# LasseWolter/laughter-detection-icsi

Measured on AMD Instinct MI355X. Metric: 1 s@16 kHz segments/sec (featurize+ResNet fwd/bwd), higher is better.
Workload: dtype f32 (64->64 and 32->32 convolutions: f16x2 split operands with per-tile power-of-two scales, f32 accumulate; error vs float64 within 1.5x of the exact-f32 kernels'); 1 GPU; BASELINE configs[2]: end-to-end featurize (HIP fbank 44 mel) + ResNetBigger resnet_base fwd/bwd + clip + Adam, random labels, dropout 0.5; global_batch=512, parallelism=dp1, overlap_wgrad=False, overlap_wgrad_small=True, bf16x3_convs=True, f16x2_convs=True, relu_bits=True, virtual_a1=True

## Files before the change

### include/lad_hip.h

```cpp
#ifndef LAD_HIP_H
#define LAD_HIP_H

#include <stdint.h>

#ifdef __cplusplus
extern "C" {
#endif

#define LAD_VERSION 100

enum lad_status {
    LAD_OK = 0,
    LAD_ERR_INVALID = -1,
    LAD_ERR_HIP = -2,
    LAD_ERR_NOMEM = -3,
    LAD_NOT_COVERED = 1
};

int lad_version(void);
const char *lad_last_error(void);

enum lad_pad_mode {
    LAD_PAD_KALDI_MIRROR = 0,
    LAD_PAD_CENTER_REFLECT = 1,
// ... 20 lines not shown

int lad_fbank_plan_create(const lad_fbank_cfg *cfg, const float *window, const float *melbank,
                          const float *dct, void **plan_out);
int lad_fbank_plan_destroy(void *plan);
int lad_fbank_plan_set_kernel(void *plan, int32_t which);
int lad_fbank_plan_has_fast_kernel(const void *plan);
int64_t lad_fbank_num_frames(const void *plan, int64_t samples_per_clip);
int lad_fbank_forward(void *plan, const float *pcm, int64_t n_clips, int64_t samples_per_clip,
                      float *out, void *stream);
int lad_fbank_forward_long(void *plan, const float *pcm, int64_t n_samples, float *out, void *stream);

int lad_gather_segments(const float *const *chan_ptr, const int64_t *chan_frames, const int32_t *chan,
                        const int64_t *first, const int32_t *count, int64_t n_seg, int32_t n_frames, int32_t F, float pad,
                        float *out, void *stream);

typedef struct lad_augment_params {
    uint64_t seed;
    uint32_t epoch;
    float p, mix_p;
    float snr_lo, snr_hi;
    float gain_lo, gain_hi;
    int32_t W;
    int32_t n_time, Wt;
    int32_t n_freq, Wf;
} lad_augment_params;
int lad_gather_segments_aug(const float *const *chan_ptr, const int64_t *chan_frames, const int32_t *chan,
                            const int64_t *first, const int32_t *count, int64_t n_seg, int32_t n_frames, int32_t F, float pad,
                            const lad_augment_params *params, const int32_t *noise_list, int32_t n_noise,
                            int64_t min_noise_frames, float *out, void *stream);

int lad_assemble_windows(const void *stream_act, const void *strips, void *out, int64_t n_windows, int32_t H, int32_t W,
                         int32_t band, int32_t row_bytes, void *stream);


int64_t lad_act_rows(int64_t batch, int32_t H, int32_t W);

int64_t lad_conv_packed_weight_floats(int32_t cout, int32_t cin, int32_t taps, int32_t mode);
int lad_conv_pack_weights(const float *w, int32_t cout, int32_t cin, int32_t taps, int32_t mode, float *wt,
                          void *stream);
int lad_conv_pack_weights_multi(const void *descs, int32_t n_desc, void *stream);
int64_t lad_conv_num_tiles(int64_t batch, int32_t H, int32_t W);
int lad_conv_fwd(const float *in, const float *wt, const float *bias, const float *addend, float *out,
                 float *stat_partials, int64_t batch, int32_t H, int32_t W, int32_t cin, int32_t cout, int32_t taps,
                 void *stream);
int lad_conv_s2_fwd(const float *in, const float *wt, const float *bias, float *out, float *stat_partials,
                    int64_t batch, int32_t H, int32_t W, int32_t cin, int32_t cout, int32_t taps, void *stream);
int lad_bn_fold(const float *gamma, const float *beta, const float *running_mean, const float *running_var,
                const float *conv_bias, int32_t channels, float *scale, float *shift, void *stream);
int lad_conv_fwd_eval(const float *in, const float *wt, const float *scale, const float *shift, const float *addend,
                      float *out, int64_t batch, int32_t H, int32_t W, int32_t cin, int32_t cout, int32_t taps,
                      int32_t relu, void *stream);
int lad_conv_s2_fwd_eval(const float *in, const float *wt, const float *scale, const float *shift, float *out,
                         int64_t batch, int32_t H, int32_t W, int32_t cin, int32_t cout, int32_t taps, int32_t relu,
                         void *stream);
int lad_upsample2(const float *src, float *up, int64_t batch, int32_t H, int32_t W, int32_t channels, void *stream);
int lad_conv_s2_dgrad(const float *dout, const float *wt, float *dx, int64_t batch, int32_t H, int32_t W, int32_t cin,
                      int32_t cout, int32_t taps, int32_t accumulate, void *stream);
int64_t lad_conv_s2_wgrad_workspace_floats(int32_t cin, int32_t cout, int32_t taps);
int lad_conv_s2_wgrad(const float *in, const float *dout, float *workspace, float *dw, float *dbias, int64_t batch, int32_t H,
                      int32_t W, int32_t cin, int32_t cout, int32_t taps, void *stream);
int64_t lad_conv_s2_wgrad_fused_workspace_floats(int32_t cin, int32_t cout);
int lad_conv_s2_wgrad_fused(const float *in, const float *dout, const float *dout_sc, float *workspace, float *dw,
                            float *dbias, float *dw_sc, int64_t batch, int32_t H, int32_t W, int32_t cin, int32_t cout,
                            void *stream);
int lad_conv_s2_fwd_fused(const float *in, const float *wt, const float *bias, const float *wt_sc, float *out,
                          float *stat_partials, float *out_sc, float *stat_partials_sc, int64_t batch, int32_t H, int32_t W,
                          int32_t cin, int32_t cout, void *stream);
int lad_conv_s2_dgrad_fused(const float *dout, const float *wt, const float *dout_sc, const float *wt_sc, float *dx,
                            int64_t batch, int32_t H, int32_t W, int32_t cin, int32_t cout, void *stream);
int64_t lad_conv_s2b3_packed_weight_bytes(void);
int lad_conv_s2b3_pack_weights(const float *w, const float *w_sc, void *wt, void *stream);
int lad_conv_s2b3_fwd(const float *in, const void *wt, const float *bias, float *out, float *stat_partials, float *out_sc,
                      float *stat_partials_sc, int64_t batch, int32_t H, int32_t W, void *stream);
int64_t lad_conv_s2b3_dgrad_packed_weight_bytes(void);
int lad_conv_s2b3_dgrad_pack_weights(const float *w, const float *w_sc, void *wt, void *stream);
int lad_conv_s2b3_pack_weights_pair(const float *w, const float *w_sc, void *wt_fwd, void *wt_dgrad, void *stream);
int64_t lad_conv_s2b3_dgrad_partials(int64_t batch, int32_t H, int32_t W);
int lad_conv_s2b3_dgrad(const float *dout, const float *dout_sc, const void *wt, float *dx, float *stat_partials, const float *bn_x,
                        const uint64_t *bn_bits, const float *bn_coef, int64_t batch, int32_t H, int32_t W, void *stream);
int64_t lad_conv_s2_dgrad_partials(int64_t batch, int32_t H, int32_t W);
int lad_conv_s2_dgrad_fused_bnstat(const float *dout, const float *wt, const float *dout_sc, const float *wt_sc, float *dx,
                                   float *stat_partials, const float *bn_x, const uint64_t *bn_bits, const float *bn_coef,
                                   int64_t batch, int32_t H, int32_t W, int32_t cin, int32_t cout, void *stream);
int64_t lad_conv_wgrad_workspace_floats(int32_t cin, int32_t cout, int32_t taps);
int lad_conv_wgrad(const float *in, const float *dout, float *workspace, float *dw, float *dbias, int64_t batch,
                   int32_t H, int32_t W, int32_t cin, int32_t cout, int32_t taps, void *stream);

int64_t lad_conv_b3_packed_weight_bytes(void);
int lad_conv_b3_pack_weights(const float *w, int32_t mode, void *wt, void *stream);
int lad_conv_b3_fwd_f32(const float *in, const void *wt, const float *bias, const float *addend, float *out,
                        float *partials, int64_t batch, int32_t H, int32_t W, void *stream);
int lad_conv_b3_fwd_f32_gated(const float *in, const void *wt, const float *bias, const float *addend,
                              const uint64_t *addend_bits, float *out, float *partials, int64_t batch, int32_t H,
                              int32_t W, void *stream);
int lad_conv_b3_dgrad_bnstat(const float *in, const void *wt, const float *addend, const uint64_t *addend_bits,
                             float *out, float *stat_partials, const float *bn_x, const uint64_t *bn_bits,
                             const float *bn_coef, int64_t batch, int32_t H, int32_t W, void *stream);
int64_t lad_conv_b3c_packed_weight_bytes(int32_t channels);
int lad_conv_b3c_pack_weights(const float *w, int32_t mode, void *wt, int32_t channels, void *stream);
int lad_conv_b3c_fwd_f32(const float *in, const void *wt, const float *bias, const float *addend, float *out,
                         float *partials, int64_t batch, int32_t H, int32_t W, int32_t channels, void *stream);
int lad_conv_b3c_dgrad_bnstat(const float *in, const void *wt, const float *addend, float *out, float *stat_partials,
                              const float *bn_x, const float *bn_coef, int64_t batch, int32_t H, int32_t W,
                              int32_t channels, void *stream);
int lad_conv_b3c_fwd_f32_bnrelu(const float *in, const float *in_coef, const void *wt, const float *bias, float *out,
                                float *partials, int64_t batch, int32_t H, int32_t W, int32_t channels, void *stream);
int64_t lad_conv_h2_packed_weight_bytes(int32_t channels);
int lad_conv_h2_pack_weights_multi(const void *table, int32_t n, int32_t channels, void *stream);
int lad_conv_wgrad_h2(const float *in, const float *in_coef, const float *dout, float *workspace, float *dw, float *dbias,
                      int64_t batch, int32_t H, int32_t W, int32_t channels, void *stream);
int lad_conv_wgrad_h2_bnbwd(const float *in, const float *in_coef, const float *dy, const float *bn_x, const uint64_t *bn_bits,
                            const float *bn_coef, const float *bcoef, float *dc, float *workspace, float *dw, float *dbias,
                            int64_t batch, int32_t H, int32_t W, int32_t channels, void *stream);
int lad_conv_h2(const float *in, const float *in_coef, const void *wt, const float *bias, const float *addend,
                const uint64_t *addend_bits, float *out, float *partials, const float *bn_x, const uint64_t *bn_bits,
                const float *bn_coef, int64_t batch, int32_t H, int32_t W, int32_t channels, void *stream);
int64_t lad_conv_wgrad_b3c_workspace_floats(int32_t channels);
int lad_conv_wgrad_b3c(const float *in, const float *in_coef, const float *dout, float *workspace, float *dw, float *dbias,
                       int64_t batch, int32_t H, int32_t W, int32_t channels, void *stream);
int lad_conv_b3_fwd_f32_bnrelu(const float *in, const float *in_coef, const void *wt, const float *bias, float *out,
                               float *partials, int64_t batch, int32_t H, int32_t W, void *stream);
int lad_conv_wgrad_b3_bnrelu(const float *in, const float *in_coef, const float *dout, float *workspace, float *dw,
                             float *dbias, int64_t batch, int32_t H, int32_t W, void *stream);
int lad_wgrad_defer_begin(void);
int lad_wgrad_defer_flush(void *stream);
int lad_conv_wgrad_b3(const float *in, const float *dout, float *workspace, float *dw, float *dbias, int64_t batch,
                      int32_t H, int32_t W, void *stream);

int lad_stem_fwd(const float *feat, const float *weight, float *out, float *stat_partials, int64_t batch, int32_t H,
                 int32_t W, int32_t cout, void *stream);
int lad_stem_fwd_eval(const float *feat, const float *weight, const float *scale, const float *shift, float *out,
                      int64_t batch, int32_t H, int32_t W, int32_t cout, int64_t frame_stride, int64_t frames_avail,
                      void *stream);
int64_t lad_stem_moments_workspace_doubles(void);
int64_t lad_stem_moments_doubles(void);
int lad_stem_bn_stats(const float *feat, const float *weight, const float *gamma, const float *beta, float *running_mean,
                      float *running_var, float momentum, float *coef, double *moments, double *workspace, int64_t batch, int32_t H,
                      int32_t W, int32_t cout, void *stream);
int64_t lad_stem_bwd_onepass_workspace_floats(void);
int lad_stem_bwd_onepass(const float *feat, const float *weight, const float *dy, const float *coef, const float *gamma,
                         const double *moments, float *workspace, float *dw, float *dgamma, float *dbeta, int64_t batch, int32_t H,
                         int32_t W, int32_t cout, void *stream);
int64_t lad_stem_wgrad_workspace_floats(void);
int lad_stem_wgrad(const float *feat, const float *dout, float *workspace, float *dw, int64_t batch, int32_t H,
                   int32_t W, int32_t cout, void *stream);
int lad_stem_wgrad_bn(const float *feat, const float *dy, const float *x, const float *weight, const float *coef,
                      const float *bcoef, float *workspace, float *dw, int64_t batch, int32_t H, int32_t W, int32_t cout,
                      void *stream);
int64_t lad_stem_bn_bwd_groups(int64_t batch, int32_t H, int32_t W);
int lad_stem_bn_bwd_sums(const float *feat, const float *weight, const float *dy, const float *coef, float *partials,
                         int64_t batch, int32_t H, int32_t W, int32_t cout, void *stream);

int lad_bn_finalize(float *stat_partials, int64_t n_tiles, int32_t channels, int64_t count, const float *gamma,
                    const float *beta, float *running_mean, float *running_var, float momentum, float *coef,
                    void *stream);
int lad_bn_finalize_pair(float *stat_partials_a, float *stat_partials_b, int64_t n_tiles, int32_t channels, int64_t count,
                         const float *gamma_a, const float *beta_a, float *running_mean_a, float *running_var_a, float *coef_a,
                         const float *gamma_b, const float *beta_b, float *running_mean_b, float *running_var_b, float *coef_b,
                         float momentum, void *stream);
int lad_bn_act(const float *x, const float *coef, const float *res, const float *res_coef, float *y, int64_t batch,
               int32_t H, int32_t W, int32_t channels, int32_t relu, void *stream);
int64_t lad_bn_bwd_workspace_floats(int32_t channels);
int lad_bn_bwd(const float *dy, const float *y, const float *x, const float *coef, const float *gamma,
               const float *xs, const float *scoef, const float *sgamma, float *dx, float *aux, float *dgamma,
               float *dbeta, float *dsgamma, float *dsbeta, float *workspace, float *bcoef, float *pre_partials,
               int64_t pre_tiles, int64_t batch, int32_t H, int32_t W, int32_t channels, int32_t relu, int32_t mode,
               void *stream);
int lad_bn_act_bits(const float *x, const float *coef, const float *res, const float *res_coef, float *y,
                    uint64_t *y_bits, int64_t batch, int32_t H, int32_t W, int32_t channels, void *stream);
int lad_bn_bwd_bits(const float *dy, const uint64_t *y_bits, const float *x, const float *coef, const float *gamma,
                    float *dx, float *dgamma, float *dbeta, float *workspace, float *bcoef, float *pre_partials,
                    int64_t pre_tiles, int64_t batch, int32_t H, int32_t W, int32_t channels, void *stream);
int lad_conv_fwd_bnstat(const float *in, const float *wt, const float *addend, float *out, float *stat_partials,
                        const float *bn_x, const float *bn_y, const float *bn_coef, int64_t batch, int32_t H, int32_t W,
                        int32_t cin, int32_t cout, int32_t taps, void *stream);

int lad_pool_fwd(const float *x, float *pooled, int64_t batch, int32_t H, int32_t W, int32_t channels, void *stream);
int lad_pool_bwd(const float *dpooled, float *dx, int64_t batch, int32_t H, int32_t W, int32_t channels, void *stream);
int64_t lad_head_workspace_floats(int64_t batch, int32_t F);
int lad_head_fwd_train(const float *const *params, const float *pooled, int64_t batch, int32_t F, const float *drop1,
                       const float *drop2, const int32_t *labels, float momentum, float *h, float *stats,
                       float *probs, float *metrics, void *stream);
int lad_head_fwd_train_rng(const float *const *params, const float *pooled, int64_t batch, int32_t F, float *drop1, float *drop2, float keep,
                           uint64_t seed, int64_t *rng_counter, int64_t *nbt, int32_t n_nbt, const int32_t *labels, float momentum,
                           float *h, float *stats, float *probs, float *metrics, void *stream);
int lad_head_fwd_eval(const float *const *params, const float *pooled, int64_t batch, int32_t F, float *probs,
                      void *stream);
int lad_bce_metrics(const float *probs, const int32_t *labels, int64_t n, float *metrics, void *stream);
int lad_head_bwd(const float *const *params, float *const *grads, const float *pooled, const float *h,
                 const float *stats, const float *probs, const float *dprobs, int64_t batch, int32_t F,
                 const float *drop1, const float *drop2, const int32_t *labels, float *workspace, float *dpooled,
                 void *stream);

int64_t lad_f16_packed_weight_halfs(int32_t cout, int32_t cin, int32_t taps);
int lad_f16_pack_weights(const float *w, int32_t cout, int32_t cin, int32_t taps, void *wt, void *stream);
int lad_f16_stem_fwd(const float *feat, const float *weight, const float *scale, const float *shift, void *out,
                     int64_t batch, int32_t H, int32_t W, int32_t cout, int64_t frame_stride, int64_t frames_avail,
                     void *stream);
int lad_f16_conv_fwd(const void *in, const void *wt, const float *scale, const float *shift, const void *addend, void *out,
                     int64_t batch, int32_t H, int32_t W, int32_t cin, int32_t cout, int32_t taps, int32_t relu,
                     void *stream);
int lad_f16_conv_s2_fwd(const void *in, const void *wt, const float *scale, const float *shift, void *out, int64_t batch,
                        int32_t H, int32_t W, int32_t cin, int32_t cout, int32_t taps, int32_t relu, void *stream);
int lad_f16_block_fwd(const void *x, const void *wt1, const float *scale1, const float *shift1, const void *wt2,
                      const float *scale2, const float *shift2, void *y, int64_t batch, int32_t H, int32_t W, int32_t channels,
                      void *stream);
int lad_f16_block_fwd_stem_rows(const void *stream_act, int64_t stream_rows, int64_t stream_row0, const float *feat, int64_t frames_avail,
                                const float *stem_weight, const float *stem_scale, const float *stem_shift, const void *wt1,
                                const float *scale1, const float *shift1, const void *wt2, const float *scale2, const float *shift2, void *y,
                                int64_t batch, int32_t H, int32_t W, void *stream);
int lad_f16_conv_s2_strips_fwd(const void *act, const void *wt, const float *scale, const float *shift, void *out, const void *wt_sc,
                               const float *scale_sc, const float *shift_sc, void *out_sc, int64_t n_windows, int32_t H, int32_t W,
                               int32_t band, int32_t strip_rows, int64_t bottom_image0, int64_t stream_row0, int64_t act_rows,
                               int32_t out_rows, void *stream);
int lad_f16_tail_fwd(const void *act, int64_t n_windows, int32_t H, int32_t W, int32_t band, int32_t strip_rows, int64_t bot_img0,
                     int64_t stream_row0, int32_t phases, int64_t phase_img, int64_t act_rows, const void *const *conv_params,
                     const float *const *head_params, int32_t F, float *probs, void *stream);
int lad_f16_conv_s2_fwd_windows(const void *act, const void *wt, const float *scale, const float *shift, void *out,
                                int64_t n_windows, int32_t H, int32_t W, int32_t band, int32_t cin, int32_t cout, int32_t taps,
                                int32_t relu, void *stream);
int lad_f16_conv_s2_fwd_mapped(const void *act, const void *wt, const float *scale, const float *shift, void *out,
                               int64_t n_windows, int32_t H, int32_t W, int32_t band, int32_t strip_rows, int64_t bottom_image0,
                               int64_t stream_row0, int32_t phases, int64_t phase_rows, int64_t act_rows, int32_t out_rows,
                               int32_t cin, int32_t cout, int32_t taps, int32_t relu, void *stream);
int lad_f16_conv_s2_fwd_sc(const void *in, const void *wt, const float *scale, const float *shift, void *out, const void *wt_sc,
                           const float *scale_sc, const float *shift_sc, void *out_sc, int64_t batch, int32_t H, int32_t W,
                           int32_t cin, int32_t cout, int32_t relu, void *stream);
int lad_f16_conv_s2_fwd_mapped_sc(const void *act, const void *wt, const float *scale, const float *shift, void *out,
                                  const void *wt_sc, const float *scale_sc, const float *shift_sc, void *out_sc, int64_t n_windows,
                                  int32_t H, int32_t W, int32_t band, int32_t strip_rows, int64_t bottom_image0, int64_t stream_row0,
                                  int32_t phases, int64_t phase_rows, int64_t act_rows, int32_t out_rows, int32_t cin, int32_t cout,
                                  int32_t relu, void *stream);
int lad_f16_pool_fwd(const void *x, float *pooled, int64_t batch, int32_t H, int32_t W, int32_t channels, void *stream);

int32_t lad_grad_sumsq_partials(void);
int lad_grad_sumsq(const float *grad, int64_t n, float *partials, int64_t *step_counter, void *stream);
int lad_grad_accumulate(float *acc, const float *grad, int64_t n, double scale, void *stream);
int lad_adam_step(float *param, float *grad, float *exp_avg, float *exp_avg_sq, int64_t n,
                  const float *sumsq_partials, double grad_scale, double max_norm, double lr, double beta1,
                  double beta2, double eps, int64_t step, const int64_t *step_counter, int32_t zero_grad,
                  float *norm_out, void *stream);

enum lad_runs_dtype { LAD_RUNS_F32 = 0, LAD_RUNS_F64 = 1 };
int32_t lad_runs_tile_frames(void);
int32_t lad_runs_max_thresholds(void);
int64_t lad_runs_workspace_bytes(int64_t channels, int64_t frames, int32_t n_thresholds);
int lad_runs_count(const void *probs, int32_t dtype, int64_t channels, int64_t frames, const double *thresholds,
                   int32_t n_thresholds, void *workspace, void *stream);
int lad_runs_fill(const void *probs, int32_t dtype, int64_t channels, int64_t frames, const double *thresholds,
                  int32_t n_thresholds, const void *workspace, const int32_t *counts_host, int32_t *table,
// ... 89 lines not shown
```

### laughter-detection-icsi_amd/_hip.py

```python
import ctypes
import os

import torch

_HERE = os.path.dirname(os.path.abspath(__file__))
LIB_PATH = os.environ.get("LAD_HIP_LIB") or os.path.join(_HERE, "liblad_hip.so")

c_void_p = ctypes.c_void_p
c_int = ctypes.c_int
c_i64 = ctypes.c_int64
c_float = ctypes.c_float
c_double = ctypes.c_double
c_i32 = ctypes.c_int32
c_float_p = ctypes.POINTER(ctypes.c_float)


class LadHipError(RuntimeError):
    pass


class FbankCfg(ctypes.Structure):
    _fields_ = [("n_fft", ctypes.c_int32), ("frame_len", ctypes.c_int32), ("hop", ctypes.c_int32),
                ("n_mels", ctypes.c_int32), ("n_mfcc", ctypes.c_int32), ("pad_mode", ctypes.c_int32),
                ("log_mode", ctypes.c_int32), ("remove_dc", ctypes.c_int32), ("preemph", ctypes.c_float),
                ("log_floor", ctypes.c_float)]


class AugmentParams(ctypes.Structure):
    _fields_ = [("seed", ctypes.c_uint64), ("epoch", ctypes.c_uint32), ("p", ctypes.c_float), ("mix_p", ctypes.c_float),
                ("snr_lo", ctypes.c_float), ("snr_hi", ctypes.c_float), ("gain_lo", ctypes.c_float), ("gain_hi", ctypes.c_float),
                ("W", ctypes.c_int32), ("n_time", ctypes.c_int32), ("Wt", ctypes.c_int32), ("n_freq", ctypes.c_int32),
                ("Wf", ctypes.c_int32)]


SIGNATURES = {
    "lad_version": (c_int, []),
    "lad_last_error": (ctypes.c_char_p, []),
    "lad_fbank_plan_create": (c_int, [ctypes.POINTER(FbankCfg), c_void_p, c_void_p, c_void_p,
                                      ctypes.POINTER(c_void_p)]),
    "lad_fbank_plan_destroy": (c_int, [c_void_p]),
    "lad_fbank_plan_set_kernel": (c_int, [c_void_p, c_int]),
    "lad_fbank_plan_has_fast_kernel": (c_int, [c_void_p]),
    "lad_fbank_num_frames": (c_i64, [c_void_p, c_i64]),
    "lad_fbank_forward": (c_int, [c_void_p, c_void_p, c_i64, c_i64, c_void_p, c_void_p]),
    "lad_fbank_forward_long": (c_int, [c_void_p, c_void_p, c_i64, c_void_p, c_void_p]),
    "lad_gather_segments": (c_int, [c_void_p] * 5 + [c_i64, c_i32, c_i32, c_float, c_void_p, c_void_p]),
    "lad_gather_segments_aug": (c_int, [c_void_p] * 5 + [c_i64, c_i32, c_i32, c_float, ctypes.POINTER(AugmentParams), c_void_p, c_i32, c_i64,
                                        c_void_p, c_void_p]),
    "lad_assemble_windows": (c_int, [c_void_p, c_void_p, c_void_p, c_i64, c_i32, c_i32, c_i32, c_i32, c_void_p]),
    "lad_act_rows": (c_i64, [c_i64, c_i32, c_i32]),
    "lad_conv_packed_weight_floats": (c_i64, [c_i32, c_i32, c_i32, c_i32]),
    "lad_conv_pack_weights": (c_int, [c_void_p, c_i32, c_i32, c_i32, c_i32, c_void_p, c_void_p]),
    "lad_conv_pack_weights_multi": (c_int, [c_void_p, c_i32, c_void_p]),
    "lad_conv_num_tiles": (c_i64, [c_i64, c_i32, c_i32]),
    "lad_conv_fwd": (c_int, [c_void_p] * 6 + [c_i64, c_i32, c_i32, c_i32, c_i32, c_i32, c_void_p]),
    "lad_conv_b3_packed_weight_bytes": (c_i64, []),
    "lad_conv_b3_pack_weights": (c_int, [c_void_p, c_i32, c_void_p, c_void_p]),
    "lad_conv_b3_fwd_f32": (c_int, [c_void_p] * 6 + [c_i64, c_i32, c_i32, c_void_p]),
    "lad_conv_b3c_packed_weight_bytes": (c_i64, [c_i32]),
    "lad_conv_b3c_pack_weights": (c_int, [c_void_p, c_i32, c_void_p, c_i32, c_void_p]),
    "lad_conv_b3c_fwd_f32": (c_int, [c_void_p] * 6 + [c_i64, c_i32, c_i32, c_i32, c_void_p]),
    "lad_conv_b3c_fwd_f32_bnrelu": (c_int, [c_void_p] * 6 + [c_i64, c_i32, c_i32, c_i32, c_void_p]),
    "lad_conv_b3c_dgrad_bnstat": (c_int, [c_void_p] * 7 + [c_i64, c_i32, c_i32, c_i32, c_void_p]),
    "lad_conv_h2_packed_weight_bytes": (c_i64, [c_i32]),
    "lad_conv_h2_pack_weights_multi": (c_int, [c_void_p, c_i32, c_i32, c_void_p]),
    "lad_conv_wgrad_h2": (c_int, [c_void_p] * 6 + [c_i64, c_i32, c_i32, c_i32, c_void_p]),
    "lad_conv_h2": (c_int, [c_void_p] * 11 + [c_i64, c_i32, c_i32, c_i32, c_void_p]),
    "lad_conv_wgrad_h2_bnbwd": (c_int, [c_void_p] * 11 + [c_i64, c_i32, c_i32, c_i32, c_void_p]),
    "lad_conv_wgrad_b3c_workspace_floats": (c_i64, [c_i32]),
    "lad_conv_wgrad_b3c": (c_int, [c_void_p] * 6 + [c_i64, c_i32, c_i32, c_i32, c_void_p]),
    "lad_conv_b3_fwd_f32_gated": (c_int, [c_void_p] * 7 + [c_i64, c_i32, c_i32, c_void_p]),
    "lad_conv_b3_fwd_f32_bnrelu": (c_int, [c_void_p] * 6 + [c_i64, c_i32, c_i32, c_void_p]),
    "lad_conv_wgrad_b3_bnrelu": (c_int, [c_void_p] * 6 + [c_i64, c_i32, c_i32, c_void_p]),
    "lad_wgrad_defer_begin": (c_int, []),
    "lad_wgrad_defer_flush": (c_int, [c_void_p]),
    "lad_conv_b3_dgrad_bnstat": (c_int, [c_void_p] * 9 + [c_i64, c_i32, c_i32, c_void_p]),
    "lad_conv_wgrad_b3": (c_int, [c_void_p] * 5 + [c_i64, c_i32, c_i32, c_void_p]),
    "lad_conv_s2_fwd": (c_int, [c_void_p] * 5 + [c_i64, c_i32, c_i32, c_i32, c_i32, c_i32, c_void_p]),
    "lad_bn_fold": (c_int, [c_void_p] * 5 + [c_i32, c_void_p, c_void_p, c_void_p]),
    "lad_conv_fwd_eval": (c_int, [c_void_p] * 6 + [c_i64, c_i32, c_i32, c_i32, c_i32, c_i32, c_i32, c_void_p]),
    "lad_conv_s2_fwd_eval": (c_int, [c_void_p] * 5 + [c_i64, c_i32, c_i32, c_i32, c_i32, c_i32, c_i32, c_void_p]),
    "lad_upsample2": (c_int, [c_void_p, c_void_p, c_i64, c_i32, c_i32, c_i32, c_void_p]),
    "lad_conv_s2_dgrad": (c_int, [c_void_p] * 3 + [c_i64, c_i32, c_i32, c_i32, c_i32, c_i32, c_i32, c_void_p]),
    "lad_conv_s2_wgrad_workspace_floats": (c_i64, [c_i32, c_i32, c_i32]),
    "lad_conv_s2_fwd_fused": (c_int, [c_void_p] * 8 + [c_i64, c_i32, c_i32, c_i32, c_i32, c_void_p]),
    "lad_conv_s2_dgrad_partials": (c_i64, [c_i64, c_i32, c_i32]),
    "lad_conv_s2b3_packed_weight_bytes": (c_i64, []),
    "lad_conv_s2b3_pack_weights": (c_int, [c_void_p, c_void_p, c_void_p, c_void_p]),
    "lad_conv_s2b3_fwd": (c_int, [c_void_p] * 7 + [c_i64, c_i32, c_i32, c_void_p]),
    "lad_conv_s2b3_dgrad_packed_weight_bytes": (c_i64, []),
    "lad_conv_s2b3_dgrad_pack_weights": (c_int, [c_void_p, c_void_p, c_void_p, c_void_p]),
    "lad_conv_s2b3_pack_weights_pair": (c_int, [c_void_p] * 5),
    "lad_conv_s2b3_dgrad_partials": (c_i64, [c_i64, c_i32, c_i32]),
    "lad_conv_s2b3_dgrad": (c_int, [c_void_p] * 8 + [c_i64, c_i32, c_i32, c_void_p]),
    "lad_conv_s2_dgrad_fused_bnstat": (c_int, [c_void_p] * 9 + [c_i64, c_i32, c_i32, c_i32, c_i32, c_void_p]),
    "lad_conv_s2_dgrad_fused": (c_int, [c_void_p] * 5 + [c_i64, c_i32, c_i32, c_i32, c_i32, c_void_p]),
    "lad_conv_s2_wgrad_fused_workspace_floats": (c_i64, [c_i32, c_i32]),
    "lad_conv_s2_wgrad_fused": (c_int, [c_void_p] * 7 + [c_i64, c_i32, c_i32, c_i32, c_i32, c_void_p]),
    "lad_conv_s2_wgrad": (c_int, [c_void_p] * 5 + [c_i64, c_i32, c_i32, c_i32, c_i32, c_i32, c_void_p]),
    "lad_conv_wgrad_workspace_floats": (c_i64, [c_i32, c_i32, c_i32]),
    "lad_conv_wgrad": (c_int, [c_void_p] * 5 + [c_i64, c_i32, c_i32, c_i32, c_i32, c_i32, c_void_p]),
    "lad_stem_fwd": (c_int, [c_void_p] * 4 + [c_i64, c_i32, c_i32, c_i32, c_void_p]),
    "lad_stem_fwd_eval": (c_int, [c_void_p] * 5 + [c_i64, c_i32, c_i32, c_i32, c_i64, c_i64, c_void_p]),
    "lad_stem_wgrad_workspace_floats": (c_i64, []),
    "lad_stem_wgrad": (c_int, [c_void_p] * 4 + [c_i64, c_i32, c_i32, c_i32, c_void_p]),
    "lad_stem_wgrad_bn": (c_int, [c_void_p] * 8 + [c_i64, c_i32, c_i32, c_i32, c_void_p]),
    "lad_stem_bn_bwd_groups": (c_i64, [c_i64, c_i32, c_i32]),
    "lad_stem_bn_bwd_sums": (c_int, [c_void_p] * 5 + [c_i64, c_i32, c_i32, c_i32, c_void_p]),
    "lad_bn_finalize": (c_int, [c_void_p, c_i64, c_i32, c_i64, c_void_p, c_void_p, c_void_p, c_void_p, c_float,
                                c_void_p, c_void_p]),
    "lad_stem_moments_workspace_doubles": (c_i64, []),
    "lad_stem_moments_doubles": (c_i64, []),
    "lad_stem_bn_stats": (c_int, [c_void_p] * 6 + [c_float] + [c_void_p] * 3 + [c_i64, c_i32, c_i32, c_i32, c_void_p]),
    "lad_stem_bwd_onepass_workspace_floats": (c_i64, []),
    "lad_stem_bwd_onepass": (c_int, [c_void_p] * 10 + [c_i64, c_i32, c_i32, c_i32, c_void_p]),
    "lad_bn_finalize_pair": (c_int, [c_void_p, c_void_p, c_i64, c_i32, c_i64] + [c_void_p] * 10 + [c_float, c_void_p]),
    "lad_bn_act": (c_int, [c_void_p] * 5 + [c_i64, c_i32, c_i32, c_i32, c_i32, c_void_p]),
    "lad_bn_bwd_workspace_floats": (c_i64, [c_i32]),
    "lad_bn_act_bits": (c_int, [c_void_p] * 6 + [c_i64, c_i32, c_i32, c_i32, c_void_p]),
    "lad_bn_bwd_bits": (c_int, [c_void_p] * 11 + [c_i64, c_i64, c_i32, c_i32, c_i32, c_void_p]),
    "lad_bn_bwd": (c_int, [c_void_p] * 17 + [c_i64, c_i64, c_i32, c_i32, c_i32, c_i32, c_i32, c_void_p]),
    "lad_conv_fwd_bnstat": (c_int, [c_void_p] * 8 + [c_i64, c_i32, c_i32, c_i32, c_i32, c_i32, c_void_p]),
    "lad_pool_fwd": (c_int, [c_void_p, c_void_p, c_i64, c_i32, c_i32, c_i32, c_void_p]),
    "lad_pool_bwd": (c_int, [c_void_p, c_void_p, c_i64, c_i32, c_i32, c_i32, c_void_p]),
    "lad_head_workspace_floats": (c_i64, [c_i64, c_i32]),
    "lad_head_fwd_train": (c_int, [c_void_p, c_void_p, c_i64, c_i32, c_void_p, c_void_p, c_void_p, c_float,
                                   c_void_p, c_void_p, c_void_p, c_void_p, c_void_p]),
    "lad_head_fwd_train_rng": (c_int, [c_void_p, c_void_p, c_i64, c_i32, c_void_p, c_void_p, c_float, ctypes.c_uint64, c_void_p, c_void_p, c_i32,
                                       c_void_p, c_float, c_void_p, c_void_p, c_void_p, c_void_p, c_void_p]),
    "lad_head_fwd_eval": (c_int, [c_void_p, c_void_p, c_i64, c_i32, c_void_p, c_void_p]),
    "lad_bce_metrics": (c_int, [c_void_p, c_void_p, c_i64, c_void_p, c_void_p]),
    "lad_head_bwd": (c_int, [c_void_p] * 7 + [c_i64, c_i32] + [c_void_p] * 6),
    "lad_f16_packed_weight_halfs": (c_i64, [c_i32, c_i32, c_i32]),
    "lad_f16_pack_weights": (c_int, [c_void_p, c_i32, c_i32, c_i32, c_void_p, c_void_p]),
    "lad_f16_stem_fwd": (c_int, [c_void_p] * 5 + [c_i64, c_i32, c_i32, c_i32, c_i64, c_i64, c_void_p]),
    "lad_f16_conv_fwd": (c_int, [c_void_p] * 6 + [c_i64, c_i32, c_i32, c_i32, c_i32, c_i32, c_i32, c_void_p]),
    "lad_f16_block_fwd": (c_int, [c_void_p] * 8 + [c_i64, c_i32, c_i32, c_i32, c_void_p]),
    "lad_f16_conv_s2_fwd_sc": (c_int, [c_void_p] * 9 + [c_i64, c_i32, c_i32, c_i32, c_i32, c_i32, c_void_p]),
    "lad_f16_conv_s2_fwd_mapped_sc": (c_int, [c_void_p] * 9 + [c_i64, c_i32, c_i32, c_i32, c_i32, c_i64, c_i64, c_i32, c_i64, c_i64, c_i32,
                                              c_i32, c_i32, c_i32, c_void_p]),
    "lad_f16_conv_s2_fwd": (c_int, [c_void_p] * 5 + [c_i64, c_i32, c_i32, c_i32, c_i32, c_i32, c_i32, c_void_p]),
    "lad_f16_conv_s2_fwd_windows": (c_int, [c_void_p] * 5 + [c_i64, c_i32, c_i32, c_i32, c_i32, c_i32, c_i32, c_i32, c_void_p]),
    "lad_f16_conv_s2_fwd_mapped": (c_int, [c_void_p] * 5 + [c_i64, c_i32, c_i32, c_i32, c_i32, c_i64, c_i64, c_i32, c_i64, c_i64, c_i32,
                                                          c_i32, c_i32, c_i32, c_i32, c_void_p]),
    "lad_f16_block_fwd_stem_rows": (c_int, [c_void_p, c_i64, c_i64, c_void_p, c_i64] + [c_void_p] * 10 + [c_i64, c_i32, c_i32, c_void_p]),
    "lad_f16_conv_s2_strips_fwd": (c_int, [c_void_p] * 9 + [c_i64, c_i32, c_i32, c_i32, c_i32, c_i64, c_i64, c_i64, c_i32, c_void_p]),
    "lad_f16_tail_fwd": (c_int, [c_void_p, c_i64, c_i32, c_i32, c_i32, c_i32, c_i64, c_i64, c_i32, c_i64, c_i64, c_void_p, c_void_p, c_i32,
                                 c_void_p, c_void_p]),
    "lad_f16_pool_fwd": (c_int, [c_void_p, c_void_p, c_i64, c_i32, c_i32, c_i32, c_void_p]),
    "lad_grad_sumsq_partials": (c_i32, []),
    "lad_grad_sumsq": (c_int, [c_void_p, c_i64, c_void_p, c_void_p, c_void_p]),
    "lad_grad_accumulate": (c_int, [c_void_p, c_void_p, c_i64, c_double, c_void_p]),
    "lad_adam_step": (c_int, [c_void_p] * 4 + [c_i64, c_void_p] + [c_double] * 6 + [c_i64, c_void_p, c_i32, c_void_p, c_void_p]),
    "lad_runs_tile_frames": (c_i32, []),
    "lad_runs_max_thresholds": (c_i32, []),
    "lad_runs_workspace_bytes": (c_i64, [c_i64, c_i64, c_i32]),
    "lad_runs_count": (c_int, [c_void_p, c_i32, c_i64, c_i64, ctypes.POINTER(c_double), c_i32, c_void_p, c_void_p]),
    "lad_runs_fill": (c_int, [c_void_p, c_i32, c_i64, c_i64, ctypes.POINTER(c_double), c_i32, c_void_p,
                              ctypes.POINTER(c_i32), c_void_p, c_i64, c_void_p]),
    "lad_score_max_min_lengths": (c_i32, []),
    "lad_score_workspace_bytes": (c_i64, [c_i64, c_i64, c_i32, c_i32]),
    "lad_score_runs": (c_int, [c_void_p, c_void_p, ctypes.POINTER(c_i32), c_i64, c_i64, c_i32, c_void_p, c_void_p,
                               ctypes.POINTER(c_i32), ctypes.POINTER(c_i32), c_i64, c_void_p, ctypes.POINTER(c_double),
                               ctypes.POINTER(c_double), c_i32, c_void_p, c_void_p, c_void_p]),
    "lad_score_events_workspace_bytes": (c_i64, [c_i64, c_i64, c_i32, c_i32, c_i64]),
    "lad_score_events": (c_int, [c_void_p, c_void_p, ctypes.POINTER(c_i32), c_i64, c_i64, c_i32, c_void_p, c_void_p,
                                 ctypes.POINTER(c_i32), ctypes.POINTER(c_i32), c_i64, c_void_p, ctypes.POINTER(c_double),
                                 ctypes.POINTER(c_double), c_i32, c_i32, c_i32, c_void_p, c_void_p, c_void_p]),
    "lad_binarize_max_settings": (c_i32, []),
    "lad_binarize_workspace_bytes": (c_i64, [c_i64, c_i64, c_i32]),
    "lad_binarize_count": (c_int, [c_void_p, c_i32, c_i64, c_i64, ctypes.POINTER(c_double), ctypes.POINTER(c_double), c_i32,
                                   c_void_p, c_void_p]),
    "lad_binarize_fill": (c_int, [c_void_p, c_i32, c_i64, c_i64] + [ctypes.POINTER(c_double)] * 3
                          + [c_i32, c_void_p, ctypes.POINTER(c_double), c_void_p, ctypes.POINTER(c_i32), c_void_p, c_void_p, c_i64,
                             c_void_p]),
    "lad_viterbi_max_settings": (c_i32, []),
    "lad_viterbi_table_entries": (c_i32, []),
    "lad_viterbi_workspace_bytes": (c_i64, [c_i64, c_i64, c_i32]),
    "lad_viterbi_count": (c_int, [c_void_p, c_i32, c_i64, c_i64, c_void_p] + [ctypes.POINTER(c_i32)] * 3
                          + [c_i32, c_void_p, c_void_p, c_void_p]),
    "lad_viterbi_fill": (c_int, [c_void_p, ctypes.POINTER(c_i32), c_i64, c_i64, c_i32, c_void_p, c_i64, c_void_p]),
    "lad_surface_max_levels": (c_i32, []),
    "lad_surface_tile_frames": (c_i32, []),
    "lad_surface_workspace_bytes": (c_i64, [c_i64, c_i64, c_i64, c_i32, c_i32]),
    "lad_score_surface": (c_int, [c_void_p, c_i32, c_i64, c_i64, ctypes.POINTER(c_double), c_i32, c_void_p, c_void_p,
                                  ctypes.POINTER(c_i32), ctypes.POINTER(c_i32), c_i64, c_void_p, ctypes.POINTER(c_double),
                                  ctypes.POINTER(c_double), c_i32, c_void_p, c_void_p, c_void_p]),
    "lad_surface_events_workspace_bytes": (c_i64, [c_i64, c_i64, c_i64, c_i32, c_i32]),
    "lad_score_surface_events": (c_int, [c_void_p, c_i32, c_i64, c_i64, ctypes.POINTER(c_double), c_i32, c_void_p, c_void_p,
                                         ctypes.POINTER(c_i32), ctypes.POINTER(c_i32), c_i64, c_void_p, ctypes.POINTER(c_double),
                                         ctypes.POINTER(c_double), c_i32, c_i32, c_i32, c_void_p, c_void_p, c_void_p, c_void_p]),
    "lad_resample_out_len": (c_i64, [c_i64, c_i32, c_i32]),
    "lad_resample_tile_outputs": (c_i32, []),
    "lad_resample_max_up": (c_i32, []),
    "lad_resample_max_down": (c_i32, []),
    "lad_resample_max_taps": (c_i32, []),
    "lad_resample_max_lds_bytes": (c_i64, []),
    "lad_resample_lds_bytes": (c_i64, [c_i32, c_i32, c_i32]),
    "lad_resample": (c_int, [c_void_p, c_i32, c_i64, c_void_p, c_i32, c_i32, c_i32, c_i64, c_i64, c_void_p, c_void_p]),
    "lad_lowpass_tile_frames": (c_i32, []),
    "lad_lowpass_workspace_bytes": (c_i64, [c_i64, c_i64]),
    "lad_lowpass": (c_int, [c_void_p, c_i32, c_i64, c_i64, ctypes.POINTER(c_i64)] + [ctypes.POINTER(c_double)] * 3
# ... 54 lines not shown
```

### laughter-detection-icsi_amd/csrc/bn.hip

```cpp
#include "lad_common.h"
#include "lad_device.h"
#include "lad_bn_math.h"

namespace {
using namespace lad;

constexpr float BN_EPS = 1e-5f;
constexpr int THREADS = 256;

struct FinSet {
    const float *partials, *gamma, *beta;
    float *running_mean, *running_var, *coef;
};
struct FinSets {
    FinSet s[2];
};
__global__ void bn_finalize_kernel(FinSets sets, int64_t n_tiles, int C, double count, float momentum) {
    const FinSet f = sets.s[blockIdx.y];
    const float *__restrict__ partials = f.partials;
    float *__restrict__ coef = f.coef;
    const int c = blockIdx.x;
    double s1 = 0.0, s2 = 0.0;
    int64_t t = threadIdx.x;
    const int64_t bd = blockDim.x;
// ... 109 lines not shown
    __syncthreads();
    if (!last_s) return;
    if (threadIdx.x == 0) __hip_atomic_store(ft.ticket, 0u, __ATOMIC_RELAXED, __HIP_MEMORY_SCOPE_AGENT);
    const int slices = (int)gridDim.x;
    double *tot = &red[0][0];
    if (threadIdx.x < cols) {
        double tt = 0.0;
        double *hd = reinterpret_cast<double *>(partials) + threadIdx.x;
        const int64_t step = rows_per_slice * cols / 2;
        int b = 0;
        for (; b + 32 <= slices; b += 32) {
            double v[32];
#pragma unroll
            for (int u = 0; u < 32; ++u) v[u] = __hip_atomic_load(hd + (b + u) * step, __ATOMIC_RELAXED, __HIP_MEMORY_SCOPE_AGENT);
#pragma unroll
            for (int u = 0; u < 32; ++u) tt += v[u];
        }
        for (; b + 8 <= slices; b += 8) {
            double v[8];
#pragma unroll
            for (int u = 0; u < 8; ++u) v[u] = __hip_atomic_load(hd + (b + u) * step, __ATOMIC_RELAXED, __HIP_MEMORY_SCOPE_AGENT);
#pragma unroll
            for (int u = 0; u < 8; ++u) tt += v[u];
        }
        for (; b < slices; ++b) tt += __hip_atomic_load(hd + b * step, __ATOMIC_RELAXED, __HIP_MEMORY_SCOPE_AGENT);
        tot[threadIdx.x] = tt;
    }
    __syncthreads();
    const int c = threadIdx.x;
    if (c >= C) return;
    if (!ft.backward) {
        float *coef = ft.out;
        const double count = ft.count;
        const double mean = tot[c] / count;
        double var = tot[C + c] / count - mean * mean;
        if (var < 0.0) var = 0.0;
        const double invstd_d = 1.0 / sqrt(var + (double)BN_EPS);
        const float invstd = (float)invstd_d;
        const float scale = ft.gamma[c] * invstd;
        coef[0 * C + c] = scale;
        coef[1 * C + c] = ft.beta[c] - (float)mean * scale;
        coef[2 * C + c] = (float)mean;
        coef[3 * C + c] = invstd;
        coef[4 * C + c] = (float)(mean - (double)(float)mean);
        coef[5 * C + c] = (float)(invstd_d - (double)invstd);
        if (ft.running_mean != nullptr) {
            const double unbiased = count > 1.0 ? var * count / (count - 1.0) : var;
            ft.running_mean[c] = (1.0f - ft.momentum) * ft.running_mean[c] + ft.momentum * (float)mean;
            ft.running_var[c] = (1.0f - ft.momentum) * ft.running_var[c] + ft.momentum * (float)unbiased;
        }
    } else {
        float *bcoef = ft.out;
        const double t0 = tot[c], t1 = tot[C + c];
        ft.dbeta[c] = (float)t0;
        ft.dgamma[c] = (float)t1;
        const double k2 = t0 / ft.count, k3 = t1 / ft.count;
        bcoef[0 * C + c] = ft.gamma[c] * ft.coef[3 * C + c];
        bcoef[1 * C + c] = (float)k2;
        bcoef[2 * C + c] = (float)k3;
        bcoef[4 * C + c] = (float)(k2 - (double)(float)k2);
        bcoef[6 * C + c] = (float)(k3 - (double)(float)k3);
    }
}

struct RowGeom {
    int64_t n_img_rows;
    int Hp, Wp;
};

struct RowPack {
    int rows, sub, f0, fstep;
};
__device__ __forceinline__ RowPack row_pack(int per_row) {
    RowPack p{1, 0, (int)threadIdx.x, (int)blockDim.x};
    if (2 * per_row <= (int)blockDim.x) {
        p.rows = (int)blockDim.x / per_row;
        p.sub = (int)threadIdx.x / per_row;
        p.f0 = (int)threadIdx.x - p.sub * per_row;
        p.fstep = per_row;
    }
    return p;
}

template <int RES, bool BITS = false>
__global__ void bn_act_kernel(const float4 *__restrict__ x, const float *__restrict__ coef,
                              const float4 *__restrict__ res, const float *__restrict__ rcoef, float4 *__restrict__ y,
                              RowGeom g, int C, int c4shift, int relu, unsigned long long *__restrict__ bits = nullptr) {
    const int c = (threadIdx.x * 4) & (C - 1);
    const int per_row = g.Wp << c4shift;
    const float4 sc = *reinterpret_cast<const float4 *>(coef + c);
    const float4 sh = *reinterpret_cast<const float4 *>(coef + C + c);
    float4 rs = sc, rh = sh;
    if (RES == 2) {
        rs = *reinterpret_cast<const float4 *>(rcoef + c);
        rh = *reinterpret_cast<const float4 *>(rcoef + C + c);
    }
    const RowPack rp = row_pack(per_row);
    for (int64_t r = (int64_t)blockIdx.x * rp.rows + rp.sub; rp.sub < rp.rows && r < g.n_img_rows; r += (int64_t)gridDim.x * rp.rows) {
        const int yp = (int)(r % g.Hp);
        const bool border_row = (yp == 0);
        const int64_t base = r * per_row;
        for (int f = rp.f0; f < per_row; f += rp.fstep) {
            const int64_t idx = base + f;
            const int xp = f >> c4shift;
            float4 o = make_float4(0.f, 0.f, 0.f, 0.f);
            if (!(border_row | (xp == 0))) {
                const float4 v = x[idx];
                o = make_float4(fmaf(v.x, sc.x, sh.x), fmaf(v.y, sc.y, sh.y), fmaf(v.z, sc.z, sh.z), fmaf(v.w, sc.w, sh.w));
                if (RES == 1) {
                    const float4 rr = res[idx];
                    o.x += rr.x; o.y += rr.y; o.z += rr.z; o.w += rr.w;
                } else if (RES == 2) {
                    const float4 rr = res[idx];
                    o.x += fmaf(rr.x, rs.x, rh.x); o.y += fmaf(rr.y, rs.y, rh.y);
                    o.z += fmaf(rr.z, rs.z, rh.z); o.w += fmaf(rr.w, rs.w, rh.w);
                }
                if (relu) {
                    o.x = fmaxf(o.x, 0.f); o.y = fmaxf(o.y, 0.f); o.z = fmaxf(o.z, 0.f); o.w = fmaxf(o.w, 0.f);
                }
            }
            y[idx] = o;
            if (BITS) {
                const unsigned long long word = pack_sign_bits(o, threadIdx.x & 63);
                if ((threadIdx.x & 15) == 0) bits[idx >> 4] = word;
            }
        }
    }
}

template <int C, bool SHORT>
__global__ __launch_bounds__(THREADS) void bn_bwd_reduce_kernel(const float4 *__restrict__ dy, const float4 *__restrict__ y,
                                                                const float4 *__restrict__ x, const float *__restrict__ coef,
                                                                const float4 *__restrict__ xs, const float *__restrict__ scoef,
                                                                float *__restrict__ partials, int64_t rows, int relu,
                                                                const unsigned long long *__restrict__ bits) {
    constexpr int C4 = C / 4;
    constexpr int RP = THREADS / C4;
    constexpr int K = SHORT ? 3 : 2;
    const int c4 = threadIdx.x % C4, rp = threadIdx.x / C4;
    const Norm4 nm = load_norm(coef, C, c4 * 4);
    Norm4 sn = nm;
    if (SHORT) sn = load_norm(scoef, C, c4 * 4);
    const float4 fscale = *reinterpret_cast<const float4 *>(coef + c4 * 4);
    const float4 fshift = *reinterpret_cast<const float4 *>(coef + C + c4 * 4);
    float4 a0 = make_float4(0, 0, 0, 0), a1 = a0, a2 = a0;
    for (int64_t row = (int64_t)blockIdx.x * RP + rp; row < rows; row += (int64_t)gridDim.x * RP) {
        const int64_t idx = row * C4 + c4;
        float4 d = dy[idx];
        const float4 xv = x[idx];
        if (relu == 1) {
            const float4 yy = y[idx];
            d.x = yy.x > 0.f ? d.x : 0.f; d.y = yy.y > 0.f ? d.y : 0.f;
            d.z = yy.z > 0.f ? d.z : 0.f; d.w = yy.w > 0.f ? d.w : 0.f;
        } else if (relu == 2) {
            d = mask_from_x(d, xv, fscale, fshift);
        } else if (relu == 3) {
            d = mask_from_bits(d, bits[row], c4);
        }
        a0.x += d.x; a0.y += d.y; a0.z += d.z; a0.w += d.w;
        const float4 xh = xhat4(xv, nm);
        a1.x = fmaf(d.x, xh.x, a1.x); a1.y = fmaf(d.y, xh.y, a1.y);
        a1.z = fmaf(d.z, xh.z, a1.z); a1.w = fmaf(d.w, xh.w, a1.w);
        if (SHORT) {
            const float4 sh = xhat4(xs[idx], sn);
            a2.x = fmaf(d.x, sh.x, a2.x); a2.y = fmaf(d.y, sh.y, a2.y);
            a2.z = fmaf(d.z, sh.z, a2.z); a2.w = fmaf(d.w, sh.w, a2.w);
        }
    }
    __shared__ float red[RP][K][C];
    *reinterpret_cast<float4 *>(&red[rp][0][c4 * 4]) = a0;
    *reinterpret_cast<float4 *>(&red[rp][1][c4 * 4]) = a1;
    if (SHORT) *reinterpret_cast<float4 *>(&red[rp][2][c4 * 4]) = a2;
    __syncthreads();
    for (int t = threadIdx.x; t < K * C; t += THREADS) {
        const int k = t / C, c = t - k * C;
        float s = 0.f;
#pragma unroll 4
        for (int p = 0; p < RP; ++p) s += red[p][k][c];
        partials[((int64_t)blockIdx.x * K + k) * C + c] = s;
    }
}

__global__ void bn_bwd_finalize_kernel(const float *__restrict__ partials, int groups, int K, int C, double count,
                                       const float *__restrict__ gamma, const float *__restrict__ coef,
                                       const float *__restrict__ sgamma, const float *__restrict__ scoef,
                                       float *__restrict__ dgamma, float *__restrict__ dbeta,
                                       float *__restrict__ dsgamma, float *__restrict__ dsbeta, float *__restrict__ bcoef) {
    const int c = blockIdx.x;
    double s[3] = {0.0, 0.0, 0.0};
    int g = threadIdx.x;
    const int bd = blockDim.x;
    const int k2 = K - 1;
    for (; g + 3 * bd < groups; g += 4 * bd) {
        float v[4][3];
#pragma unroll
        for (int u = 0; u < 4; ++u) {
            const float *row = partials + (int64_t)(g + u * bd) * K * C + c;
            v[u][0] = row[0];
            v[u][1] = row[C];
            v[u][2] = row[k2 * C];
        }
#pragma unroll
        for (int u = 0; u < 4; ++u) {
            s[0] += (double)v[u][0];
            s[1] += (double)v[u][1];
            s[2] += (double)v[u][2];
        }
    }
    for (; g < groups; g += bd) {
        const float *row = partials + (int64_t)g * K * C + c;
        const float v0 = row[0], v1 = row[C], v2 = row[k2 * C];
        s[0] += (double)v0;
        s[1] += (double)v1;
        s[2] += (double)v2;
    }
    __shared__ double red[3][THREADS / 64];
    for (int k = 0; k < 3; ++k) {
        const double v = wave_sum64d(s[k]);
        if ((threadIdx.x & 63) == 0) red[k][threadIdx.x >> 6] = v;
    }
    __syncthreads();
    if (threadIdx.x == 0) {
        double t[3] = {0.0, 0.0, 0.0};
        for (int k = 0; k < 3; ++k)
            for (int w = 0; w < THREADS / 64; ++w) t[k] += red[k][w];
        dbeta[c] = (float)t[0];
        dgamma[c] = (float)t[1];
        const double k2 = t[0] / count, k3 = t[1] / count;
        bcoef[0 * C + c] = gamma[c] * coef[3 * C + c];
        bcoef[1 * C + c] = (float)k2;
        bcoef[2 * C + c] = (float)k3;
        bcoef[4 * C + c] = (float)(k2 - (double)(float)k2);
        bcoef[6 * C + c] = (float)(k3 - (double)(float)k3);
        if (K == 3) {
            const double j3 = t[2] / count;
            dsbeta[c] = (float)t[0];
            dsgamma[c] = (float)t[2];
            bcoef[3 * C + c] = sgamma[c] * scoef[3 * C + c];
            bcoef[5 * C + c] = (float)j3;
            bcoef[7 * C + c] = (float)(j3 - (double)(float)j3);
        }
    }
}

template <int MODE>
__global__ void bn_bwd_apply_kernel(const float4 *__restrict__ dy, const float4 *__restrict__ y, const float4 *__restrict__ x,
                                    const float *__restrict__ coef, const float *__restrict__ bcoef,
                                    const float4 *__restrict__ xs, const float *__restrict__ scoef, float4 *__restrict__ dx,
                                    float4 *__restrict__ aux, RowGeom g, int C, int c4shift, int relu,
                                    const unsigned long long *__restrict__ bits) {
    const int c = (threadIdx.x * 4) & (C - 1);
    const int per_row = g.Wp << c4shift;
    const float4 zero = make_float4(0.f, 0.f, 0.f, 0.f);
    const float4 fsc = *reinterpret_cast<const float4 *>(coef + c), fsh = *reinterpret_cast<const float4 *>(coef + C + c);
    const Norm4 nm = load_norm(coef, C, c);
    const float4 k1 = *reinterpret_cast<const float4 *>(bcoef + 0 * C + c);
    const float4 k2 = *reinterpret_cast<const float4 *>(bcoef + 1 * C + c);
    const float4 k3 = *reinterpret_cast<const float4 *>(bcoef + 2 * C + c);
    const float4 k2l = *reinterpret_cast<const float4 *>(bcoef + 4 * C + c);
    const float4 k3l = *reinterpret_cast<const float4 *>(bcoef + 6 * C + c);
    Norm4 sn = nm;
    float4 j1 = k1, j3 = k3, j3l = k3l;
    if (MODE == 2) {
        sn = load_norm(scoef, C, c);
        j1 = *reinterpret_cast<const float4 *>(bcoef + 3 * C + c);
        j3 = *reinterpret_cast<const float4 *>(bcoef + 5 * C + c);
        j3l = *reinterpret_cast<const float4 *>(bcoef + 7 * C + c);
    }
    const RowPack rp = row_pack(per_row);
    for (int64_t r = (int64_t)blockIdx.x * rp.rows + rp.sub; rp.sub < rp.rows && r < g.n_img_rows; r += (int64_t)gridDim.x * rp.rows) {
        const int yp = (int)(r % g.Hp);
        const bool border_row = (yp == 0);
        const int64_t base = r * per_row;
        for (int f = rp.f0; f < per_row; f += rp.fstep) {
            const int64_t idx = base + f;
            const int xp = f >> c4shift;
            if (border_row | (xp == 0)) {
                dx[idx] = zero;
                if (MODE != 0) aux[idx] = zero;
                continue;
            }
            float4 d = dy[idx];
            const float4 xv = x[idx];
            if (relu == 1) {
                const float4 yy = y[idx];
                d.x = yy.x > 0.f ? d.x : 0.f; d.y = yy.y > 0.f ? d.y : 0.f;
                d.z = yy.z > 0.f ? d.z : 0.f; d.w = yy.w > 0.f ? d.w : 0.f;
            } else if (relu == 2) {
                d = mask_from_x(d, xv, fsc, fsh);
            } else if (relu == 3) {
                d = mask_from_bits(d, bits[idx >> 4], threadIdx.x & 15);
            }
            const float4 xh = xhat4(xv, nm);
            float4 o;
            o.x = bn_dx1(d.x, xh.x, k1.x, k2.x, k2l.x, k3.x, k3l.x);
            o.y = bn_dx1(d.y, xh.y, k1.y, k2.y, k2l.y, k3.y, k3l.y);
            o.z = bn_dx1(d.z, xh.z, k1.z, k2.z, k2l.z, k3.z, k3l.z);
            o.w = bn_dx1(d.w, xh.w, k1.w, k2.w, k2l.w, k3.w, k3l.w);
            dx[idx] = o;
            if (MODE == 1) {
                aux[idx] = d;
            } else if (MODE == 2) {
                const float4 sh = xhat4(xs[idx], sn);
                float4 sv;
                sv.x = bn_dx1(d.x, sh.x, j1.x, k2.x, k2l.x, j3.x, j3l.x);
                sv.y = bn_dx1(d.y, sh.y, j1.y, k2.y, k2l.y, j3.y, j3l.y);
                sv.z = bn_dx1(d.z, sh.z, j1.z, k2.z, k2l.z, j3.z, j3l.z);
                sv.w = bn_dx1(d.w, sh.w, j1.w, k2.w, k2l.w, j3.w, j3l.w);
                aux[idx] = sv;
            }
        }
    }
}

unsigned row_grid(int64_t n_img_rows, int float4_per_row) {
    const int rows = 2 * float4_per_row <= THREADS ? THREADS / float4_per_row : 1;
    return (unsigned)std::min<int64_t>(lad::ceil_div(n_img_rows, (int64_t)rows), float4_per_row >= 2 * THREADS ? 256 * 256 : 256 * 32);
}
int log2_exact(int v) {
    int s = 0;
    while ((1 << s) < v) ++s;
    return s;
}
RowGeom make_row_geom(int64_t batch, int H, int W) {
    RowGeom g;
    g.Hp = H + 1;
    g.Wp = W + 1;
    g.n_img_rows = batch * g.Hp;
    return g;
}
constexpr int BWD_GROUPS = 1024;
}

extern "C" int lad_bn_finalize(float *stat_partials, int64_t n_tiles, int32_t channels, int64_t count,
                               const float *gamma, const float *beta, float *running_mean, float *running_var,
                               float momentum, float *coef, void *stream) {
    using namespace lad;
    LAD_REQUIRE(stat_partials && gamma && beta && coef, "lad_bn_finalize: null buffer");
    LAD_REQUIRE(channels > 0 && n_tiles > 0 && count > 0, "lad_bn_finalize: bad sizes");
    LAD_REQUIRE((running_mean == nullptr) == (running_var == nullptr), "lad_bn_finalize: running stats must come in pairs");
    if (n_tiles >= TWO_LEVEL_MIN_TILES && 2 * channels <= 128 && THREADS % (channels / 2) == 0) {
        const int64_t rps = ceil_div(n_tiles, FIN_SLICES);
        const int slices = (int)(n_tiles / rps);
        const FinTail ft{0, (double)count, gamma, beta, nullptr, running_mean, running_var, momentum, coef, nullptr, nullptr, launch_ticket()};
        LAD_REQUIRE(ft.ticket, "lad_bn_finalize: no ticket for the two-level sum");
        hipLaunchKernelGGL(bn_slice_sum_kernel, dim3(slices), dim3(THREADS), 0, (hipStream_t)stream, stat_partials, n_tiles, channels, rps, ft);
        return check_launch("bn_slice_sum_kernel");
    }
    const FinSets sets{{{stat_partials, gamma, beta, running_mean, running_var, coef}, {nullptr, nullptr, nullptr, nullptr, nullptr, nullptr}}};
    hipLaunchKernelGGL(bn_finalize_kernel, dim3(channels, 1), dim3(THREADS), 0, (hipStream_t)stream, sets, n_tiles, channels, (double)count, momentum);
    return check_launch("bn_finalize_kernel");
}

extern "C" int lad_bn_finalize_pair(float *stat_partials_a, float *stat_partials_b, int64_t n_tiles, int32_t channels, int64_t count,
                                    const float *gamma_a, const float *beta_a, float *running_mean_a, float *running_var_a, float *coef_a,
                                    const float *gamma_b, const float *beta_b, float *running_mean_b, float *running_var_b, float *coef_b,
                                    float momentum, void *stream) {
    using namespace lad;
    LAD_REQUIRE(stat_partials_a && stat_partials_b && gamma_a && beta_a && coef_a && gamma_b && beta_b && coef_b, "lad_bn_finalize_pair: null buffer");
    LAD_REQUIRE(channels > 0 && n_tiles > 0 && count > 0, "lad_bn_finalize_pair: bad sizes");
    LAD_REQUIRE((running_mean_a == nullptr) == (running_var_a == nullptr) && (running_mean_b == nullptr) == (running_var_b == nullptr),
                "lad_bn_finalize_pair: running stats must come in pairs");
    if (n_tiles >= TWO_LEVEL_MIN_TILES && 2 * channels <= 128 && THREADS % (channels / 2) == 0) {
        const int rc = lad_bn_finalize(stat_partials_a, n_tiles, channels, count, gamma_a, beta_a, running_mean_a, running_var_a, momentum, coef_a, stream);
        return rc ? rc : lad_bn_finalize(stat_partials_b, n_tiles, channels, count, gamma_b, beta_b, running_mean_b, running_var_b, momentum, coef_b, stream);
    }
    const FinSets sets{{{stat_partials_a, gamma_a, beta_a, running_mean_a, running_var_a, coef_a},
                        {stat_partials_b, gamma_b, beta_b, running_mean_b, running_var_b, coef_b}}};
    hipLaunchKernelGGL(bn_finalize_kernel, dim3(channels, 2), dim3(THREADS), 0, (hipStream_t)stream, sets, n_tiles, channels, (double)count, momentum);
    return check_launch("bn_finalize_kernel");
}

__global__ void bn_fold_kernel(const float *__restrict__ gamma, const float *__restrict__ beta,
                               const float *__restrict__ running_mean, const float *__restrict__ running_var,
                               const float *__restrict__ conv_bias, int C, float *__restrict__ scale, float *__restrict__ shift) {
    const int c = blockIdx.x * blockDim.x + threadIdx.x;
    if (c < C) {
        const float s = gamma[c] / sqrtf(running_var[c] + BN_EPS);
        const float b = conv_bias != nullptr ? conv_bias[c] : 0.0f;
        scale[c] = s;
        shift[c] = fmaf(b - running_mean[c], s, beta[c]);
    }
}

extern "C" int lad_bn_fold(const float *gamma, const float *beta, const float *running_mean, const float *running_var,
                           const float *conv_bias, int32_t channels, float *scale, float *shift, void *stream) {
    using namespace lad;
    LAD_REQUIRE(gamma && beta && running_mean && running_var && scale && shift && channels > 0, "lad_bn_fold: bad argument");
    hipLaunchKernelGGL(bn_fold_kernel, dim3((unsigned)ceil_div(channels, 64)), dim3(64), 0, (hipStream_t)stream, gamma, beta,
                       running_mean, running_var, conv_bias, channels, scale, shift);
    return check_launch("bn_fold_kernel");
}

namespace {
int bn_act_impl(const float *x, const float *coef, const float *res, const float *res_coef, float *y, unsigned long long *bits,
                int64_t batch, int32_t H, int32_t W, int32_t channels, int32_t relu, void *stream, const char *who) {
    using namespace lad;
    LAD_REQUIRE(x && coef && y, "%s: null buffer", who);
    LAD_REQUIRE(channels >= 4 && channels <= 4 * THREADS && (channels & (channels - 1)) == 0, "%s: channels must be a power of two in 4..1024", who);
    LAD_REQUIRE(res != nullptr || res_coef == nullptr, "%s: res_coef without res", who);
    LAD_REQUIRE(batch >= 0 && H >= 1 && W >= 1, "%s: bad geometry", who);
    LAD_REQUIRE(bits == nullptr || channels == 64, "%s: sign bits are kept for 64-channel activations only", who);
    if (batch == 0) return LAD_OK;
    const RowGeom g = make_row_geom(batch, H, W);
    const int sh = log2_exact(channels / 4);
    const dim3 grid(row_grid(g.n_img_rows, g.Wp << sh)), block(THREADS);
    hipStream_t st = (hipStream_t)stream;
#define LAD_ACT(RES, R, RC)                                                                                                   \
    do {                                                                                                                      \
        if (bits)                                                                                                             \
            hipLaunchKernelGGL((bn_act_kernel<RES, true>), grid, block, 0, st, (const float4 *)x, coef, (const float4 *)(R), RC, \
                               (float4 *)y, g, channels, sh, relu, bits);                                                     \
        else                                                                                                                  \
            hipLaunchKernelGGL((bn_act_kernel<RES, false>), grid, block, 0, st, (const float4 *)x, coef, (const float4 *)(R), RC, \
                               (float4 *)y, g, channels, sh, relu, nullptr);                                                  \
    } while (0)
    if (res == nullptr)
        LAD_ACT(0, nullptr, nullptr);
    else if (res_coef == nullptr)
        LAD_ACT(1, res, nullptr);
    else
        LAD_ACT(2, res, res_coef);
#undef LAD_ACT
    return check_launch("bn_act_kernel");
}
}

extern "C" int lad_bn_act(const float *x, const float *coef, const float *res, const float *res_coef, float *y,
                          int64_t batch, int32_t H, int32_t W, int32_t channels, int32_t relu, void *stream) {
    return bn_act_impl(x, coef, res, res_coef, y, nullptr, batch, H, W, channels, relu, stream, "lad_bn_act");
}

extern "C" int lad_bn_act_bits(const float *x, const float *coef, const float *res, const float *res_coef, float *y,
                               uint64_t *y_bits, int64_t batch, int32_t H, int32_t W, int32_t channels, void *stream) {
    using namespace lad;
    LAD_REQUIRE(y_bits, "lad_bn_act_bits: null sign-bit buffer");
    return bn_act_impl(x, coef, res, res_coef, y, (unsigned long long *)y_bits, batch, H, W, channels, 1, stream, "lad_bn_act_bits");
}

extern "C" int64_t lad_bn_bwd_workspace_floats(int32_t channels) { return (int64_t)BWD_GROUPS * 3 * channels; }

namespace {
int bn_bwd_impl(const float *dy, const float *y, const unsigned long long *bits, const float *x, const float *coef, const float *gamma,
                const float *xs, const float *scoef, const float *sgamma, float *dx, float *aux,
                float *dgamma, float *dbeta, float *dsgamma, float *dsbeta, float *workspace, float *bcoef,
                float *pre_partials, int64_t pre_tiles, int64_t batch, int32_t H, int32_t W, int32_t channels,
                int32_t relu, int32_t mode, void *stream) {
    using namespace lad;
    LAD_REQUIRE(relu != 3 || (bits && channels == 64), "lad_bn_bwd_bits: sign bits are kept for 64-channel activations only");
    LAD_REQUIRE(dy && coef && gamma && dgamma && dbeta && workspace && bcoef, "lad_bn_bwd: null buffer");
    LAD_REQUIRE(x || (pre_partials && !dx), "lad_bn_bwd: x may only be omitted when the sums are given and nothing is applied");
    LAD_REQUIRE(dx || mode == 0, "lad_bn_bwd: dx may only be omitted (sums and coefficients only) in mode 0");
    LAD_REQUIRE(relu >= 0 && relu <= 3, "lad_bn_bwd: relu must be 0 (none), 1 (mask from y), 2 (mask recomputed from x) or 3 (sign bits: lad_bn_bwd_bits)");
    LAD_REQUIRE(relu != 1 || y, "lad_bn_bwd: relu = 1 needs y");
    LAD_REQUIRE(relu != 2 || mode == 0, "lad_bn_bwd: relu = 2 (mask recomputed from x) is for the residual-free BatchNorm only");
    LAD_REQUIRE(mode >= 0 && mode <= 2, "lad_bn_bwd: bad mode");
    LAD_REQUIRE(mode == 0 || aux, "lad_bn_bwd: mode needs aux");
    LAD_REQUIRE(mode != 2 || (xs && scoef && sgamma && dsgamma && dsbeta), "lad_bn_bwd: mode 2 needs the shortcut tensors");
    LAD_REQUIRE(channels == 16 || channels == 32 || channels == 64 || channels == 128, "lad_bn_bwd: channels must be 16, 32, 64 or 128");
    LAD_REQUIRE(batch >= 0 && H >= 1 && W >= 1, "lad_bn_bwd: bad geometry");
    if (batch == 0) return LAD_OK;
    const RowGeom rg = make_row_geom(batch, H, W);
    const int64_t rows = rg.n_img_rows * rg.Wp;
    const int64_t count = batch * H * W;
    hipStream_t st = (hipStream_t)stream;
    const int rp = THREADS / (channels / 4);
    int groups = (int)std::min<int64_t>(BWD_GROUPS, ceil_div(rows, rp));
    const bool sh = mode == 2;
    const float *sums = workspace;
    if (pre_partials != nullptr) {
        LAD_REQUIRE(!sh && pre_tiles >= 1 && pre_tiles < (1 << 30), "lad_bn_bwd: pre-computed sums are for modes 0 and 1");
        sums = pre_partials;
        groups = (int)pre_tiles;
    } else {
#define LAD_RED(CC)                                                                                                  \
    if (channels == CC) {                                                                                            \
        if (sh)                                                                                                      \
            hipLaunchKernelGGL((bn_bwd_reduce_kernel<CC, true>), dim3(groups), dim3(THREADS), 0, st, (const float4 *)dy, \
                               (const float4 *)y, (const float4 *)x, coef, (const float4 *)xs, scoef, workspace, rows, relu, bits); \
        else                                                                                                         \
            hipLaunchKernelGGL((bn_bwd_reduce_kernel<CC, false>), dim3(groups), dim3(THREADS), 0, st, (const float4 *)dy, \
                               (const float4 *)y, (const float4 *)x, coef, nullptr, nullptr, workspace, rows, relu, bits); \
    }
    LAD_RED(16) LAD_RED(32) LAD_RED(64) LAD_RED(128)
#undef LAD_RED
    }
    int rc = check_launch("bn_bwd_reduce_kernel");
    if (rc) return rc;
    if (pre_partials != nullptr && groups >= TWO_LEVEL_MIN_TILES && 2 * channels <= 128 && THREADS % (channels / 2) == 0) {
        const int64_t rps = ceil_div((int64_t)groups, FIN_SLICES);
        const int slices = (int)(groups / rps);
        const FinTail ft{1, (double)count, gamma, nullptr, coef, nullptr, nullptr, 0.0f, bcoef, dgamma, dbeta, launch_ticket()};
        LAD_REQUIRE(ft.ticket, "lad_bn_bwd: no ticket for the two-level sum");
        hipLaunchKernelGGL(bn_slice_sum_kernel, dim3(slices), dim3(THREADS), 0, st, pre_partials, (int64_t)groups, channels, rps, ft);
    } else {
        hipLaunchKernelGGL(bn_bwd_finalize_kernel, dim3(channels), dim3(THREADS), 0, st, sums, groups, sh ? 3 : 2, channels,
                           (double)count, gamma, coef, sgamma, scoef, dgamma, dbeta, dsgamma, dsbeta, bcoef);
    }
    rc = check_launch("bn_bwd_finalize_kernel");
    if (rc) return rc;
    if (dx == nullptr) return LAD_OK;
    const int c4s = log2_exact(channels / 4);
    const dim3 grid(row_grid(rg.n_img_rows, rg.Wp << c4s)), block(THREADS);
    if (mode == 0)
        hipLaunchKernelGGL(bn_bwd_apply_kernel<0>, grid, block, 0, st, (const float4 *)dy, (const float4 *)y, (const float4 *)x,
                           coef, bcoef, nullptr, nullptr, (float4 *)dx, nullptr, rg, channels, c4s, relu, bits);
    else if (mode == 1)
        hipLaunchKernelGGL(bn_bwd_apply_kernel<1>, grid, block, 0, st, (const float4 *)dy, (const float4 *)y, (const float4 *)x,
                           coef, bcoef, nullptr, nullptr, (float4 *)dx, (float4 *)aux, rg, channels, c4s, relu, bits);
    else
        hipLaunchKernelGGL(bn_bwd_apply_kernel<2>, grid, block, 0, st, (const float4 *)dy, (const float4 *)y, (const float4 *)x,
                           coef, bcoef, (const float4 *)xs, scoef, (float4 *)dx, (float4 *)aux, rg, channels, c4s, relu, bits);
    return check_launch("bn_bwd_apply_kernel");
}
}

extern "C" int lad_bn_bwd(const float *dy, const float *y, const float *x, const float *coef, const float *gamma,
                          const float *xs, const float *scoef, const float *sgamma, float *dx, float *aux,
                          float *dgamma, float *dbeta, float *dsgamma, float *dsbeta, float *workspace, float *bcoef,
                          float *pre_partials, int64_t pre_tiles, int64_t batch, int32_t H, int32_t W, int32_t channels,
                          int32_t relu, int32_t mode, void *stream) {
    using namespace lad;
    LAD_REQUIRE(relu >= 0 && relu <= 2, "lad_bn_bwd: relu must be 0, 1 or 2");
    return bn_bwd_impl(dy, y, nullptr, x, coef, gamma, xs, scoef, sgamma, dx, aux, dgamma, dbeta, dsgamma, dsbeta, workspace, bcoef,
                       pre_partials, pre_tiles, batch, H, W, channels, relu, mode, stream);
}

extern "C" int lad_bn_bwd_bits(const float *dy, const uint64_t *y_bits, const float *x, const float *coef, const float *gamma,
                               float *dx, float *dgamma, float *dbeta, float *workspace, float *bcoef, float *pre_partials,
                               int64_t pre_tiles, int64_t batch, int32_t H, int32_t W, int32_t channels, void *stream) {
    using namespace lad;
    LAD_REQUIRE(y_bits && x, "lad_bn_bwd_bits: null buffer");
// ... 4 lines not shown
```

### laughter-detection-icsi_amd/csrc/conv_h2.hip

```cpp
#include "lad_common.h"
#include "lad_device.h"
#include "lad_b3_tile.h"
#include "lad_bn_math.h"
#include "lad_h2.h"

#include <algorithm>
#include <cstdlib>

namespace {
using namespace lad;
using namespace lad::b3t;

constexpr int KC = 32;
constexpr int ROWB = 128;
constexpr int FPIECES = KC * 4 / 16;

template <int C>
struct H2 {
    static constexpr int NSTAGE = C / KC;
    static constexpr int NCT = C / 16;
    static constexpr int PLANE_B = NCT * 1024;
    static constexpr int TAP_BYTES = 2 * PLANE_B;
    static constexpr int IMG_BYTES = TAPS * NSTAGE * TAP_BYTES;
    static constexpr int TAIL_BYTES = 16;
// ... 295 lines not shown
            b3_epilogue<C, STAT>(store_acc, bias, addend, abits, out, partials, mask_s + rb * TM, reinterpret_cast<float *>(smem_b), qs, g.rows, bst);
        else
            h2_epilogue<C, STAT, (EPI & 1) != 0, (EPI >> 1) & 3, (EPI & 8) != 0, (EPI & 16) != 0>(
                store_acc, bias, addend, abits, out, partials, mask_s + rb * TM, reinterpret_cast<float *>(smem_b), qs, g.rows, bst);
    }
    LAD_H2_STAMP(12)
}

template <int C, int RB>
size_t h2_lds_bytes(const Geom &g) {
    using K = H2<C>;
    const int nrows = TM * RB + 2 * (g.Wp + 1);
    const size_t main_bytes = std::max<size_t>(NSLOT * K::TAP_BYTES + (size_t)nrows * ROWB, (size_t)TM * (C + 4) * 4);
    return main_bytes + TM * RB + 16;
}

int h2_two_rounds() {
    static int n = 0;
    if (n == 0) {
        int dev = 0;
        hipDeviceProp_t prop;
        n = (hipGetDevice(&dev) == hipSuccess && hipGetDeviceProperties(&prop, dev) == hipSuccess && prop.multiProcessorCount > 0)
                ? 4 * prop.multiProcessorCount : 1024;
    }
    return n;
}

struct H2Args {
    const float *in, *in_coef;
    const unsigned char *wt;
    const float *bias, *addend;
    const unsigned long long *abits;
    float *out, *partials;
    B3Stat bst;
    Geom g;
    hipStream_t stream;
};

template <int C, int RB, bool STAT, bool INBN, int EPI>
int launch_h2_form(const H2Args &a) {
    static lad::DeviceOnce attr_set;
    if (!attr_set) {
        LAD_HIP_CHECK(hipFuncSetAttribute((const void *)conv_h2_kernel<C, RB, STAT, INBN, EPI>, hipFuncAttributeMaxDynamicSharedMemorySize, 96 * 1024));
        attr_set = true;
    }
    const int64_t tiles = ceil_div(a.g.rows, TM * RB);
    hipLaunchKernelGGL((conv_h2_kernel<C, RB, STAT, INBN, EPI>), dim3((unsigned)(ceil_div(tiles, 8) * 8)), dim3(THREADS), (h2_lds_bytes<C, RB>(a.g)),
                       a.stream, a.in, a.wt, a.bias, a.addend, a.abits, a.out, a.partials, a.g, a.bst, a.in_coef);
    return check_launch("conv_h2_kernel");
}

template <int C, int RB, bool STAT, bool INBN>
int launch_h2_rb(const H2Args &a) {
    const int form = h2_epi(a.bias != nullptr, a.addend == nullptr ? H2_ADD_NONE : a.abits == nullptr ? H2_ADD_PLAIN : H2_ADD_GATED,
                            a.partials != nullptr, STAT && a.bst.bits != nullptr);
#define LAD_H2_FORM(...)                                                                                                           \
    if (form == h2_epi(__VA_ARGS__)) return launch_h2_form<C, RB, STAT, INBN, h2_epi(__VA_ARGS__)>(a);
    if constexpr (STAT) {
        LAD_H2_FORM(false, H2_ADD_NONE, true, false)
        LAD_H2_FORM(false, H2_ADD_GATED, true, true)
    } else {
        LAD_H2_FORM(true, H2_ADD_NONE, true, false)
        LAD_H2_FORM(true, H2_ADD_PLAIN, true, false)
        if constexpr (!INBN) {
            LAD_H2_FORM(false, H2_ADD_NONE, false, false)
            LAD_H2_FORM(false, H2_ADD_PLAIN, false, false)
            LAD_H2_FORM(false, H2_ADD_GATED, false, false)
        }
    }
#undef LAD_H2_FORM
    return launch_h2_form<C, RB, STAT, INBN, H2_EPI_ANY>(a);
}

template <int C, bool STAT, bool INBN>
int launch_h2(const float *in, const float *in_coef, const void *wt, const float *bias, const float *addend, const uint64_t *abits,
              float *out, float *partials, const B3Stat &bst, int64_t batch, int32_t H, int32_t W, void *stream, const char *who) {
    const Geom g = make_geom(batch, H, W);
    LAD_REQUIRE(g.rows < ((int64_t)1 << 31) && g.img < (1 << 20), "%s: more than 2^31 rows, or an image of more than 2^20 positions", who);
    LAD_REQUIRE(W <= 46, "%s: image too wide for the tile (W = %d)", who, W);
    const H2Args a{in, in_coef, (const unsigned char *)wt, bias, addend, (const unsigned long long *)abits, out, partials, bst, g, (hipStream_t)stream};
    if (ceil_div(g.rows, TM * 2) < h2_two_rounds()) return launch_h2_rb<C, 1, STAT, INBN>(a);
    return launch_h2_rb<C, 2, STAT, INBN>(a);
}
}

extern "C" int64_t lad_conv_h2_packed_weight_bytes(int32_t channels) {
    if (channels == 64) return H2<64>::IMG_BYTES + H2<64>::TAIL_BYTES;
    if (channels == 32) return H2<32>::IMG_BYTES + H2<32>::TAIL_BYTES;
    return -1;
}

extern "C" int lad_conv_h2_pack_weights_multi(const void *table, int32_t n, int32_t channels, void *stream) {
    using namespace lad;
    LAD_REQUIRE(table && n >= 1, "lad_conv_h2_pack_weights_multi: empty table");
    static_assert(sizeof(PackRec) == 24, "record layout");
    if (channels == 64) hipLaunchKernelGGL(pack_h2_kernel<64>, dim3(n * PACK_SPLIT), dim3(1024), 0, (hipStream_t)stream, (const PackRec *)table);
    else if (channels == 32) hipLaunchKernelGGL(pack_h2_kernel<32>, dim3(n * PACK_SPLIT), dim3(1024), 0, (hipStream_t)stream, (const PackRec *)table);
    else if (channels == 0) hipLaunchKernelGGL(pack_h2_kernel<0>, dim3(n * PACK_SPLIT), dim3(1024), 0, (hipStream_t)stream, (const PackRec *)table);
    else return fail(LAD_ERR_INVALID, "lad_conv_h2_pack_weights_multi: 64 or 32 channels, or 0 = per record (got %d)", channels);
    return check_launch("pack_h2_kernel");
}

extern "C" int lad_conv_h2(const float *in, const float *in_coef, const void *wt, const float *bias, const float *addend,
                           const uint64_t *addend_bits, float *out, float *partials, const float *bn_x, const uint64_t *bn_bits,
                           const float *bn_coef, int64_t batch, int32_t H, int32_t W, int32_t channels, void *stream) {
    using namespace lad;
    const char *who = "lad_conv_h2";
    LAD_REQUIRE(batch >= 1 && H >= 1 && W >= 1, "%s: bad geometry", who);
    LAD_REQUIRE(in && wt && out, "%s: null buffer", who);
    LAD_REQUIRE(addend_bits == nullptr || addend != nullptr, "%s: sign bits without an addend", who);
    LAD_REQUIRE((const void *)in != (const void *)out, "%s: the convolution cannot run in place", who);
    const bool stat = bn_x != nullptr;
    LAD_REQUIRE(!stat || (partials && bn_coef), "%s: the BatchNorm sums need partials and bn_coef", who);
    LAD_REQUIRE(stat || bn_bits == nullptr, "%s: bn_bits without bn_x", who);
    LAD_REQUIRE(!(stat && in_coef), "%s: an input BatchNorm and the backward sums are not combined", who);
    LAD_REQUIRE(channels == 64 || (addend_bits == nullptr && bn_bits == nullptr), "%s: sign bits are kept for 64-channel activations only", who);
    const B3Stat bst{bn_x, (const unsigned long long *)bn_bits, bn_coef};
    if (channels == 64) {
        if (stat) return launch_h2<64, true, false>(in, nullptr, wt, bias, addend, addend_bits, out, partials, bst, batch, H, W, stream, who);
        if (in_coef) return launch_h2<64, false, true>(in, in_coef, wt, bias, addend, addend_bits, out, partials, bst, batch, H, W, stream, who);
        return launch_h2<64, false, false>(in, nullptr, wt, bias, addend, addend_bits, out, partials, bst, batch, H, W, stream, who);
    }
    if (channels == 32) {
        if (stat) return launch_h2<32, true, false>(in, nullptr, wt, bias, addend, addend_bits, out, partials, bst, batch, H, W, stream, who);
        if (in_coef) return launch_h2<32, false, true>(in, in_coef, wt, bias, addend, addend_bits, out, partials, bst, batch, H, W, stream, who);
        return launch_h2<32, false, false>(in, nullptr, wt, bias, addend, addend_bits, out, partials, bst, batch, H, W, stream, who);
    }
    return fail(LAD_ERR_INVALID, "%s: 64 or 32 channels (got %d)", who, channels);
}

#ifdef LAD_STAMP
extern "C" int lad_debug_read_h2_stamps(unsigned long long *host_dst, int64_t n) {
    return hipMemcpyFromSymbol(host_dst, HIP_SYMBOL(lad_dbg_h2), n * sizeof(unsigned long long)) == hipSuccess ? 0 : -2;
}
#endif
```

### laughter-detection-icsi_amd/csrc/conv_s2_bwd.hip

```cpp
#include <type_traits>

#include "lad_common.h"
#include "lad_device.h"
#include "lad_bn_math.h"

namespace {
using namespace lad;

constexpr int THREADS = 256;
constexpr int TM = 128;

template <int N>
struct NTl {
    static constexpr int NT = (N + 31) / 32;
    static constexpr int NP = NT * 32;
};

struct ClassGeom {
    int A, Bx;
    int py, px;
    int64_t total;
};

__device__ __forceinline__ uint32_t udiv_f64(uint32_t n, uint32_t d, double inv, uint32_t &rem) {
    uint32_t qt = (uint32_t)((double)n * inv);
    uint32_t r = n - qt * d;
    if (r >= d) { r -= d; ++qt; }
    rem = r;
    return qt;
}

template <int G, int NT>
struct S2Chunk {
    static constexpr int cap(int g) { return (g > 1 && g * (1 + NT) > 24) ? cap(g / 2) : g; }
    static constexpr int GC = cap(G);
    static_assert(G % GC == 0, "chunks of whole 8-channel groups");
};

struct S2Stat {
    const float *x;
    const unsigned long long *bits;
    const float *coef;
    float *partials;
};

template <int KC, int NC, int TAPS, bool SC = false, bool STAT = false>
__global__ __launch_bounds__(THREADS, 2) void dgrad_s2_kernel(const float *__restrict__ dout, const float *__restrict__ wt,
                                                              float *__restrict__ dx, Geom glo, Geom ghi, int H, int W,
                                                              int64_t batch, int accumulate,
                                                              const float *__restrict__ dout_sc = nullptr,
                                                              const float *__restrict__ wt_sc = nullptr,
                                                              S2Stat bst = S2Stat{nullptr, nullptr, nullptr, nullptr}) {
    static_assert(!SC || TAPS == 9, "the shortcut rides with the 3x3 convolution");
    static_assert(!STAT || (SC && NC == 64), "the fused sums are written for the 64-channel transition with the shortcut fused");
    constexpr int NT = NTl<NC>::NT;
    constexpr int NP = NTl<NC>::NP;
    constexpr int K4 = KC / 4;
    constexpr int G = KC / 8;
    constexpr int GC = S2Chunk<G, NT>::GC;
    constexpr int LDO = NC + 4;
    __shared__ __attribute__((aligned(16))) float out_s[TM * LDO];
    __shared__ int qrow_s[TM];
    const int tid = threadIdx.x, lane = tid & 63, wave = tid >> 6;
    const int i = lane & 31, gk = lane >> 5;
    ClassGeom c;
    c.py = (TAPS == 9) ? (blockIdx.y >> 1) : 0;
    c.px = (TAPS == 9) ? (blockIdx.y & 1) : 0;
    c.A = (H - c.py + 1) / 2;
    c.Bx = (W - c.px + 1) / 2;
    c.total = batch * c.A * c.Bx;
    const int64_t m0 = (int64_t)blockIdx.x * TM;
    if (m0 >= c.total) {
        if (STAT && tid < 2 * NC) bst.partials[((int64_t)blockIdx.y * gridDim.x + blockIdx.x) * (2 * NC) + tid] = 0.0f;
        return;
    }

    const uint32_t per_img = (uint32_t)(c.A * c.Bx);
    const uint32_t m = (uint32_t)m0 + wave * 32 + i;
    const bool ok = (int64_t)m < c.total;
    uint32_t r, bq;
    const uint32_t img = udiv_f64(ok ? m : 0u, per_img, 1.0 / (double)per_img, r);
    const uint32_t aq = udiv_f64(r, (uint32_t)c.Bx, 1.0 / (double)c.Bx, bq);
    const int a = (int)aq, b = (int)bq;
    const int64_t lo_base = (int64_t)img * glo.img;
    if (gk == 0) qrow_s[wave * 32 + i] = ok ? (int)(img * (uint32_t)ghi.img + (uint32_t)(2 * a + c.py + 1) * (uint32_t)ghi.Wp + (uint32_t)(2 * b + c.px + 1)) : -1;

    f32x16 acc[NT];
#pragma unroll
    for (int n = 0; n < NT; ++n)
#pragma unroll
        for (int rr = 0; rr < 16; ++rr) acc[n][rr] = 0.0f;

    const float *w_base = wt + (gk * NP + i) * 4;
    const int nky = (TAPS == 9 && c.py) ? 2 : 1, nkx = (TAPS == 9 && c.px) ? 2 : 1;
    const int ntap = nky * nkx;
    const int nloop = ntap + ((SC && blockIdx.y == 0) ? 1 : 0);
#pragma unroll 1
    for (int t = 0; t < nloop; ++t) {
        const bool sc_tap = SC && t == ntap;
        const int ky = (TAPS == 9) ? (c.py ? 2 * (t / nkx) : 1) : 0;
        const int kx = (TAPS == 9) ? (c.px ? 2 * (t % nkx) : 1) : 0;
        const int ypo = (TAPS == 9) ? (2 * a + c.py + 1 - ky) / 2 + 1 : a + 1;
        const int xpo = (TAPS == 9) ? (2 * b + c.px + 1 - kx) / 2 + 1 : b + 1;
        const float *ap = (sc_tap ? dout_sc : dout) + (lo_base + (int64_t)ypo * glo.Wp + xpo) * KC + 4 * gk;
        const int slot = (TAPS == 9) ? 8 - (3 * ky + kx) : 0;
        const float *wp = sc_tap ? wt_sc + (gk * NP + i) * 4 : w_base + slot * (K4 * NP * 4);
        float4 av[G], bv[G][NT];
#pragma unroll
        for (int g0 = 0; g0 < G; g0 += GC) {
#pragma unroll
            for (int c8 = g0; c8 < g0 + GC; ++c8) {
                av[c8] = *reinterpret_cast<const float4 *>(ap + c8 * 8);
#pragma unroll
                for (int n = 0; n < NT; ++n) bv[c8][n] = *reinterpret_cast<const float4 *>(wp + (c8 * 2 * NP + n * 32) * 4);
            }
#pragma unroll
            for (int c8 = g0; c8 < g0 + GC; ++c8) {
#pragma unroll
                for (int n = 0; n < NT; ++n) acc[n] = mfma32(av[c8].x, bv[c8][n].x, acc[n]);
#pragma unroll
                for (int n = 0; n < NT; ++n) acc[n] = mfma32(av[c8].y, bv[c8][n].y, acc[n]);
#pragma unroll
                for (int n = 0; n < NT; ++n) acc[n] = mfma32(av[c8].z, bv[c8][n].z, acc[n]);
#pragma unroll
                for (int n = 0; n < NT; ++n) acc[n] = mfma32(av[c8].w, bv[c8][n].w, acc[n]);
            }
        }
    }
    float *my = out_s + wave * 32 * LDO;
#pragma unroll
    for (int n = 0; n < NT; ++n) {
        const int co = n * 32 + i;
        if (co < NC) {
#pragma unroll
            for (int rr = 0; rr < 16; ++rr) my[acc_row(rr, lane) * LDO + co] = acc[n][rr];
        }
    }
// ... 277 lines not shown
    LAD_DG_CASE(32, 32, 9)
    LAD_DG_CASE(32, 32, 1)
    return fail(LAD_ERR_INVALID, "lad_conv_s2_dgrad: unsupported (cin=%d, cout=%d, taps=%d)", cin, cout, taps);
}

extern "C" int64_t lad_conv_s2_wgrad_workspace_floats(int32_t cin, int32_t cout, int32_t taps) {
    if (cin <= 0 || cout <= 0 || (taps != 1 && taps != 9)) return -1;
    return (int64_t)MAX_GROUPS * ((int64_t)taps * cin * cout + cout);
}

#define LAD_WG2_CASE(CI, CO, T)               \
    if (cin == CI && cout == CO && taps == T) \
        return launch_wgrad<CI, CO, T>(in, dout, workspace, dw, dbias, batch, H, W, (hipStream_t)stream);

extern "C" int lad_conv_s2_wgrad(const float *in, const float *dout, float *workspace, float *dw, float *dbias, int64_t batch,
                                 int32_t H, int32_t W, int32_t cin, int32_t cout, int32_t taps, void *stream) {
    using namespace lad;
    LAD_REQUIRE(in && dout && workspace && dw, "lad_conv_s2_wgrad: null buffer");
    LAD_REQUIRE(batch >= 1 && H >= 1 && W >= 1, "lad_conv_s2_wgrad: bad geometry");
    LAD_WG2_CASE(64, 32, 9)
    LAD_WG2_CASE(32, 16, 9)
    LAD_WG2_CASE(16, 16, 9)
    LAD_WG2_CASE(64, 32, 1)
    LAD_WG2_CASE(32, 16, 1)
    LAD_WG2_CASE(16, 16, 1)
    LAD_WG2_CASE(128, 64, 9)
    LAD_WG2_CASE(128, 64, 1)
    LAD_WG2_CASE(32, 32, 9)
    LAD_WG2_CASE(32, 32, 1)
    return fail(LAD_ERR_INVALID, "lad_conv_s2_wgrad: unsupported (cin=%d, cout=%d, taps=%d)", cin, cout, taps);
}

extern "C" int64_t lad_conv_s2_wgrad_fused_workspace_floats(int32_t cin, int32_t cout) {
    if (cin <= 0 || cout <= 0) return -1;
    return (int64_t)MAX_GROUPS * ((int64_t)9 * cin * cout + cout + (int64_t)cin * cout);
}

#define LAD_WG2F_CASE(CI, CO)      \
    if (cin == CI && cout == CO) \
        return launch_wgrad<CI, CO, 9, true>(in, dout, workspace, dw, dbias, batch, H, W, (hipStream_t)stream, dout_sc, dw_sc);

extern "C" int lad_conv_s2_wgrad_fused(const float *in, const float *dout, const float *dout_sc, float *workspace, float *dw,
                                       float *dbias, float *dw_sc, int64_t batch, int32_t H, int32_t W, int32_t cin, int32_t cout,
                                       void *stream) {
    using namespace lad;
    LAD_REQUIRE(in && dout && dout_sc && workspace && dw && dw_sc, "lad_conv_s2_wgrad_fused: null buffer");
    LAD_REQUIRE(batch >= 1 && H >= 1 && W >= 1, "lad_conv_s2_wgrad_fused: bad geometry");
    LAD_WG2F_CASE(64, 32)
    LAD_WG2F_CASE(32, 16)
    LAD_WG2F_CASE(16, 16)
    return fail(LAD_ERR_INVALID, "lad_conv_s2_wgrad_fused: unsupported (cin=%d, cout=%d)", cin, cout);
}

#define LAD_DGF_CASE(CI, CO)     \
    if (cin == CI && cout == CO) \
        return launch_dgrad<CO, CI, 9, true>(dout, wt, dx, batch, H, W, 0, (hipStream_t)stream, dout_sc, wt_sc);

extern "C" int lad_conv_s2_dgrad_fused(const float *dout, const float *wt, const float *dout_sc, const float *wt_sc, float *dx,
                                       int64_t batch, int32_t H, int32_t W, int32_t cin, int32_t cout, void *stream) {
    using namespace lad;
    LAD_REQUIRE(dout && wt && dout_sc && wt_sc && dx, "lad_conv_s2_dgrad_fused: null buffer");
    LAD_REQUIRE(batch >= 1 && H >= 1 && W >= 1, "lad_conv_s2_dgrad_fused: bad geometry");
    LAD_DGF_CASE(64, 32)
    LAD_DGF_CASE(32, 16)
    LAD_DGF_CASE(16, 16)
    return fail(LAD_ERR_INVALID, "lad_conv_s2_dgrad_fused: unsupported (cin=%d, cout=%d)", cin, cout);
}

extern "C" int64_t lad_conv_s2_dgrad_partials(int64_t batch, int32_t H, int32_t W) {
    if (batch < 1 || H < 1 || W < 1) return -1;
    return 4 * lad::ceil_div(batch * ((H + 1) / 2) * ((W + 1) / 2), TM);
}

extern "C" int lad_conv_s2_dgrad_fused_bnstat(const float *dout, const float *wt, const float *dout_sc, const float *wt_sc, float *dx,
                                              float *stat_partials, const float *bn_x, const uint64_t *bn_bits, const float *bn_coef,
                                              int64_t batch, int32_t H, int32_t W, int32_t cin, int32_t cout, void *stream) {
    using namespace lad;
    LAD_REQUIRE(dout && wt && dout_sc && wt_sc && dx && stat_partials && bn_x && bn_bits && bn_coef, "lad_conv_s2_dgrad_fused_bnstat: null buffer");
    LAD_REQUIRE(batch >= 1 && H >= 1 && W >= 1, "lad_conv_s2_dgrad_fused_bnstat: bad geometry");
    LAD_REQUIRE(cin == 64 && cout == 32, "lad_conv_s2_dgrad_fused_bnstat: the 64 <- 32 transition only (got cin=%d, cout=%d)", cin, cout);
    return launch_dgrad<32, 64, 9, true, true>(dout, wt, dx, batch, H, W, 0, (hipStream_t)stream, dout_sc, wt_sc,
                                               S2Stat{bn_x, (const unsigned long long *)bn_bits, bn_coef, stat_partials});
}
```

### laughter-detection-icsi_amd/csrc/lad_bn_math.h

```cpp
#pragma once
#include <hip/hip_runtime.h>

#include "lad_device.h"

namespace lad {

struct Norm4 {
    float4 mean, mean_lo, istd, istd_lo;
};
__device__ __forceinline__ Norm4 load_norm(const float *__restrict__ coef, int C, int c) {
    Norm4 n;
    n.mean = *reinterpret_cast<const float4 *>(coef + 2 * C + c);
    n.istd = *reinterpret_cast<const float4 *>(coef + 3 * C + c);
    n.mean_lo = *reinterpret_cast<const float4 *>(coef + 4 * C + c);
    n.istd_lo = *reinterpret_cast<const float4 *>(coef + 5 * C + c);
    return n;
}
__device__ __forceinline__ float xhat1(float x, float m, float ml, float s, float sl) {
    const float t = (x - m) - ml;
    return fmaf(t, s, t * sl);
}
__device__ __forceinline__ float4 xhat4(const float4 x, const Norm4 &n) {
    return make_float4(xhat1(x.x, n.mean.x, n.mean_lo.x, n.istd.x, n.istd_lo.x), xhat1(x.y, n.mean.y, n.mean_lo.y, n.istd.y, n.istd_lo.y),
                       xhat1(x.z, n.mean.z, n.mean_lo.z, n.istd.z, n.istd_lo.z), xhat1(x.w, n.mean.w, n.mean_lo.w, n.istd.w, n.istd_lo.w));
}
__device__ __forceinline__ float4 mask_from_x(float4 d, const float4 x, const float4 sc, const float4 sh) {
    d.x = fmaf(x.x, sc.x, sh.x) > 0.f ? d.x : 0.f;
    d.y = fmaf(x.y, sc.y, sh.y) > 0.f ? d.y : 0.f;
    d.z = fmaf(x.z, sc.z, sh.z) > 0.f ? d.z : 0.f;
    d.w = fmaf(x.w, sc.w, sh.w) > 0.f ? d.w : 0.f;
    return d;
}
__device__ __forceinline__ unsigned long long pack_sign_bits(const float4 o, int lane) {
    const unsigned long long bx = __ballot(o.x > 0.f), by = __ballot(o.y > 0.f), bz = __ballot(o.z > 0.f), bw = __ballot(o.w > 0.f);
    const int sh = lane & 48;
    return ((bx >> sh) & 0xFFFFull) | (((by >> sh) & 0xFFFFull) << 16) | (((bz >> sh) & 0xFFFFull) << 32) | (((bw >> sh) & 0xFFFFull) << 48);
}
__device__ __forceinline__ float4 mask_from_bits(float4 d, unsigned long long word, int j ) {
    const unsigned lo = (unsigned)word >> j, hi = (unsigned)(word >> 32) >> j;
    d.x = (lo & 1u) ? d.x : 0.f;
    d.y = (lo & 0x10000u) ? d.y : 0.f;
    d.z = (hi & 1u) ? d.z : 0.f;
    d.w = (hi & 0x10000u) ? d.w : 0.f;
    return d;
}
__device__ __forceinline__ u32x4 bn_relu_piece(u32x4 v, f32x4 scale, f32x4 shift, bool keep) {
    float4 f = as_f4(v);
    f.x = keep ? fmaxf(fmaf(f.x, scale.x, shift.x), 0.f) : 0.f;
    f.y = keep ? fmaxf(fmaf(f.y, scale.y, shift.y), 0.f) : 0.f;
    f.z = keep ? fmaxf(fmaf(f.z, scale.z, shift.z), 0.f) : 0.f;
    f.w = keep ? fmaxf(fmaf(f.w, scale.w, shift.w), 0.f) : 0.f;
    return as_u4(f);
}
__device__ __forceinline__ float bn_dx1(float d, float xh, float k1, float k2, float k2l, float k3, float k3l) {
    float t = (d - k2) - k2l;
    t = fmaf(-xh, k3, t);
    t = fmaf(-xh, k3l, t);
    return k1 * t;
}

}
```

### laughter-detection-icsi_amd/engine.py

```python
import ctypes
import math
import struct
from typing import FrozenSet, NamedTuple, Optional, Tuple

import torch

import _hip

_VP = ctypes.c_void_p


PREDICT_CHUNK = {"fp16": 8192, "fp32": 2048}
BASE_WIDTHS = (64, 32, 16, 16)
STREAM_SUPER_MAX = 1 << 20


class _LazyLevels(dict):

    def __init__(self, make):
        super().__init__()
        self._make = make

    def __missing__(self, key):
        value = self[key] = self._make(key)
        return value


def _align4(n):
    return (n + 3) & ~3


def _b3_shape(cin, cout, taps, stride):
    return cin == cout and cin in (64, 32) and taps == 9 and stride == 1


def _s2b3_shape(cin, cout, taps, stride):
    return cin == 64 and cout == 32 and taps == 9 and stride == 2


class _ConvParams:

    def __init__(self, name, cin, cout, taps, stride, base_widths, views, lib, dev):
        self.name, self.cin, self.cout, self.taps = name, cin, cout, taps
        self.w, self.gw = views[name + ".weight"]
        self.b, self.gb = views.get(name + ".bias", (None, None))
        self.shortcut = None

        def image(n, dtype):
            return torch.zeros(int(n), device=dev, dtype=dtype)

        self.wt_f = image(lib.lad_conv_packed_weight_floats(cout, cin, taps, 0), torch.float32)
        self.wt_d = image(lib.lad_conv_packed_weight_floats(cout, cin, taps, 1), torch.float32)
        self.wt_h = image(lib.lad_f16_packed_weight_halfs(cout, cin, taps), torch.float16)
        if _b3_shape(cin, cout, taps, stride) and base_widths:
            self.wt3_f, self.wt3_d = (image(lib.lad_conv_b3c_packed_weight_bytes(cin), torch.uint8) for _ in range(2))
            self.wt2_f, self.wt2_d = (image(lib.lad_conv_h2_packed_weight_bytes(cin), torch.uint8) for _ in range(2))
        if _s2b3_shape(cin, cout, taps, stride) and base_widths:
            self.wt3_s2f = image(lib.lad_conv_s2b3_packed_weight_bytes(), torch.uint8)
            self.wt3_s2d = image(lib.lad_conv_s2b3_dgrad_packed_weight_bytes(), torch.uint8)


class _BnParams:

    def __init__(self, name, c, views, bufs, dev, conv_bias=None):
        self.name, self.c, self.conv_bias = name, c, conv_bias
        self.g, self.gg = views[name + ".weight"]
        self.b, self.gb = views[name + ".bias"]
        self.rm, self.rv = bufs[name + ".running_mean"], bufs[name + ".running_var"]
        if not (self.rm.is_cuda and self.rm.is_contiguous() and self.rm.dtype == torch.float32):
            raise _hip.LadHipError(f"{name}: running statistics must be contiguous float32 GPU tensors")
        self.fold = (torch.zeros(c, device=dev), torch.zeros(c, device=dev))


class _ConvSpec:

    def __init__(self, name, cin, cout, taps, stride, h_in, w_in, base_widths=True):
        self.name, self.cin, self.cout, self.taps, self.stride = name, cin, cout, taps, stride
        self.h_in, self.w_in = h_in, w_in
        self.h_out = (h_in + stride - 1) // stride
        self.w_out = (w_in + stride - 1) // stride
        self.b3 = _b3_shape(cin, cout, taps, stride) and w_in <= 46 and base_widths
        self.b3_full = self.b3 and cin == 64
        self.b3_wgrad = self.b3 and (cin == 64 or w_in <= 30)
        self.s2b3 = _s2b3_shape(cin, cout, taps, stride) and (w_in + 1) // 2 <= 45 and base_widths
        self.par = None

    def rows(self, B):
        return B * (self.h_in + 1) * (self.w_in + 1) + self.w_in + 2


class _BlockSpec:

    def __init__(self, name):
        self.name = name
        self.conv1 = self.bn1 = self.conv2 = self.bn2 = self.sc_conv = self.sc_bn = None


def block_geometry(stem_cout, filter_sizes, H, W, base_widths):
    blocks = []
    cin, h, w = stem_cout, H, W
    for bi, cout in enumerate(filter_sizes, start=1):
        for j in range(2):
            name = f"block{bi}.{j}"
            stride = 2 if (j == 0 and bi > 1) else 1
            b = _BlockSpec(name)
            b.conv1 = _ConvSpec(name + ".conv1", cin, cout, 9, stride, h, w, base_widths)
            h, w = b.conv1.h_out, b.conv1.w_out
            b.conv2 = _ConvSpec(name + ".conv2", cout, cout, 9, 1, h, w, base_widths)
            if stride != 1 or cin != cout:
                b.sc_conv = _ConvSpec(name + ".shortcut.0", cin, cout, 1, stride, b.conv1.h_in, b.conv1.w_in, base_widths)
            blocks.append(b)
            cin = cout
    return blocks


class _ConvChoice(NamedTuple):
    arith: str
    wgrad: str
    wgrad_bn: bool
    label_fwd: str
    label_dgrad: str


class _BlockChoice(NamedTuple):
    entry: str
    a1_virtual: bool
    bits: bool
    dgrad2_bn: Optional[str]
    dgrad1_bn: Optional[str]
    sc_wgrad_fused: bool
    conv1: _ConvChoice
    conv2: _ConvChoice
    sc: Optional[_ConvChoice]


class _TrainSchedule(NamedTuple):
    blocks: Tuple[_BlockChoice, ...]
    stem_onepass: bool
    images: FrozenSet[Tuple[str, str]]
    opts: Tuple[Tuple[str, object], ...]


_ROW_LIMIT = (1 << 31) - (1 << 20)


def train_schedule(blocks, B, opts, stem_onepass):
    o = dict(opts)

    def arith(cs):
        fits = cs.rows(B) < _ROW_LIMIT if cs.cin == 64 else cs.rows(B) * cs.cin * 4 < _ROW_LIMIT
        if not (o["bf16x3"] and cs.b3 and (cs.cin == 64 or o["bf16x3_32"]) and fits):
            return "f32"
        return "h2" if o["f16x2"] and (cs.cin == 64 or o["f16x2_32"]) else "b3"

    def conv(cs, dgrad_f32=False, label_fwd=None):
        a = arith(cs)
        wg = "f32" if a == "f32" or not cs.b3_wgrad else "h2" if a == "h2" and cs.cin == 64 else "b3c"
        f32_label = f"conv_s{cs.stride}<{cs.cin},{cs.cout},{cs.taps}>"
        return _ConvChoice(a, wg, bool(o["fuse_bn_bwd_wgrad"]) and wg == "h2",
                           label_fwd or (f32_label if a == "f32" else f"conv_{a}<{cs.cin},{cs.cout},{cs.taps}>"),
                           f"conv_s1<{cs.cout},{cs.cin},{cs.taps}>" if a == "f32" or dgrad_f32 else f"conv_{a}<{cs.cout},{cs.cin},{cs.taps}>")

    out = []
    for bi, b in enumerate(blocks):
        c1, c2, sc = b.conv1, b.conv2, b.sc_conv
        a1, a2 = arith(c1), arith(c2)
        below_bits = bi > 0 and out[bi - 1].bits
        entry = "plain"
        if c1.stride != 1 and o["fuse_s2_shortcut"]:
            entry = "s2b3" if o["bf16x3"] and o["s2_b3"] and c1.s2b3 and c1.rows(B) < _ROW_LIMIT else "s2_fused"
        bits = bool(o["relu_bits"]) and sc is None and c1.b3_full and a1 != "f32" and not o["fuse_bn_bwd"]
        dgrad2_bn = "f32" if o["fuse_bn_bwd"] else "split" if o["fuse_bn_bwd_b3"] and a2 != "f32" else None
        if c1.stride != 1:
            fused = entry == "s2b3" or (entry == "s2_fused" and c1.cin == 64 and c1.cout == 32)
            dgrad1_bn = "split" if fused and o["fuse_bn_bwd_b3"] and below_bits else None
        elif bits:
            dgrad1_bn = "split" if o["fuse_bn_bwd_b3"] and below_bits else None
        else:
            dgrad1_bn = "f32" if o["fuse_bn_bwd"] and bi > 0 and blocks[bi - 1].sc_conv is None else None
        s2_label = f"conv_{'s2b3' if entry == 's2b3' else 's2'}<{c1.cin},{c1.cout},9>" if c1.stride != 1 else None
        out.append(_BlockChoice(entry, bool(o["virtual_a1"]) and a2 != "f32" and c2.b3_wgrad, bits, dgrad2_bn, dgrad1_bn,
                                c1.stride != 1 and bool(o["fuse_s2_shortcut_wgrad"]),
                                conv(c1, dgrad1_bn == "f32", s2_label), conv(c2, dgrad2_bn == "f32"), conv(sc) if sc is not None else None))
    images = {(ch.arith if ch.arith == "h2" else "b3c", cs.name) for b, blk in zip(blocks, out)
              for cs, ch in ((b.conv1, blk.conv1), (b.conv2, blk.conv2)) if ch.arith != "f32"}
    images |= {("s2b3", b.conv1.name) for b, blk in zip(blocks, out) if blk.entry == "s2b3"}
    return _TrainSchedule(tuple(out), bool(stem_onepass), frozenset(images), tuple(o.items()))


def conv_s1_entry(arith, cin, in_coef=False, gated=False, bn=None):
    if arith == "h2" and bn != "y":
        return "lad_conv_h2"
    if arith == "b3" and in_coef and not gated and bn is None:
        return "lad_conv_b3c_fwd_f32_bnrelu"
    if arith == "b3" and gated and not in_coef and cin == 64 and bn in (None, "bits"):
        return "lad_conv_b3_dgrad_bnstat" if bn else "lad_conv_b3_fwd_f32_gated"
    if arith == "b3" and not in_coef and not gated and bn in (None, "x"):
        return "lad_conv_b3c_dgrad_bnstat" if bn else "lad_conv_b3c_fwd_f32"
    if arith == "f32" and not in_coef and not gated and bn != "bits":
        return "lad_conv_fwd_bnstat" if bn else "lad_conv_fwd"
    raise _hip.LadHipError(f"no stride-1 convolution kernel for arithmetic {arith!r} at {cin} channels with in_coef={in_coef}, "
                           f"gated={gated}, bn={bn!r}")


def conv_wgrad_entry(kind, in_coef=False, bn=False):
    if kind == "h2":
        return "lad_conv_wgrad_h2_bnbwd" if bn else "lad_conv_wgrad_h2"
    if kind == "b3c" and not bn:
        return "lad_conv_wgrad_b3c"
    if kind == "f32" and not bn and not in_coef:
        return "lad_conv_wgrad"
    raise _hip.LadHipError(f"no weight-gradient kernel for {kind!r} with in_coef={in_coef}, bn={bn}")


def _s2_shortcut_rides(b, opts):
    return bool(opts["f16_s2_shortcut_fused"]) and b.conv1.cin != 32


def _block_fits_lds(b, B, opts, hw=None):
    c = b.conv1
    if b.sc_conv is not None or c.stride != 1 or c.taps != 9 or c.cin != c.cout:
        return False
    h, w = hw if hw is not None else (c.h_in, c.w_in)
    img = (h + 1) * (w + 1)
    if c.cin == 64:
        return bool(opts["strip_block_fused"]) and B >= 256 and img <= 512 and img + w <= 562
    return bool(opts["small_block_fused"]) and c.cin in (16, 32) and B >= 512 and img <= 2048


def _tail_blocks_ok(tail):
    if len(tail) != 4:
        return False
    for k, b in enumerate(tail):
        down = k % 2 == 0
        cin = 32 if k == 0 else 16
        if (b.conv1.cin, b.conv1.cout, b.conv1.taps, b.conv1.stride) != (cin, 16, 9, 2 if down else 1):
            return False
        if (b.conv2.cin, b.conv2.cout, b.conv2.taps, b.conv2.stride) != (16, 16, 9, 1):
            return False
        if down != (b.sc_conv is not None) or (down and (b.sc_conv.cin, b.sc_conv.cout, b.sc_conv.taps, b.sc_conv.stride) != (cin, 16, 1, 2)):
            return False
    return True


class _StreamLayout(NamedTuple):
    B: int
    H: int
    W: int
    half: bool
    mode: str
    run: Optional[Tuple[int, int]]
    n1: int
    band: int
    Ht: Optional[int]
    Hs: Optional[int]
    n_strip: Optional[int]
    n_strip_max: Optional[int]
    img_t_rows: Optional[int]
    stream_row0: Optional[int]
    cat_rows: Optional[int]
    k3: Optional[int]
    H2: Optional[int]
    W2: Optional[int]
    band2: Optional[int]
    Ht2: Optional[int]
    shift2: Optional[int]
    h2s: Optional[int]
    n_strip2: Optional[int]
    n_strip2_max: Optional[int]
    img_t2: Optional[int]
    img_s2: Optional[int]
    stream2_base: Optional[int]
    rows2: Optional[int]
    window_fused: Tuple[bool, ...]
    rides: Tuple[bool, ...]
# ... 48 lines not shown
    n_strip_max = n_strip if run is None else run[1] + H - Ht
    stream_row0 = cat_rows = None
    if direct:
        stream_row0 = n_strip_max * img_t_rows
        cat_rows = stream_row0 + (stream_rows + 1) * (W + 1) + W + 2 + (2 * (W + 1) if share2 else 0)
    strip_fused = tuple(bool(half) and _block_fits_lds(b, n_strip, o, (Ht, W)) for b in blocks[:n1])
    stream_fused = tuple(bool(half) and _block_fits_lds(b, 1, o, (stream_rows, W)) for b in blocks[:n1])
    stem_kept = bool(half and o["strip_stem_shared"])
    strip_stem_rows = stem_kept and Ht >= 3 and strip_fused[0] and blocks[0].conv1.cin == 64
    level1 = (n1, band, Ht, Hs, n_strip, n_strip_max, img_t_rows, stream_row0, cat_rows)
    if not share2:
        return _StreamLayout(B, H, W, bool(half), mode, None, *level1, *(None,) * 13, window_fused, rides, stream_fused, strip_fused,
                             stem_kept, strip_stem_rows, (), (), False, False)
    H2, W2 = nb.conv1.h_out, nb.conv1.w_out
    h2s = (stream_rows + 1) // 2
    n_strip2 = B + shift2
    n_strip2_max = n_strip2 if run is None else run[1] + shift2
    img_t2, img_s2 = (Ht2 + 1) * (W2 + 1), (h2s + 1) * (W2 + 1)
    stream2_base = n_strip2_max * img_t2
    rows2 = stream2_base + 2 * img_s2 + W2 + 2
    return _StreamLayout(B, H, W, True, mode, run, *level1, k3, H2, W2, band2, Ht2, shift2, h2s, n_strip2, n_strip2_max, img_t2, img_s2,
                         stream2_base, rows2, window_fused, rides, stream_fused, strip_fused, stem_kept, strip_stem_rows,
                         tuple(_block_fits_lds(b, 2, o, (h2s, W2)) for b in blocks[n1 + 1:k3]),
                         tuple(_block_fits_lds(b, n_strip2, o, (Ht2, W2)) for b in blocks[n1 + 1:k3]),
                         rides[n1] and bool(o["strip2_resident"]) and (nb.conv1.cin, nb.conv1.cout) == (64, 32),
                         bool(o["tail_fused"]) and _tail_blocks_ok(blocks[k3:]))


class _StreamRun:
    __slots__ = ("i0", "S", "B_max", "base", "frames_avail", "cat", "cat2", "stem")

    def __init__(self, i0, S, B_max, base, frames_avail):
        self.i0, self.S, self.B_max = i0, S, B_max
        self.base, self.frames_avail = base, frames_avail
        self.cat = self.cat2 = self.stem = None


class ResNetEngine:
    KERNEL_OPTIONS =("bf16x3", "bf16x3_32", "f16x2", "f16x2_32", "relu_bits", "virtual_a1", "fuse_bn_bwd", "fuse_bn_bwd_b3", "fuse_bn_bwd_wgrad", "fuse_s2_shortcut",
                      "fuse_s2_shortcut_wgrad", "s2_b3")
    INFER_OPTIONS = ("stream_direct", "stream_level2", "stream_super", "strip_block_fused", "small_block_fused", "tail_fused", "strip2_resident",
                     "strip_stem_shared", "f16_s2_shortcut_fused")

    def __init__(self, model):
        self.model = model
        self.device = None
        self._flat_p = self._flat_g = None
        self._plans = {}
        self._step_count = 0
        self._lib = None
        self._grad_dirty = False
        self._train_forwards = 0
        self._weights_version = 0
        self.fuse_bn_bwd = False
        self.overlap_wgrad = False
        self.overlap_wgrad_small = "auto"
        self.stem_onepass = True
        self.bf16x3 = True
        self.fuse_bn_bwd_b3 = True
        self.fuse_bn_bwd_wgrad = True
        self.f16x2 = True
        self.f16x2_32 = True
        self.bf16x3_32 = True
        self.virtual_a1 = True
        self.s2_b3 = True
        self.stream_direct = True
        self.stream_level2 = True
        self.strip_block_fused = True
        self.small_block_fused = True
        self.stream_super = True
        self.tail_fused = True
        self.strip2_resident = True
        self.strip_stem_shared = True
        self._sup_cache = {}
        self._sup_plans = {}
        self._layouts = {}
        self.f16_s2_shortcut_fused = True
        self.fuse_s2_shortcut = True
        self.fuse_s2_shortcut_wgrad = True
        self.defer_wgrad_sums = True
        self._defer_on = False
        self._schedules = {}
        self.relu_bits = True
        self._side = None
        self._side_readers = {}
        self._side_pending = False
        self.debug_capture = None
        self.kernel_events = None
        self.base_widths = list(model.filter_sizes) == list(BASE_WIDTHS)
        if not self.base_widths:
            for k in self.KERNEL_OPTIONS:
                setattr(self, k, False)

    def lib(self):
        if self._lib is None:
            self._lib = _hip.lib()
        return self._lib

    def _named_params(self):
        return list(self.model.named_parameters())

    def ensure_flat(self):
        params = self._named_params()
        dev = params[0][1].device
        if dev.type != "cuda":
            raise _hip.LadHipError("ResNetBigger runs on the MI355X only: call model.set_device('cuda') first "
                                   "(the HIP path has no CPU fallback)")
        ok = self._flat_p is not None and self._flat_p.device == dev
        if ok:
            base = self._flat_p.data_ptr()
            for (name, p), off in zip(params, self._offsets):
                if p.data_ptr() != base + 4 * off or p.dtype != torch.float32:
                    ok = False
                    break
        if ok:
            return
        offs, total = [], 0
        for _, p in params:
            offs.append(total)
            total += _align4(p.numel())
        flat_p = torch.zeros(total, device=dev, dtype=torch.float32)
        flat_g = torch.zeros(total, device=dev, dtype=torch.float32)
        with torch.no_grad():
            for (name, p), off in zip(params, offs):
                view = flat_p[off:off + p.numel()].view(p.shape)
                view.copy_(p.data.to(torch.float32))
                old_grad = p.grad
                p.data = view
                gview = flat_g[off:off + p.numel()].view(p.shape)
                if old_grad is not None:
                    gview.copy_(old_grad)
                    p.grad = gview
        self._flat_p, self._flat_g, self._offsets, self._n_flat = flat_p, flat_g, offs, total
        self._acc_g = None
        self._exp_avg = torch.zeros_like(flat_p)
        self._exp_avg_sq = torch.zeros_like(flat_p)
        self._norm_partials = torch.zeros(int(self.lib().lad_grad_sumsq_partials()), device=dev)
        self._norm_out = torch.zeros(1, device=dev)
        self._step_dev = torch.zeros(1, device=dev, dtype=torch.int64)
        self._rng_counter = torch.zeros(1, device=dev, dtype=torch.int64)
        self._rng_seed = None
        self.device = dev
        self._plans = {}
        self._views = {name: (flat_p[off:off + p.numel()].view(p.shape), flat_g[off:off + p.numel()].view(p.shape))
                       for (name, p), off in zip(params, offs)}
        bns = [m for m in self.model.modules() if isinstance(m, (torch.nn.BatchNorm1d, torch.nn.BatchNorm2d))]
        self._nbt = torch.zeros(len(bns), device=dev, dtype=torch.int64)
        with torch.no_grad():
            for i, m in enumerate(bns):
                self._nbt[i] = m.num_batches_tracked.to(dev)
                m._buffers["num_batches_tracked"] = self._nbt[i]
        self._build_specs()
        self._weights_version += 1
        self._param_list = [p for _, p in params]

    def bump_num_batches_tracked(self):
        self.ensure_flat()
        self._nbt.add_(1)

    def grad_views(self):
        return {k: v[1] for k, v in self._views.items()}

    def attach_grads(self):
        for name, p in self._named_params():
            g = self._views[name][1]
            if p.grad is None or p.grad.data_ptr() != g.data_ptr():
                p.grad = g

    def _build_specs(self):
        m = self.model
        bufs = dict(m.named_buffers())
        lib, dev = self.lib(), self.device

        def bn(name, c, conv_bias=None):
            return _BnParams(name, c, self._views, bufs, dev, conv_bias)
# ... 10 lines not shown
            if b.sc_conv is not None:
                self._convs[b.conv1.name].shortcut = self._convs[b.sc_conv.name]
        self._geom_specs = {}
        self._packed = None
        self._folded = None
        self._f16_packed = None
        self._pack_tables = {}
        self._tail_ptrs = None
        self.head_bn2 = bn("bn2", m.linear_layer_size)
        self.head_bn3 = bn("bn3", 32)
        names = ["bn2.weight", "bn2.bias", None, None, "linear1.weight", "linear1.bias", "bn3.weight", "bn3.bias",
                 None, None, "linear2.weight", "linear2.bias"]
        ptrs = []
        for i, n in enumerate(names):
            if n is not None:
                ptrs.append(self._views[n][0].data_ptr())
            else:
                t = {2: self.head_bn2.rm, 3: self.head_bn2.rv, 8: self.head_bn3.rm, 9: self.head_bn3.rv}[i]
                ptrs.append(t.data_ptr())
        self._head_params = (_VP * 12)(*ptrs)
        gnames = ["bn2.weight", "bn2.bias", "linear1.weight", "linear1.bias", "bn3.weight", "bn3.bias",
                  "linear2.weight", "linear2.bias"]
        self._head_grads = (_VP * 8)(*[self._views[n][1].data_ptr() for n in gnames])

    def _blocks_for(self, H, W, partial=False):
        key = (H, W, partial)
        if key in self._geom_specs:
            return self._geom_specs[key]
        blocks = block_geometry(self.stem_cout, self.model.filter_sizes, H, W, self.base_widths)
        for b in blocks:
            b.bn1, b.bn2 = self._bns[b.name + ".bn1"], self._bns[b.name + ".bn2"]
            b.conv1.par, b.conv2.par = self._convs[b.conv1.name], self._convs[b.conv2.name]
            if b.sc_conv is not None:
                b.sc_conv.par, b.sc_bn = self._convs[b.sc_conv.name], self._bns[b.name + ".shortcut.1"]
        h, w = blocks[-1].conv2.h_out, blocks[-1].conv2.w_out
        if partial:
            self._geom_specs[key] = (blocks, h, w, 0)
            return self._geom_specs[key]
        if h < 4 or w < 4:
            raise ValueError(f"input ({H},{W}) is too small: AvgPool2d(4) sees a {h}x{w} map")
        feat = blocks[-1].conv2.cout * (h // 4) * (w // 4)
        if feat != self.model.linear_layer_size:
            raise RuntimeError(f"running_mean should contain {feat} elements not {self.model.linear_layer_size}")
        self._geom_specs[key] = (blocks, h, w, feat)
        return self._geom_specs[key]

    def _plan(self, B, H, W, train):
        key = (B, H, W, train)
        p = self._plans.get(key)
        if p is not None:
            return p
        dev = self.device
        blocks, h4, w4, feat = self._blocks_for(H, W)
        lib = self.lib()

        def act(h, w, c):
            return torch.zeros(int(lib.lad_act_rows(B, h, w)) * c, device=dev, dtype=torch.float32)

        p = {"blocks": blocks, "h4": h4, "w4": w4, "feat": feat}
        c0 = self.stem_cout
        p["stem_a"] = act(H, W, c0)
        p["stem_coef"] = torch.zeros(6 * c0, device=dev)
        if train:
            p["stem_mom"] = torch.zeros(int(lib.lad_stem_moments_doubles()), device=dev, dtype=torch.float64)
            p["stem_mom_ws"] = torch.zeros(int(lib.lad_stem_moments_workspace_doubles()), device=dev, dtype=torch.float64)
            p["stem_bwd_ws"] = torch.zeros(int(lib.lad_stem_bwd_onepass_workspace_floats()), device=dev)
        max_tiles = int(lib.lad_conv_num_tiles(B, H, W))
        for b in blocks:
            if b.conv1.s2b3:
                max_tiles = max(max_tiles, int(lib.lad_conv_s2b3_dgrad_partials(B, b.conv1.h_in, b.conv1.w_in)))
        cmax = max([64] + [b.conv1.cout for b in blocks])
        p["partials"] = torch.zeros(max_tiles * 2 * cmax, device=dev)
        p["partials_sc"] = torch.zeros(max(int(lib.lad_conv_num_tiles(B, b.conv1.h_out, b.conv1.w_out)) * 2 * b.conv1.cout
                                           for b in blocks if b.sc_conv is not None) if any(b.sc_conv is not None for b in blocks) else 0,
                                       device=dev)
        acts = []
        for b in blocks:
            ho, wo, co = b.conv1.h_out, b.conv1.w_out, b.conv1.cout
            d = {"c1": act(ho, wo, co), "a1": act(ho, wo, co), "c2": act(ho, wo, co), "y": act(ho, wo, co),
                 "coef1": torch.zeros(6 * co, device=dev), "coef2": torch.zeros(6 * co, device=dev)}
            if b.sc_conv is not None:
                d["cs"] = act(ho, wo, co)
                d["coefs"] = torch.zeros(6 * co, device=dev)
            elif train and b.conv1.b3_full:
                d["ybits"] = torch.zeros(int(lib.lad_act_rows(B, ho, wo)), device=dev, dtype=torch.int64)
            acts.append(d)
        p["acts"] = acts
        p["pooled"] = torch.zeros(B * feat, device=dev)
        p["probs"] = torch.zeros(B, device=dev)
        if train:
            p["h"] = torch.zeros(B * 32, device=dev)
            p["hstats"] = torch.zeros(2 * feat + 64, device=dev)
            p["metrics"] = torch.zeros(8, device=dev)
            p["head_ws"] = torch.zeros(int(lib.lad_head_workspace_floats(B, feat)), device=dev)
            p["dpooled"] = torch.zeros(B * feat, device=dev)
            levels = {}
            for b, d in zip(blocks, acts):
                ho, wo, co = b.conv1.h_out, b.conv1.w_out, b.conv1.cout
                d["dc1"], d["dc2"] = act(ho, wo, co), act(ho, wo, co)
                if b.conv1.stride != 1:
                    d["aux"] = act(ho, wo, co)
            sizes = {(H, W): c0}
            for b in blocks:
                sizes[(b.conv1.h_out, b.conv1.w_out)] = max(sizes.get((b.conv1.h_out, b.conv1.w_out), 0), b.conv1.cout)
                sizes[(b.conv1.h_in, b.conv1.w_in)] = max(sizes.get((b.conv1.h_in, b.conv1.w_in), 0), b.conv1.cin,
                                                            b.conv1.cout)
            for (h, w), c in sizes.items():
                levels[(h, w)] = [act(h, w, c) for _ in range(4)]
            p["g"] = levels
            ws = max(max(int(lib.lad_conv_wgrad_workspace_floats(cs.cin, cs.cout, cs.taps)),
                         int(lib.lad_conv_s2_wgrad_fused_workspace_floats(cs.cin, cs.cout)) if cs.stride != 1 else 0)
                     for b in blocks for cs in (b.conv1, b.conv2, b.sc_conv) if cs is not None)
            ws = max(ws, int(lib.lad_stem_wgrad_workspace_floats()), int(lib.lad_conv_wgrad_b3c_workspace_floats(32)))
            p["wgrad_ws"] = torch.zeros(ws, device=dev)
            p["wgrad_ws_of"] = {}
            for b in blocks:
                for cs in (b.conv1, b.conv2, b.sc_conv):
                    if cs is not None:
                        n = int(lib.lad_conv_wgrad_workspace_floats(cs.cin, cs.cout, cs.taps))
                        if cs.b3_wgrad:
                            n = max(n, int(lib.lad_conv_wgrad_b3c_workspace_floats(cs.cin)))
                        if cs.stride != 1:
                            n = int(lib.lad_conv_s2_wgrad_fused_workspace_floats(cs.cin, cs.cout)) if cs.taps == 9 else \
                                int(lib.lad_conv_s2_wgrad_workspace_floats(cs.cin, cs.cout, cs.taps))
                        p["wgrad_ws_of"][cs.name] = torch.zeros(n, device=dev)
            p["bn_ws"] = torch.zeros(int(lib.lad_bn_bwd_workspace_floats(cmax)), device=dev)
            p["bcoef"] = torch.zeros(8 * cmax, device=dev)
        self._plans[key] = p
        return p

    def _st(self):
        return _hip.stream_handle(self.device)

    def notify_weights_changed(self):
        self._weights_version += 1

    def _weights_stamp(self):
        return (self._weights_version, sum(p._version for p in self._param_list))

    def _state_tag(self):
        bufs = sum(b._version for b in self.model.buffers())
        return self._weights_stamp() + (bufs, self._train_forwards)

    def _pack_weights(self, need_dgrad, sched=None):
        ver = self._weights_stamp()
        want = sched.images if sched is not None else frozenset()
        have = self._packed
        fresh = have is not None and have[0] == ver
        if fresh and have[1] >= need_dgrad and want <= have[2]:
            return
        lib, st = self.lib(), self._st()
        if not (fresh and have[1] >= need_dgrad):
            table = self._pack_tables.get(need_dgrad)
            if table is None:
                recs = [struct.pack("<QQiiii", par.w.data_ptr(), (par.wt_f if mode == 0 else par.wt_d).data_ptr(), par.cout, par.cin, par.taps, mode)
                        for par in self._convs.values() for mode in ((0, 1) if need_dgrad else (0,))]
                table = self._pack_tables[need_dgrad] = (torch.frombuffer(bytearray(b"".join(recs)), dtype=torch.uint8).to(self.device), len(recs))
            _hip.check(lib.lad_conv_pack_weights_multi(_hip.ptr(table[0]), table[1], st), "lad_conv_pack_weights_multi")
        h2 = []
        for kind, name in sorted(want - have[2] if fresh else want):
            par = self._convs[name]
            if kind == "s2b3":
                _hip.check(lib.lad_conv_s2b3_pack_weights_pair(_hip.ptr(par.w), _hip.ptr(par.shortcut.w), _hip.ptr(par.wt3_s2f),
                                                               _hip.ptr(par.wt3_s2d), st), "lad_conv_s2b3_pack_weights_pair")
            elif kind == "b3c":
                for mode, wt in ((0, par.wt3_f), (1, par.wt3_d)):
                    _hip.check(lib.lad_conv_b3c_pack_weights(_hip.ptr(par.w), mode, _hip.ptr(wt), par.cin, st), "lad_conv_b3c_pack_weights")
            else:
                h2.append(par)
        if h2:
            hkey = ("h2",) + tuple(par.name for par in h2)
            htab = self._pack_tables.get(hkey)
            if htab is None:
                recs = [struct.pack("<QQii", par.w.data_ptr(), wt.data_ptr(), mode, par.cin) for par in h2
                        for mode, wt in ((0, par.wt2_f), (1, par.wt2_d))]
                htab = self._pack_tables[hkey] = (torch.frombuffer(bytearray(b"".join(recs)), dtype=torch.uint8).to(self.device), len(recs))
            _hip.check(lib.lad_conv_h2_pack_weights_multi(_hip.ptr(htab[0]), htab[1], 0, st), "lad_conv_h2_pack_weights_multi")
        self._packed = (ver, need_dgrad or have[1], want | have[2]) if fresh else (ver, need_dgrad, want)

    def _eval_prepare(self, half):
        if not half:
            self._pack_weights(need_dgrad=False)
        tag = self._state_tag()
        lib, st = self.lib(), self._st()
        if self._folded != tag:
            for bn in (self.stem_bn, *self._bns.values()):
                _hip.check(lib.lad_bn_fold(_hip.ptr(bn.g), _hip.ptr(bn.b), _hip.ptr(bn.rm), _hip.ptr(bn.rv), _hip.ptr(bn.conv_bias),
                                           bn.c, _hip.ptr(bn.fold[0]), _hip.ptr(bn.fold[1]), st), "lad_bn_fold " + bn.name)
            self._folded = tag
        if half and self._f16_packed != tag:
            for par in self._convs.values():
                _hip.check(lib.lad_f16_pack_weights(_hip.ptr(par.w), par.cout, par.cin, par.taps, _hip.ptr(par.wt_h), st),
                           "lad_f16_pack_weights " + par.name)
            self._f16_packed = tag

    def _mark(self, label):
        if self.kernel_events is None or label not in self.kernel_events:
            return None
        ev = torch.cuda.Event(enable_timing=True)
        ev.record(torch.cuda.current_stream(self.device))
        return ev

    def _mark_end(self, label, start):
        if start is not None:
            ev = torch.cuda.Event(enable_timing=True)
            ev.record(torch.cuda.current_stream(self.device))
            self.kernel_events[label].append((start, ev))

    def _schedule(self, B, H, W):
        key = (B, H, W, self.stem_onepass) + tuple(getattr(self, k) for k in self.KERNEL_OPTIONS)
        sched = self._schedules.get(key)
        if sched is None:
            sched = self._schedules[key] = train_schedule(self._blocks_for(H, W)[0], B, {k: getattr(self, k) for k in self.KERNEL_OPTIONS},
                                                          self.stem_onepass)
        return sched

    def _conv_s1(self, cs, arith, direction, x, out, B, label=None, *, in_coef=None, bias=None, addend=None, abits=None, partials=None, bn=None):
        bx, bmask, bcoef = bn if bn is not None else (None, None, None)
        fn = conv_s1_entry(arith, cs.cin, in_coef is not None, abits is not None,
                           None if bn is None else "x" if bmask is None else "bits" if bmask.dtype == torch.int64 else "y")
        P, fwd, h, w = _hip.ptr, direction == "fwd", cs.h_in, cs.w_in
        wt = P(getattr(cs.par, {"h2": "wt2_", "b3": "wt3_", "f32": "wt_"}[arith] + ("f" if fwd else "d")))
        cio = (cs.cin, cs.cout) if fwd else (cs.cout, cs.cin)
        if fn == "lad_conv_h2":
            args = (P(x), P(in_coef), wt, P(bias), P(addend), P(abits), P(out), P(partials), P(bx), P(bmask), P(bcoef), B, h, w, cs.cin)
        elif fn == "lad_conv_b3c_fwd_f32":
            args = (P(x), wt, P(bias), P(addend), P(out), P(partials), B, h, w, cs.cin)
        elif fn == "lad_conv_b3c_fwd_f32_bnrelu":
            args = (P(x), P(in_coef), wt, P(bias), P(out), P(partials), B, h, w, cs.cin)
        elif fn == "lad_conv_b3c_dgrad_bnstat":
            args = (P(x), wt, P(addend), P(out), P(partials), P(bx), P(bcoef), B, h, w, cs.cin)
        elif fn == "lad_conv_b3_fwd_f32_gated":
            args = (P(x), wt, P(bias), P(addend), P(abits), P(out), P(partials), B, h, w)
        elif fn == "lad_conv_b3_dgrad_bnstat":
            args = (P(x), wt, P(addend), P(abits), P(out), P(partials), P(bx), P(bmask), P(bcoef), B, h, w)
        elif fn == "lad_conv_fwd":
            args = (P(x), wt, P(bias), P(addend), P(out), P(partials), B, h, w, *cio, cs.taps)
        else:
            args = (P(x), wt, P(addend), P(out), P(partials), P(bx), P(bmask), P(bcoef), B, h, w, *cio, cs.taps)
        t0 = self._mark(label)
        _hip.check(getattr(self.lib(), fn)(*args, self._st()), f"{fn}({direction}) {cs.name}")
        self._mark_end(label, t0)

    def _conv_fwd(self, cs, ch, x, out, partials, B, in_coef=None):
        if cs.stride == 1:
            self._conv_s1(cs, ch.arith, "fwd", x, out, B, ch.label_fwd, in_coef=in_coef, bias=cs.par.b, partials=partials)
            return
        t0 = self._mark(ch.label_fwd)
        _hip.check(self.lib().lad_conv_s2_fwd(_hip.ptr(x), _hip.ptr(cs.par.wt_f), _hip.ptr(cs.par.b), _hip.ptr(out), _hip.ptr(partials),
                                              B, cs.h_in, cs.w_in, cs.cin, cs.cout, cs.taps, self._st()), "lad_conv_s2_fwd " + cs.name)
        self._mark_end(ch.label_fwd, t0)

    def _bn_coef(self, bn, coef, partials, B, h, w):
        lib, st = self.lib(), self._st()
        n_tiles = int(lib.lad_conv_num_tiles(B, h, w))
        _hip.check(lib.lad_bn_finalize(_hip.ptr(partials), n_tiles, bn.c, B * h * w, _hip.ptr(bn.g), _hip.ptr(bn.b),
                                       _hip.ptr(bn.rm), _hip.ptr(bn.rv), 0.1, _hip.ptr(coef), st),
                   "lad_bn_finalize " + bn.name)

    def _bn_coef_pair(self, bn_a, coef_a, part_a, bn_b, coef_b, part_b, B, h, w):
        lib, st = self.lib(), self._st()
        n_tiles = int(lib.lad_conv_num_tiles(B, h, w))
        _hip.check(lib.lad_bn_finalize_pair(_hip.ptr(part_a), _hip.ptr(part_b), n_tiles, bn_a.c, B * h * w,
                                            _hip.ptr(bn_a.g), _hip.ptr(bn_a.b), _hip.ptr(bn_a.rm), _hip.ptr(bn_a.rv), _hip.ptr(coef_a),
                                            _hip.ptr(bn_b.g), _hip.ptr(bn_b.b), _hip.ptr(bn_b.rm), _hip.ptr(bn_b.rv), _hip.ptr(coef_b),
                                            0.1, st), "lad_bn_finalize_pair " + bn_a.name)

    def _bn_act(self, x, coef, res, rcoef, y, B, h, w, c, relu=1):
        _hip.check(self.lib().lad_bn_act(_hip.ptr(x), _hip.ptr(coef), _hip.ptr(res), _hip.ptr(rcoef), _hip.ptr(y), B, h, w, c,
                                         relu, self._st()), "lad_bn_act")

    def forward(self, x, train, labels=None, drop_masks=None):
        self.ensure_flat()
        _hip.require_cuda(x, "x", torch.float32)
        if x.dim() == 4:
            if x.shape[1] != 1:
                raise ValueError("ResNetBigger expects a single input channel: (B,1,T,F)")
            B, _, H, W = x.shape
        elif x.dim() == 3:
            B, H, W = x.shape
        else:
            raise ValueError("x must be (B,1,T,F) or (B,T,F)")
        if B == 0:
            return torch.zeros(0, device=x.device)
        if not train:
            return self._forward_eval(x.view(-1), B, H, W, frame_stride=H, frames_avail=B * H)
        if B < 2:
            raise ValueError("Expected more than 1 value per channel when training, got input size "
                             f"torch.Size([{B}, {self.model.linear_layer_size}])")
        lib, st = self.lib(), self._st()
        p = self._plan(B, H, W, True)
        blocks = p["blocks"]
        sched = p["schedule"] = self._schedule(B, H, W)
        self._pack_weights(need_dgrad=True, sched=sched)
        part = p["partials"]
        if sched.stem_onepass:
            bn = self.stem_bn
            _hip.check(lib.lad_stem_bn_stats(_hip.ptr(x), _hip.ptr(self.stem_w), _hip.ptr(bn.g), _hip.ptr(bn.b), _hip.ptr(bn.rm), _hip.ptr(bn.rv),
                                             0.1, _hip.ptr(p["stem_coef"]), _hip.ptr(p["stem_mom"]), _hip.ptr(p["stem_mom_ws"]), B, H, W,
                                             self.stem_cout, st), "lad_stem_bn_stats")
        else:
            _hip.check(lib.lad_stem_fwd(_hip.ptr(x), _hip.ptr(self.stem_w), None, _hip.ptr(part), B, H, W, self.stem_cout, st),
                       "lad_stem_fwd")
            self._bn_coef(self.stem_bn, p["stem_coef"], part, B, H, W)
        c0 = self.stem_cout
        scale, shift = p["stem_coef"][:c0], p["stem_coef"][c0:2 * c0]
        _hip.check(lib.lad_stem_fwd_eval(_hip.ptr(x), _hip.ptr(self.stem_w), _hip.ptr(scale), _hip.ptr(shift), _hip.ptr(p["stem_a"]),
                                         B, H, W, c0, H, B * H, st), "lad_stem_fwd_eval (train)")
        cur = p["stem_a"]
        for b, ch, a in zip(blocks, sched.blocks, p["acts"]):
            ho, wo, co = b.conv1.h_out, b.conv1.w_out, b.conv1.cout
            if ch.entry == "plain":
                self._conv_fwd(b.conv1, ch.conv1, cur, a["c1"], part, B)
                self._bn_coef(b.bn1, a["coef1"], part, B, ho, wo)
            else:
                t0 = self._mark(ch.conv1.label_fwd)
                if ch.entry == "s2b3":
                    _hip.check(lib.lad_conv_s2b3_fwd(_hip.ptr(cur), _hip.ptr(b.conv1.par.wt3_s2f), _hip.ptr(b.conv1.par.b), _hip.ptr(a["c1"]), _hip.ptr(part),
                                                     _hip.ptr(a["cs"]), _hip.ptr(p["partials_sc"]), B, b.conv1.h_in, b.conv1.w_in, st),
                               "lad_conv_s2b3_fwd " + b.conv1.name)
                else:
                    _hip.check(lib.lad_conv_s2_fwd_fused(_hip.ptr(cur), _hip.ptr(b.conv1.par.wt_f), _hip.ptr(b.conv1.par.b), _hip.ptr(b.sc_conv.par.wt_f),
                                                         _hip.ptr(a["c1"]), _hip.ptr(part), _hip.ptr(a["cs"]), _hip.ptr(p["partials_sc"]),
                                                         B, b.conv1.h_in, b.conv1.w_in, b.conv1.cin, b.conv1.cout, st),
                               "lad_conv_s2_fwd_fused " + b.conv1.name)
                self._mark_end(ch.conv1.label_fwd, t0)
                self._bn_coef_pair(b.bn1, a["coef1"], part, b.sc_bn, a["coefs"], p["partials_sc"], B, ho, wo)
            if ch.a1_virtual:
                self._conv_fwd(b.conv2, ch.conv2, a["c1"], a["c2"], part, B, in_coef=a["coef1"])
            else:
                self._bn_act(a["c1"], a["coef1"], None, None, a["a1"], B, ho, wo, co)
                self._conv_fwd(b.conv2, ch.conv2, a["a1"], a["c2"], part, B)
            self._bn_coef(b.bn2, a["coef2"], part, B, ho, wo)
            if b.sc_conv is not None:
                if ch.entry == "plain":
                    self._conv_fwd(b.sc_conv, ch.sc, cur, a["cs"], part, B)
                    self._bn_coef(b.sc_bn, a["coefs"], part, B, ho, wo)
                self._bn_act(a["c2"], a["coef2"], a["cs"], a["coefs"], a["y"], B, ho, wo, co)
            elif ch.bits:
                _hip.check(lib.lad_bn_act_bits(_hip.ptr(a["c2"]), _hip.ptr(a["coef2"]), _hip.ptr(cur), None, _hip.ptr(a["y"]),
                                               _hip.ptr(a["ybits"]), B, ho, wo, co, st), "lad_bn_act_bits")
            else:
                self._bn_act(a["c2"], a["coef2"], cur, None, a["y"], B, ho, wo, co)
            a["x"] = cur
            cur = a["y"]
        last = blocks[-1].conv2
        _hip.check(lib.lad_pool_fwd(_hip.ptr(cur), _hip.ptr(p["pooled"]), B, p["h4"], p["w4"], last.cout, st), "lad_pool_fwd")
        m1 = m2 = None
        rng = isinstance(drop_masks, str) and drop_masks == "rng"
        if drop_masks is not None and not rng:
            m1, m2 = drop_masks
            _hip.require_cuda(m1, "drop mask 1", torch.float32)
            _hip.require_cuda(m2, "drop mask 2", torch.float32)
            if tuple(m1.shape) != (B, p["feat"]) or tuple(m2.shape) != (B, 32):
                raise ValueError("dropout masks must be (B,linear_layer_size) and (B,32)")
        if labels is not None:
            _hip.require_cuda(labels, "labels", torch.int32)
            if labels.numel() != B:
                raise ValueError("labels must have one entry per sample")
        if rng:
            keep = 1.0 - float(self.model.dropout.p)
            if keep < 1.0:
                if "m1" not in p:
                    p["m1"] = torch.zeros((B, p["feat"]), device=self.device)
                    p["m2"] = torch.zeros((B, 32), device=self.device)
                m1, m2 = p["m1"], p["m2"]
            seed = int(torch.cuda.default_generators[self.device.index or 0].initial_seed()) & ((1 << 64) - 1)
            if seed != self._rng_seed:
                self._rng_seed = seed
                self._rng_counter.zero_()
            _hip.check(lib.lad_head_fwd_train_rng(self._head_params, _hip.ptr(p["pooled"]), B, p["feat"], _hip.ptr(m1), _hip.ptr(m2), keep,
                                                  seed, _hip.ptr(self._rng_counter), _hip.ptr(self._nbt), int(self._nbt.numel()),
                                                  _hip.ptr(labels), 0.1, _hip.ptr(p["h"]), _hip.ptr(p["hstats"]), _hip.ptr(p["probs"]),
                                                  _hip.ptr(p["metrics"]), st), "lad_head_fwd_train_rng")
        else:
            _hip.check(lib.lad_head_fwd_train(self._head_params, _hip.ptr(p["pooled"]), B, p["feat"], _hip.ptr(m1), _hip.ptr(m2),
                                              _hip.ptr(labels), 0.1, _hip.ptr(p["h"]), _hip.ptr(p["hstats"]),
                                              _hip.ptr(p["probs"]), _hip.ptr(p["metrics"]), st), "lad_head_fwd_train")
        p["saved"] = (x, labels, m1, m2, B, H, W)
        self._last_train_plan = p
        self._train_forwards += 1
        return p["probs"]

    def _plan_eval(self, B, H, W, dtype=torch.float32, partial=False, owner=None):
        key = (B, H, W, "eval", dtype) + (("partial",) if partial else ())
        if owner is not None and key not in self._sup_plans.setdefault(owner, []):
            self._sup_plans[owner].append(key)
        p = self._plans.get(key)
        if p is not None:
            return p
        dev = self.device
        blocks, h4, w4, feat = self._blocks_for(H, W, partial)
        p = {"blocks": blocks, "h4": h4, "w4": w4, "feat": feat}
        levels = {(H, W): self.stem_cout}
        for b in blocks:
            k = (b.conv1.h_out, b.conv1.w_out)
            levels[k] = max(levels.get(k, 0), b.conv1.cout)
        rows_of = lambda k: int(self.lib().lad_act_rows(B, k[0], k[1]))
        p["lv"] = _LazyLevels(lambda k: [torch.zeros(rows_of(k) * levels[k], device=dev, dtype=dtype) for _ in range(4)])
        p["pooled"] = torch.zeros(B * feat, device=dev)
        p["probs"] = torch.zeros(B, device=dev)
        self._plans[key] = p
        return p

    def _conv_eval(self, cs, bn, x, addend, out, B, relu):
        lib, st = self.lib(), self._st()
        label = f"conv_s{cs.stride}<{cs.cin},{cs.cout},{cs.taps}>"
        t0 = self._mark(label)
        if cs.stride == 1:
            _hip.check(lib.lad_conv_fwd_eval(_hip.ptr(x), _hip.ptr(cs.par.wt_f), _hip.ptr(bn.fold[0]), _hip.ptr(bn.fold[1]),
                                             _hip.ptr(addend), _hip.ptr(out), B, cs.h_in, cs.w_in, cs.cin, cs.cout, cs.taps, relu, st),
                       "lad_conv_fwd_eval " + cs.name)
        else:
            if addend is not None:
                raise _hip.LadHipError("stride-2 eval convolution takes no residual")
            _hip.check(lib.lad_conv_s2_fwd_eval(_hip.ptr(x), _hip.ptr(cs.par.wt_f), _hip.ptr(bn.fold[0]), _hip.ptr(bn.fold[1]),
                                                _hip.ptr(out), B, cs.h_in, cs.w_in, cs.cin, cs.cout, cs.taps, relu, st),
                       "lad_conv_s2_fwd_eval " + cs.name)
        self._mark_end(label, t0)

    def _conv_eval_f16(self, cs, bn, x, addend, out, B, relu):
# ... 463 lines not shown
        if self._defer_on:
            _hip.check(lib.lad_wgrad_defer_begin(), "lad_wgrad_defer_begin")
        _hip.check(lib.lad_head_bwd(self._head_params, self._head_grads, _hip.ptr(p["pooled"]), _hip.ptr(p["h"]),
                                    _hip.ptr(p["hstats"]), _hip.ptr(p["probs"]), _hip.ptr(dprobs), B, p["feat"], _hip.ptr(m1),
                                    _hip.ptr(m2), _hip.ptr(labels), _hip.ptr(p["head_ws"]), _hip.ptr(p["dpooled"]), st),
                   "lad_head_bwd")
        g_out = p["g"][(last.h_out, last.w_out)]
        dy = g_out[0]
        _hip.check(lib.lad_pool_bwd(_hip.ptr(p["dpooled"]), _hip.ptr(dy), B, p["h4"], p["w4"], last.cout, st), "lad_pool_bwd")
        pre2 = False
        pre2_tiles = 0
        for bi in range(len(blocks) - 1, -1, -1):
            b, a, ch = blocks[bi], acts[bi], sched.blocks[bi]
            c1s, c2s = b.conv1, b.conv2
            ho, wo, co = c1s.h_out, c1s.w_out, c1s.cout
            hi, wi = c1s.h_in, c1s.w_in
            G = p["g"][(ho, wo)]
            free = [t for t in G if t is not dy]
            aux, da1 = (self._w(a["aux"]) if "aux" in a else free[0]), free[1]
            dc2, dc1 = self._w(a["dc2"]), self._w(a["dc1"])
            bits = a["ybits"] if ch.bits else None
            lower = acts[bi - 1]
            fuse2 = ch.bits and ch.conv2.wgrad_bn and not self.overlap_wgrad
            fuse1 = ch.conv1.wgrad_bn and not self.overlap_wgrad
            if ch.bits:
                _hip.check(lib.lad_bn_bwd_bits(_hip.ptr(dy), _hip.ptr(bits), _hip.ptr(a["c2"]), _hip.ptr(a["coef2"]), _hip.ptr(b.bn2.g),
                                               None if fuse2 else _hip.ptr(dc2), _hip.ptr(b.bn2.gg), _hip.ptr(b.bn2.gb), _hip.ptr(p["bn_ws"]),
                                               _hip.ptr(p["bcoef"]), _hip.ptr(p["partials"]) if pre2 else None,
                                               (pre2_tiles or int(lib.lad_conv_num_tiles(B, ho, wo))) if pre2 else 0, B, ho, wo, co, st),
                           "lad_bn_bwd_bits " + b.bn2.name)
            elif b.sc_conv is None:
                self._bn_bwd(p, b.bn2, dy, a["y"], a["c2"], a["coef2"], dc2, B, ho, wo, 1, mode=1, aux=aux, pre=pre2)
            else:
                self._bn_bwd(p, b.bn2, dy, a["y"], a["c2"], a["coef2"], dc2, B, ho, wo, 1, mode=2, aux=aux,
                             sbn=b.sc_bn, xs=a["cs"], scoef=a["coefs"])
            xin, xcoef = (a["c1"], a["coef1"]) if ch.a1_virtual else (a["a1"], None)
            self._conv_wgrad(p, c2s, ch.conv2.wgrad, xin, dc2, B, in_coef=xcoef, bn=(dy, a["c2"], bits, a["coef2"]) if fuse2 else None)
            stat = (a["c1"], None, a["coef1"]) if ch.dgrad2_bn else None
            self._conv_s1(c2s, "f32" if ch.dgrad2_bn == "f32" else ch.conv2.arith, "dgrad", dc2, da1, B, ch.conv2.label_dgrad,
                          bn=stat, partials=p["partials"] if stat else None)
            self._bn_bwd(p, b.bn1, da1, None, a["c1"], a["coef1"], None if fuse1 else dc1, B, ho, wo, 2, mode=0, pre=stat is not None)
            if c1s.stride == 1:
                self._conv_wgrad(p, c1s, ch.conv1.wgrad, a["x"], dc1, B, bn=(da1, a["c1"], None, a["coef1"]) if fuse1 else None)
            if self.debug_capture is not None:
                self.debug_capture[b.name] = {"dy": dy.clone(), "dc2": dc2.clone(), "aux": aux.clone() if bits is None else None, "da1": da1.clone(),
                                              "dc1": dc1.clone()}
            if c1s.stride == 1:
                dx = dy
                if b.sc_conv is not None:
                    self._conv_wgrad(p, b.sc_conv, ch.sc.wgrad, a["x"], aux, B)
                    self._conv_s1(b.sc_conv, ch.sc.arith, "dgrad", aux, da1, B)
                    aux = da1
                stat = (lower["c2"], lower["ybits" if ch.dgrad1_bn == "split" else "y"], lower["coef2"]) if ch.dgrad1_bn else None
                self._conv_s1(c1s, "f32" if ch.dgrad1_bn == "f32" else ch.conv1.arith, "dgrad", dc1, dx, B, ch.conv1.label_dgrad,
                              addend=dy if ch.bits else aux, abits=bits, bn=stat, partials=p["partials"] if stat else None)
                pre2, pre2_tiles = stat is not None, 0
            else:
                dx = p["g"][(hi, wi)][0]
                sc = b.sc_conv

                def s2_wgrad(cs, dout, xin=a["x"]):
                    self._on_side(lambda sst: _hip.check(lib.lad_conv_s2_wgrad(
                        _hip.ptr(xin), _hip.ptr(dout), _hip.ptr(self._wg_ws(p, cs)), _hip.ptr(cs.par.gw), _hip.ptr(cs.par.gb), B, hi, wi, cs.cin, cs.cout,
                        cs.taps, sst), "lad_conv_s2_wgrad " + cs.name), dout, small=cs.cin <= 32)

                if ch.sc_wgrad_fused:
                    self._on_side(lambda sst, c1s=c1s, sc=sc, dc1=dc1, aux=aux, xin=a["x"]: _hip.check(lib.lad_conv_s2_wgrad_fused(
                        _hip.ptr(xin), _hip.ptr(dc1), _hip.ptr(aux), _hip.ptr(self._wg_ws(p, c1s)), _hip.ptr(c1s.par.gw), _hip.ptr(c1s.par.gb),
                        _hip.ptr(sc.par.gw), B, hi, wi, c1s.cin, c1s.cout, sst), "lad_conv_s2_wgrad_fused " + c1s.name), dc1, small=c1s.cin <= 32)
                    if dc1.data_ptr() in self._side_readers:
                        self._side_readers[aux.data_ptr()] = self._side_readers[dc1.data_ptr()]
                else:
                    s2_wgrad(c1s, dc1)
                stat = (lower["c2"], lower["ybits"], lower["coef2"]) if ch.dgrad1_bn else (None, None, None)
                n_part = 0
                if ch.entry == "s2b3":
                    n_part = int(lib.lad_conv_s2b3_dgrad_partials(B, hi, wi))
                    assert not ch.dgrad1_bn or n_part * 2 * 64 <= p["partials"].numel()
                    _hip.check(lib.lad_conv_s2b3_dgrad(_hip.ptr(dc1), _hip.ptr(aux), _hip.ptr(c1s.par.wt3_s2d), _hip.ptr(dx),
                                                       _hip.ptr(p["partials"]) if ch.dgrad1_bn else None, _hip.ptr(stat[0]), _hip.ptr(stat[1]),
                                                       _hip.ptr(stat[2]), B, hi, wi, st), "lad_conv_s2b3_dgrad " + c1s.name)
                elif ch.entry == "s2_fused" and ch.dgrad1_bn:
                    n_part = int(lib.lad_conv_s2_dgrad_partials(B, hi, wi))
                    assert n_part * 2 * 64 <= p["partials"].numel()
                    _hip.check(lib.lad_conv_s2_dgrad_fused_bnstat(_hip.ptr(dc1), _hip.ptr(c1s.par.wt_d), _hip.ptr(aux), _hip.ptr(sc.par.wt_d), _hip.ptr(dx),
                                                                  _hip.ptr(p["partials"]), _hip.ptr(stat[0]), _hip.ptr(stat[1]),
                                                                  _hip.ptr(stat[2]), B, hi, wi, c1s.cin, c1s.cout, st),
                               "lad_conv_s2_dgrad_fused_bnstat " + c1s.name)
                elif ch.entry == "s2_fused":
                    _hip.check(lib.lad_conv_s2_dgrad_fused(_hip.ptr(dc1), _hip.ptr(c1s.par.wt_d), _hip.ptr(aux), _hip.ptr(sc.par.wt_d), _hip.ptr(dx),
                                                           B, hi, wi, c1s.cin, c1s.cout, st), "lad_conv_s2_dgrad_fused " + c1s.name)
                else:
                    _hip.check(lib.lad_conv_s2_dgrad(_hip.ptr(dc1), _hip.ptr(c1s.par.wt_d), _hip.ptr(dx), B, hi, wi, c1s.cin, c1s.cout, 9, 0,
                                                     st), "lad_conv_s2_dgrad " + c1s.name)
                pre2, pre2_tiles = ch.dgrad1_bn is not None, n_part
                if not ch.sc_wgrad_fused:
                    s2_wgrad(sc, aux)
                if ch.entry == "plain":
                    _hip.check(lib.lad_conv_s2_dgrad(_hip.ptr(aux), _hip.ptr(sc.par.wt_d), _hip.ptr(dx), B, hi, wi, sc.cin, sc.cout, 1, 1, st),
                               "lad_conv_s2_dgrad " + sc.name)
            dy = dx
        if sched.stem_onepass:
            bn = self.stem_bn
            _hip.check(lib.lad_stem_bwd_onepass(_hip.ptr(x), _hip.ptr(self.stem_w), _hip.ptr(dy), _hip.ptr(p["stem_coef"]), _hip.ptr(bn.g),
                                                _hip.ptr(p["stem_mom"]), _hip.ptr(p["stem_bwd_ws"]), _hip.ptr(self.stem_gw), _hip.ptr(bn.gg),
                                                _hip.ptr(bn.gb), B, H, W, self.stem_cout, st), "lad_stem_bwd_onepass")
        else:
            groups = int(lib.lad_stem_bn_bwd_groups(B, H, W))
            _hip.check(lib.lad_stem_bn_bwd_sums(_hip.ptr(x), _hip.ptr(self.stem_w), _hip.ptr(dy), _hip.ptr(p["stem_coef"]),
                                                _hip.ptr(p["partials"]), B, H, W, self.stem_cout, st), "lad_stem_bn_bwd_sums")
            bn = self.stem_bn
            _hip.check(lib.lad_bn_bwd(_hip.ptr(dy), None, None, _hip.ptr(p["stem_coef"]), _hip.ptr(bn.g), None, None, None, None,
                                      None, _hip.ptr(bn.gg), _hip.ptr(bn.gb), None, None, _hip.ptr(p["bn_ws"]), _hip.ptr(p["bcoef"]),
                                      _hip.ptr(p["partials"]), groups, B, H, W, bn.c, 2, 0, st), "lad_bn_bwd " + bn.name)
            self._on_side(lambda sst: _hip.check(lib.lad_stem_wgrad_bn(_hip.ptr(x), _hip.ptr(dy), None, _hip.ptr(self.stem_w),
                                                                       _hip.ptr(p["stem_coef"]), _hip.ptr(p["bcoef"]),
                                                                       _hip.ptr(p["wgrad_ws"]), _hip.ptr(self.stem_gw), B, H, W,
                                                                       self.stem_cout, sst), "lad_stem_wgrad_bn"), dy)
        if self._defer_on:
            self._defer_on = False
            self._join_side()
            _hip.check(lib.lad_wgrad_defer_flush(st), "lad_wgrad_defer_flush")
        self._join_side()
        self._grad_dirty = True

    def export_relu_masks(self):
        p = getattr(self, "_last_train_plan", None)
        if p is None or "saved" not in p:
            raise _hip.LadHipError("export_relu_masks() without a preceding train-mode forward()")
        x, labels, m1, m2, B, H, W = p["saved"]

        def unpack(buf, h, w, c):
            body = buf[:B * (h + 1) * (w + 1) * c].view(B, h + 1, w + 1, c)[:, 1:, 1:, :]
            return (body > 0).permute(0, 3, 1, 2).cpu()

        out = {"stem": unpack(p["stem_a"], H, W, self.stem_cout)}
        for b, ch, a in zip(p["blocks"], p["schedule"].blocks, p["acts"]):
            ho, wo, co = b.conv1.h_out, b.conv1.w_out, b.conv1.cout
            if ch.a1_virtual:
                c = a["c1"][:B * (ho + 1) * (wo + 1) * co].view(B, ho + 1, wo + 1, co)[:, 1:, 1:, :].double()
                sc, sh = a["coef1"][:co].double(), a["coef1"][co:2 * co].double()
                out[b.name + ".a1"] = (c * sc + sh > 0).permute(0, 3, 1, 2).cpu()
            else:
                out[b.name + ".a1"] = unpack(a["a1"], ho, wo, co)
            out[b.name + ".y"] = unpack(a["y"], ho, wo, co)
        h = p["h"].view(B, 32).double()
        mean, var = h.mean(0), h.var(0, unbiased=False)
        u = (h - mean) / torch.sqrt(var + 1e-5) * self.head_bn3.g.double() + self.head_bn3.b.double()
        if m2 is not None:
            u = u * m2.double()
        out["head"] = (u > 0).cpu()
        return out

    def reset_optimizer(self):
        self.ensure_flat()
        self._exp_avg.zero_()
        self._exp_avg_sq.zero_()
        self._step_dev.zero_()
        self._step_count = 0

    def reset_dropout_rng(self):
        self.ensure_flat()
        self._rng_counter.zero_()

    def flat_grad(self):
        self.ensure_flat()
        return self._flat_g

    def flat_param(self):
        self.ensure_flat()
        return self._flat_p
# ... 65 lines not shown
```

Before: 49850 segments/s.

## Extend fused BatchNorm-backward and ReLU sign bits to 32- and 16-channel blocks

Adds 32-channel variants of the sign-bit BN activation, the h2 convolution with bit-gated addends, and the fused stride-2 dgrad with BN statistics. The training schedule can now keep ReLU sign bits for 32-channel blocks and fold BN backward sums into dgrad for 32->16 stride-2 and 16x16 f32 convolutions. The goal is to cut separate BN-backward reduction passes and full activation reads in the smaller blocks. It adds new kernel instantiations and schedule options, enabled by default through an environment variable.

```diff
diff --git a/include/lad_hip.h b/include/lad_hip.h
--- a/include/lad_hip.h
+++ b/include/lad_hip.h
@@ -126,6 +126,9 @@
 int lad_conv_s2_dgrad_fused_bnstat(const float *dout, const float *wt, const float *dout_sc, const float *wt_sc, float *dx,
                                    float *stat_partials, const float *bn_x, const uint64_t *bn_bits, const float *bn_coef,
                                    int64_t batch, int32_t H, int32_t W, int32_t cin, int32_t cout, void *stream);
+int lad_conv_s2_dgrad_fused_bnstat32(const float *dout, const float *wt, const float *dout_sc, const float *wt_sc, float *dx,
+                                      float *stat_partials, const float *bn_x, const uint64_t *bn_bits, const float *bn_coef,
+                                      int64_t batch, int32_t H, int32_t W, void *stream);
 int64_t lad_conv_wgrad_workspace_floats(int32_t cin, int32_t cout, int32_t taps);
 int lad_conv_wgrad(const float *in, const float *dout, float *workspace, float *dw, float *dbias, int64_t batch,
                    int32_t H, int32_t W, int32_t cin, int32_t cout, int32_t taps, void *stream);
@@ -159,6 +162,9 @@
 int lad_conv_h2(const float *in, const float *in_coef, const void *wt, const float *bias, const float *addend,
                 const uint64_t *addend_bits, float *out, float *partials, const float *bn_x, const uint64_t *bn_bits,
                 const float *bn_coef, int64_t batch, int32_t H, int32_t W, int32_t channels, void *stream);
+int lad_conv_h2_bits32(const float *in, const float *in_coef, const void *wt, const float *bias, const float *addend,
+                       const uint64_t *addend_bits, float *out, float *partials, const float *bn_x, const uint64_t *bn_bits,
+                       const float *bn_coef, int64_t batch, int32_t H, int32_t W, void *stream);
 int64_t lad_conv_wgrad_b3c_workspace_floats(int32_t channels);
 int lad_conv_wgrad_b3c(const float *in, const float *in_coef, const float *dout, float *workspace, float *dw, float *dbias,
                        int64_t batch, int32_t H, int32_t W, int32_t channels, void *stream);
@@ -210,6 +216,8 @@
                float *dbeta, float *dsgamma, float *dsbeta, float *workspace, float *bcoef, float *pre_partials,
                int64_t pre_tiles, int64_t batch, int32_t H, int32_t W, int32_t channels, int32_t relu, int32_t mode,
                void *stream);
+int lad_bn_act_bits32(const float *x, const float *coef, const float *res, const float *res_coef, float *y,
+                      uint64_t *y_bits, int64_t batch, int32_t H, int32_t W, void *stream);
 int lad_bn_act_bits(const float *x, const float *coef, const float *res, const float *res_coef, float *y,
                     uint64_t *y_bits, int64_t batch, int32_t H, int32_t W, int32_t channels, void *stream);
 int lad_bn_bwd_bits(const float *dy, const uint64_t *y_bits, const float *x, const float *coef, const float *gamma,
diff --git a/laughter-detection-icsi_amd/_hip.py b/laughter-detection-icsi_amd/_hip.py
--- a/laughter-detection-icsi_amd/_hip.py
+++ b/laughter-detection-icsi_amd/_hip.py
@@ -66,6 +66,7 @@
     "lad_conv_h2_pack_weights_multi": (c_int, [c_void_p, c_i32, c_i32, c_void_p]),
     "lad_conv_wgrad_h2": (c_int, [c_void_p] * 6 + [c_i64, c_i32, c_i32, c_i32, c_void_p]),
     "lad_conv_h2": (c_int, [c_void_p] * 11 + [c_i64, c_i32, c_i32, c_i32, c_void_p]),
+    "lad_conv_h2_bits32": (c_int, [c_void_p] * 11 + [c_i64, c_i32, c_i32, c_void_p]),
     "lad_conv_wgrad_h2_bnbwd": (c_int, [c_void_p] * 11 + [c_i64, c_i32, c_i32, c_i32, c_void_p]),
     "lad_conv_wgrad_b3c_workspace_floats": (c_i64, [c_i32]),
     "lad_conv_wgrad_b3c": (c_int, [c_void_p] * 6 + [c_i64, c_i32, c_i32, c_i32, c_void_p]),
@@ -94,6 +95,7 @@
     "lad_conv_s2b3_dgrad_partials": (c_i64, [c_i64, c_i32, c_i32]),
     "lad_conv_s2b3_dgrad": (c_int, [c_void_p] * 8 + [c_i64, c_i32, c_i32, c_void_p]),
     "lad_conv_s2_dgrad_fused_bnstat": (c_int, [c_void_p] * 9 + [c_i64, c_i32, c_i32, c_i32, c_i32, c_void_p]),
+    "lad_conv_s2_dgrad_fused_bnstat32": (c_int, [c_void_p] * 9 + [c_i64, c_i32, c_i32, c_void_p]),
     "lad_conv_s2_dgrad_fused": (c_int, [c_void_p] * 5 + [c_i64, c_i32, c_i32, c_i32, c_i32, c_void_p]),
     "lad_conv_s2_wgrad_fused_workspace_floats": (c_i64, [c_i32, c_i32]),
     "lad_conv_s2_wgrad_fused": (c_int, [c_void_p] * 7 + [c_i64, c_i32, c_i32, c_i32, c_i32, c_void_p]),
@@ -118,6 +120,7 @@
     "lad_bn_act": (c_int, [c_void_p] * 5 + [c_i64, c_i32, c_i32, c_i32, c_i32, c_void_p]),
     "lad_bn_bwd_workspace_floats": (c_i64, [c_i32]),
     "lad_bn_act_bits": (c_int, [c_void_p] * 6 + [c_i64, c_i32, c_i32, c_i32, c_void_p]),
+    "lad_bn_act_bits32": (c_int, [c_void_p] * 6 + [c_i64, c_i32, c_i32, c_void_p]),
     "lad_bn_bwd_bits": (c_int, [c_void_p] * 11 + [c_i64, c_i64, c_i32, c_i32, c_i32, c_void_p]),
     "lad_bn_bwd": (c_int, [c_void_p] * 17 + [c_i64, c_i64, c_i32, c_i32, c_i32, c_i32, c_i32, c_void_p]),
     "lad_conv_fwd_bnstat": (c_int, [c_void_p] * 8 + [c_i64, c_i32, c_i32, c_i32, c_i32, c_i32, c_void_p]),
diff --git a/laughter-detection-icsi_amd/csrc/bn.hip b/laughter-detection-icsi_amd/csrc/bn.hip
--- a/laughter-detection-icsi_amd/csrc/bn.hip
+++ b/laughter-detection-icsi_amd/csrc/bn.hip
@@ -215,7 +215,7 @@
     return p;
 }
 
-template <int RES, bool BITS = false>
+template <int RES, int BITS = 0>
 __global__ void bn_act_kernel(const float4 *__restrict__ x, const float *__restrict__ coef,
                               const float4 *__restrict__ res, const float *__restrict__ rcoef, float4 *__restrict__ y,
                               RowGeom g, int C, int c4shift, int relu, unsigned long long *__restrict__ bits = nullptr) {
@@ -254,8 +254,9 @@
             }
             y[idx] = o;
             if (BITS) {
-                const unsigned long long word = pack_sign_bits(o, threadIdx.x & 63);
-                if ((threadIdx.x & 15) == 0) bits[idx >> 4] = word;
+                constexpr int LPR = BITS ? BITS : 16;
+                const unsigned long long word = pack_sign_bits<LPR>(o, threadIdx.x & 63);
+                if ((threadIdx.x & (LPR - 1)) == 0) bits[idx >> (LPR == 16 ? 4 : 3)] = word;
             }
         }
     }
@@ -422,7 +423,7 @@
             } else if (relu == 2) {
                 d = mask_from_x(d, xv, fsc, fsh);
             } else if (relu == 3) {
-                d = mask_from_bits(d, bits[idx >> 4], threadIdx.x & 15);
+                d = mask_from_bits(d, bits[idx >> c4shift], c >> 2);
             }
             const float4 xh = xhat4(xv, nm);
             float4 o;
@@ -533,7 +534,7 @@
     LAD_REQUIRE(channels >= 4 && channels <= 4 * THREADS && (channels & (channels - 1)) == 0, "%s: channels must be a power of two in 4..1024", who);
     LAD_REQUIRE(res != nullptr || res_coef == nullptr, "%s: res_coef without res", who);
     LAD_REQUIRE(batch >= 0 && H >= 1 && W >= 1, "%s: bad geometry", who);
-    LAD_REQUIRE(bits == nullptr || channels == 64, "%s: sign bits are kept for 64-channel activations only", who);
+    LAD_REQUIRE(bits == nullptr || channels == 64 || channels == 32, "%s: sign bits are kept for 64- and 32-channel activations only", who);
     if (batch == 0) return LAD_OK;
     const RowGeom g = make_row_geom(batch, H, W);
     const int sh = log2_exact(channels / 4);
@@ -541,11 +542,14 @@
     hipStream_t st = (hipStream_t)stream;
 #define LAD_ACT(RES, R, RC)                                                                                                   \
     do {                                                                                                                      \
-        if (bits)                                                                                                             \
-            hipLaunchKernelGGL((bn_act_kernel<RES, true>), grid, block, 0, st, (const float4 *)x, coef, (const float4 *)(R), RC, \
+        if (bits && channels == 64)                                                                                           \
+            hipLaunchKernelGGL((bn_act_kernel<RES, 16>), grid, block, 0, st, (const float4 *)x, coef, (const float4 *)(R), RC, \
+                               (float4 *)y, g, channels, sh, relu, bits);                                                     \
+        else if (bits)                                                                                                        \
+            hipLaunchKernelGGL((bn_act_kernel<RES, 8>), grid, block, 0, st, (const float4 *)x, coef, (const float4 *)(R), RC, \
                                (float4 *)y, g, channels, sh, relu, bits);                                                     \
         else                                                                                                                  \
-            hipLaunchKernelGGL((bn_act_kernel<RES, false>), grid, block, 0, st, (const float4 *)x, coef, (const float4 *)(R), RC, \
+            hipLaunchKernelGGL((bn_act_kernel<RES, 0>), grid, block, 0, st, (const float4 *)x, coef, (const float4 *)(R), RC, \
                                (float4 *)y, g, channels, sh, relu, nullptr);                                                  \
     } while (0)
     if (res == nullptr)
@@ -568,7 +572,15 @@
                                uint64_t *y_bits, int64_t batch, int32_t H, int32_t W, int32_t channels, void *stream) {
     using namespace lad;
     LAD_REQUIRE(y_bits, "lad_bn_act_bits: null sign-bit buffer");
+    LAD_REQUIRE(channels == 64, "lad_bn_act_bits: sign bits are kept for 64-channel activations only (32 channels: lad_bn_act_bits32)");
     return bn_act_impl(x, coef, res, res_coef, y, (unsigned long long *)y_bits, batch, H, W, channels, 1, stream, "lad_bn_act_bits");
+}
+
+extern "C" int lad_bn_act_bits32(const float *x, const float *coef, const float *res, const float *res_coef, float *y,
+                                 uint64_t *y_bits, int64_t batch, int32_t H, int32_t W, void *stream) {
+    using namespace lad;
+    LAD_REQUIRE(y_bits, "lad_bn_act_bits32: null sign-bit buffer");
+    return bn_act_impl(x, coef, res, res_coef, y, (unsigned long long *)y_bits, batch, H, W, 32, 1, stream, "lad_bn_act_bits32");
 }
 
 extern "C" int64_t lad_bn_bwd_workspace_floats(int32_t channels) { return (int64_t)BWD_GROUPS * 3 * channels; }
@@ -580,7 +592,7 @@
                 float *pre_partials, int64_t pre_tiles, int64_t batch, int32_t H, int32_t W, int32_t channels,
                 int32_t relu, int32_t mode, void *stream) {
     using namespace lad;
-    LAD_REQUIRE(relu != 3 || (bits && channels == 64), "lad_bn_bwd_bits: sign bits are kept for 64-channel activations only");
+    LAD_REQUIRE(relu != 3 || (bits && (channels == 64 || channels == 32)), "lad_bn_bwd_bits: sign bits are kept for 64- and 32-channel activations only");
     LAD_REQUIRE(dy && coef && gamma && dgamma && dbeta && workspace && bcoef, "lad_bn_bwd: null buffer");
     LAD_REQUIRE(x || (pre_partials && !dx), "lad_bn_bwd: x may only be omitted when the sums are given and nothing is applied");
     LAD_REQUIRE(dx || mode == 0, "lad_bn_bwd: dx may only be omitted (sums and coefficients only) in mode 0");
diff --git a/laughter-detection-icsi_amd/csrc/conv_h2.hip b/laughter-detection-icsi_amd/csrc/conv_h2.hip
--- a/laughter-detection-icsi_amd/csrc/conv_h2.hip
+++ b/laughter-detection-icsi_amd/csrc/conv_h2.hip
@@ -401,6 +401,31 @@
     if (ceil_div(g.rows, TM * 2) < h2_two_rounds()) return launch_h2_rb<C, 1, STAT, INBN>(a);
     return launch_h2_rb<C, 2, STAT, INBN>(a);
 }
+
+int conv_h2_entry(const char *who, const float *in, const float *in_coef, const void *wt, const float *bias, const float *addend,
+                  const uint64_t *addend_bits, float *out, float *partials, const float *bn_x, const uint64_t *bn_bits,
+                  const float *bn_coef, int64_t batch, int32_t H, int32_t W, int32_t channels, void *stream) {
+    LAD_REQUIRE(batch >= 1 && H >= 1 && W >= 1, "%s: bad geometry", who);
+    LAD_REQUIRE(in && wt && out, "%s: null buffer", who);
+    LAD_REQUIRE(addend_bits == nullptr || addend != nullptr, "%s: sign bits without an addend", who);
+    LAD_REQUIRE((const void *)in != (const void *)out, "%s: the convolution cannot run in place", who);
+    const bool stat = bn_x != nullptr;
+    LAD_REQUIRE(!stat || (partials && bn_coef), "%s: the BatchNorm sums need partials and bn_coef", who);
+    LAD_REQUIRE(stat || bn_bits == nullptr, "%s: bn_bits without bn_x", who);
+    LAD_REQUIRE(!(stat && in_coef), "%s: an input BatchNorm and the backward sums are not combined", who);
+    const B3Stat bst{bn_x, (const unsigned long long *)bn_bits, bn_coef};
+    if (channels == 64) {
+        if (stat) return launch_h2<64, true, false>(in, nullptr, wt, bias, addend, addend_bits, out, partials, bst, batch, H, W, stream, who);
+        if (in_coef) return launch_h2<64, false, true>(in, in_coef, wt, bias, addend, addend_bits, out, partials, bst, batch, H, W, stream, who);
+        return launch_h2<64, false, false>(in, nullptr, wt, bias, addend, addend_bits, out, partials, bst, batch, H, W, stream, who);
+    }
+    if (channels == 32) {
+        if (stat) return launch_h2<32, true, false>(in, nullptr, wt, bias, addend, addend_bits, out, partials, bst, batch, H, W, stream, who);
+        if (in_coef) return launch_h2<32, false, true>(in, in_coef, wt, bias, addend, addend_bits, out, partials, bst, batch, H, W, stream, who);
+        return launch_h2<32, false, false>(in, nullptr, wt, bias, addend, addend_bits, out, partials, bst, batch, H, W, stream, who);
+    }
+    return fail(LAD_ERR_INVALID, "%s: 64 or 32 channels (got %d)", who, channels);
+}
 }
 
 extern "C" int64_t lad_conv_h2_packed_weight_bytes(int32_t channels) {
@@ -424,28 +449,15 @@
                            const uint64_t *addend_bits, float *out, float *partials, const float *bn_x, const uint64_t *bn_bits,
                            const float *bn_coef, int64_t batch, int32_t H, int32_t W, int32_t channels, void *stream) {
     using namespace lad;
-    const char *who = "lad_conv_h2";
-    LAD_REQUIRE(batch >= 1 && H >= 1 && W >= 1, "%s: bad geometry", who);
-    LAD_REQUIRE(in && wt && out, "%s: null buffer", who);
-    LAD_REQUIRE(addend_bits == nullptr || addend != nullptr, "%s: sign bits without an addend", who);
-    LAD_REQUIRE((const void *)in != (const void *)out, "%s: the convolution cannot run in place", who);
-    const bool stat = bn_x != nullptr;
-    LAD_REQUIRE(!stat || (partials && bn_coef), "%s: the BatchNorm sums need partials and bn_coef", who);
-    LAD_REQUIRE(stat || bn_bits == nullptr, "%s: bn_bits without bn_x", who);
-    LAD_REQUIRE(!(stat && in_coef), "%s: an input BatchNorm and the backward sums are not combined", who);
-    LAD_REQUIRE(channels == 64 || (addend_bits == nullptr && bn_bits == nullptr), "%s: sign bits are kept for 64-channel activations only", who);
-    const B3Stat bst{bn_x, (const unsigned long long *)bn_bits, bn_coef};
-    if (channels == 64) {
-        if (stat) return launch_h2<64, true, false>(in, nullptr, wt, bias, addend, addend_bits, out, partials, bst, batch, H, W, stream, who);
-        if (in_coef) return launch_h2<64, false, true>(in, in_coef, wt, bias, addend, addend_bits, out, partials, bst, batch, H, W, stream, who);
-        return launch_h2<64, false, false>(in, nullptr, wt, bias, addend, addend_bits, out, partials, bst, batch, H, W, stream, who);
-    }
-    if (channels == 32) {
-        if (stat) return launch_h2<32, true, false>(in, nullptr, wt, bias, addend, addend_bits, out, partials, bst, batch, H, W, stream, who);
-        if (in_coef) return launch_h2<32, false, true>(in, in_coef, wt, bias, addend, addend_bits, out, partials, bst, batch, H, W, stream, who);
-        return launch_h2<32, false, false>(in, nullptr, wt, bias, addend, addend_bits, out, partials, bst, batch, H, W, stream, who);
-    }
-    return fail(LAD_ERR_INVALID, "%s: 64 or 32 channels (got %d)", who, channels);
+    LAD_REQUIRE(channels == 64 || (addend_bits == nullptr && bn_bits == nullptr),
+                "lad_conv_h2: sign bits are kept for 64-channel activations only (32 channels: lad_conv_h2_bits32)");
+    return conv_h2_entry("lad_conv_h2", in, in_coef, wt, bias, addend, addend_bits, out, partials, bn_x, bn_bits, bn_coef, batch, H, W, channels, stream);
+}
+
+extern "C" int lad_conv_h2_bits32(const float *in, const float *in_coef, const void *wt, const float *bias, const float *addend,
+                                  const uint64_t *addend_bits, float *out, float *partials, const float *bn_x, const uint64_t *bn_bits,
+                                  const float *bn_coef, int64_t batch, int32_t H, int32_t W, void *stream) {
+    return conv_h2_entry("lad_conv_h2_bits32", in, in_coef, wt, bias, addend, addend_bits, out, partials, bn_x, bn_bits, bn_coef, batch, H, W, 32, stream);
 }
 
 #ifdef LAD_STAMP
diff --git a/laughter-detection-icsi_amd/csrc/conv_s2_bwd.hip b/laughter-detection-icsi_amd/csrc/conv_s2_bwd.hip
--- a/laughter-detection-icsi_amd/csrc/conv_s2_bwd.hip
+++ b/laughter-detection-icsi_amd/csrc/conv_s2_bwd.hip
@@ -52,7 +52,7 @@
                                                               const float *__restrict__ wt_sc = nullptr,
                                                               S2Stat bst = S2Stat{nullptr, nullptr, nullptr, nullptr}) {
     static_assert(!SC || TAPS == 9, "the shortcut rides with the 3x3 convolution");
-    static_assert(!STAT || (SC && NC == 64), "the fused sums are written for the 64-channel transition with the shortcut fused");
+    static_assert(!STAT || (SC && (NC == 64 || NC == 32)), "the fused sums need the shortcut fused and sign bits (64 or 32 channels)");
     constexpr int NT = NTl<NC>::NT;
     constexpr int NP = NTl<NC>::NP;
     constexpr int K4 = KC / 4;
@@ -496,3 +496,13 @@
     return launch_dgrad<32, 64, 9, true, true>(dout, wt, dx, batch, H, W, 0, (hipStream_t)stream, dout_sc, wt_sc,
                                                S2Stat{bn_x, (const unsigned long long *)bn_bits, bn_coef, stat_partials});
 }
+
+extern "C" int lad_conv_s2_dgrad_fused_bnstat32(const float *dout, const float *wt, const float *dout_sc, const float *wt_sc, float *dx,
+                                                 float *stat_partials, const float *bn_x, const uint64_t *bn_bits, const float *bn_coef,
+                                                 int64_t batch, int32_t H, int32_t W, void *stream) {
+    using namespace lad;
+    LAD_REQUIRE(dout && wt && dout_sc && wt_sc && dx && stat_partials && bn_x && bn_bits && bn_coef, "lad_conv_s2_dgrad_fused_bnstat32: null buffer");
+    LAD_REQUIRE(batch >= 1 && H >= 1 && W >= 1, "lad_conv_s2_dgrad_fused_bnstat32: bad geometry");
+    return launch_dgrad<16, 32, 9, true, true>(dout, wt, dx, batch, H, W, 0, (hipStream_t)stream, dout_sc, wt_sc,
+                                               S2Stat{bn_x, (const unsigned long long *)bn_bits, bn_coef, stat_partials});
+}
diff --git a/laughter-detection-icsi_amd/csrc/lad_bn_math.h b/laughter-detection-icsi_amd/csrc/lad_bn_math.h
--- a/laughter-detection-icsi_amd/csrc/lad_bn_math.h
+++ b/laughter-detection-icsi_amd/csrc/lad_bn_math.h
@@ -31,10 +31,13 @@
     d.w = fmaf(x.w, sc.w, sh.w) > 0.f ? d.w : 0.f;
     return d;
 }
+template <int LPR = 16>
 __device__ __forceinline__ unsigned long long pack_sign_bits(const float4 o, int lane) {
+    static_assert(LPR == 16 || LPR == 8, "64 or 32 channels");
+    constexpr unsigned long long FIELD = (1ull << LPR) - 1ull;
     const unsigned long long bx = __ballot(o.x > 0.f), by = __ballot(o.y > 0.f), bz = __ballot(o.z > 0.f), bw = __ballot(o.w > 0.f);
-    const int sh = lane & 48;
-    return ((bx >> sh) & 0xFFFFull) | (((by >> sh) & 0xFFFFull) << 16) | (((bz >> sh) & 0xFFFFull) << 32) | (((bw >> sh) & 0xFFFFull) << 48);
+    const int sh = lane & (64 - LPR);
+    return ((bx >> sh) & FIELD) | (((by >> sh) & FIELD) << 16) | (((bz >> sh) & FIELD) << 32) | (((bw >> sh) & FIELD) << 48);
 }
 __device__ __forceinline__ float4 mask_from_bits(float4 d, unsigned long long word, int j ) {
     const unsigned lo = (unsigned)word >> j, hi = (unsigned)(word >> 32) >> j;
diff --git a/laughter-detection-icsi_amd/engine.py b/laughter-detection-icsi_amd/engine.py
--- a/laughter-detection-icsi_amd/engine.py
+++ b/laughter-detection-icsi_amd/engine.py
@@ -1,5 +1,6 @@
 import ctypes
 import math
+import os
 import struct
 from typing import FrozenSet, NamedTuple, Optional, Tuple
 
@@ -139,13 +140,32 @@
     stem_onepass: bool
     images: FrozenSet[Tuple[str, str]]
     opts: Tuple[Tuple[str, object], ...]
+    small: Tuple[str, ...] = ()
 
 
 _ROW_LIMIT = (1 << 31) - (1 << 20)
+
+SMALL_BN_PARTS = ("bits32", "s2stat32", "f32x16")
+
+
+def small_bn_parts(value):
+    if isinstance(value, str):
+        v = value.strip().lower()
+        if v in ("", "0", "off", "false", "none"):
+            return ()
+        if v in ("1", "on", "true", "all"):
+            return SMALL_BN_PARTS
+        parts = tuple(x.strip() for x in v.split(","))
+        bad = [x for x in parts if x not in SMALL_BN_PARTS]
+        if bad:
+            raise ValueError(f"fuse_bn_bwd_small: unknown part(s) {bad}; known: {SMALL_BN_PARTS}")
+        return tuple(x for x in SMALL_BN_PARTS if x in parts)
+    return SMALL_BN_PARTS if value else ()
 
 
 def train_schedule(blocks, B, opts, stem_onepass):
     o = dict(opts)
+    small = small_bn_parts(o.pop("fuse_bn_bwd_small", False))
 
     def arith(cs):
         fits = cs.rows(B) < _ROW_LIMIT if cs.cin == 64 else cs.rows(B) * cs.cin * 4 < _ROW_LIMIT
@@ -169,10 +189,14 @@
         entry = "plain"
         if c1.stride != 1 and o["fuse_s2_shortcut"]:
             entry = "s2b3" if o["bf16x3"] and o["s2_b3"] and c1.s2b3 and c1.rows(B) < _ROW_LIMIT else "s2_fused"
-        bits = bool(o["relu_bits"]) and sc is None and c1.b3_full and a1 != "f32" and not o["fuse_bn_bwd"]
+        has_bits = c1.b3_full or ("bits32" in small and c1.b3 and c1.cin == 32 and a1 == "h2")
+        bits = bool(o["relu_bits"]) and sc is None and has_bits and a1 != "f32" and not o["fuse_bn_bwd"]
         dgrad2_bn = "f32" if o["fuse_bn_bwd"] else "split" if o["fuse_bn_bwd_b3"] and a2 != "f32" else None
+        if dgrad2_bn is None and "f32x16" in small and a2 == "f32" and (c2.cin, c2.cout, c2.taps, c2.stride) == (16, 16, 9, 1):
+            dgrad2_bn = "f32"
         if c1.stride != 1:
-            fused = entry == "s2b3" or (entry == "s2_fused" and c1.cin == 64 and c1.cout == 32)
+            fused = entry == "s2b3" or (entry == "s2_fused" and ((c1.cin, c1.cout) == (64, 32) or
+                                                                 ("s2stat32" in small and (c1.cin, c1.cout) == (32, 16))))
             dgrad1_bn = "split" if fused and o["fuse_bn_bwd_b3"] and below_bits else None
         elif bits:
             dgrad1_bn = "split" if o["fuse_bn_bwd_b3"] and below_bits else None
@@ -185,12 +209,12 @@
     images = {(ch.arith if ch.arith == "h2" else "b3c", cs.name) for b, blk in zip(blocks, out)
               for cs, ch in ((b.conv1, blk.conv1), (b.conv2, blk.conv2)) if ch.arith != "f32"}
     images |= {("s2b3", b.conv1.name) for b, blk in zip(blocks, out) if blk.entry == "s2b3"}
-    return _TrainSchedule(tuple(out), bool(stem_onepass), frozenset(images), tuple(o.items()))
+    return _TrainSchedule(tuple(out), bool(stem_onepass), frozenset(images), tuple(o.items()), small)
 
 
 def conv_s1_entry(arith, cin, in_coef=False, gated=False, bn=None):
     if arith == "h2" and bn != "y":
-        return "lad_conv_h2"
+        return "lad_conv_h2_bits32" if cin == 32 and (gated or bn == "bits") else "lad_conv_h2"
     if arith == "b3" and in_coef and not gated and bn is None:
         return "lad_conv_b3c_fwd_f32_bnrelu"
     if arith == "b3" and gated and not in_coef and cin == 64 and bn in (None, "bits"):
@@ -405,6 +429,7 @@
         self._defer_on = False
         self._schedules = {}
         self.relu_bits = True
+        self.fuse_bn_bwd_small = os.environ.get("LAD_FUSE_BN_BWD_SMALL", True)
         self._side = None
         self._side_readers = {}
         self._side_pending = False
@@ -414,6 +439,7 @@
         if not self.base_widths:
             for k in self.KERNEL_OPTIONS:
                 setattr(self, k, False)
+            self.fuse_bn_bwd_small = False
 
     def lib(self):
         if self._lib is None:
@@ -590,7 +616,7 @@
             if b.sc_conv is not None:
                 d["cs"] = act(ho, wo, co)
                 d["coefs"] = torch.zeros(6 * co, device=dev)
-            elif train and b.conv1.b3_full:
+            elif train and b.conv1.b3:
                 d["ybits"] = torch.zeros(int(lib.lad_act_rows(B, ho, wo)), device=dev, dtype=torch.int64)
             acts.append(d)
         p["acts"] = acts
@@ -716,11 +742,12 @@
             self.kernel_events[label].append((start, ev))
 
     def _schedule(self, B, H, W):
-        key = (B, H, W, self.stem_onepass) + tuple(getattr(self, k) for k in self.KERNEL_OPTIONS)
+        key = (B, H, W, self.stem_onepass, small_bn_parts(self.fuse_bn_bwd_small)) + tuple(getattr(self, k) for k in self.KERNEL_OPTIONS)
         sched = self._schedules.get(key)
         if sched is None:
-            sched = self._schedules[key] = train_schedule(self._blocks_for(H, W)[0], B, {k: getattr(self, k) for k in self.KERNEL_OPTIONS},
-                                                          self.stem_onepass)
+            opts = {k: getattr(self, k) for k in self.KERNEL_OPTIONS}
+            opts["fuse_bn_bwd_small"] = self.fuse_bn_bwd_small
+            sched = self._schedules[key] = train_schedule(self._blocks_for(H, W)[0], B, opts, self.stem_onepass)
         return sched
 
     def _conv_s1(self, cs, arith, direction, x, out, B, label=None, *, in_coef=None, bias=None, addend=None, abits=None, partials=None, bn=None):
@@ -732,6 +759,8 @@
         cio = (cs.cin, cs.cout) if fwd else (cs.cout, cs.cin)
         if fn == "lad_conv_h2":
             args = (P(x), P(in_coef), wt, P(bias), P(addend), P(abits), P(out), P(partials), P(bx), P(bmask), P(bcoef), B, h, w, cs.cin)
+        elif fn == "lad_conv_h2_bits32":
+            args = (P(x), P(in_coef), wt, P(bias), P(addend), P(abits), P(out), P(partials), P(bx), P(bmask), P(bcoef), B, h, w)
         elif fn == "lad_conv_b3c_fwd_f32":
             args = (P(x), wt, P(bias), P(addend), P(out), P(partials), B, h, w, cs.cin)
         elif fn == "lad_conv_b3c_fwd_f32_bnrelu":
@@ -845,6 +874,9 @@
                     self._conv_fwd(b.sc_conv, ch.sc, cur, a["cs"], part, B)
                     self._bn_coef(b.sc_bn, a["coefs"], part, B, ho, wo)
                 self._bn_act(a["c2"], a["coef2"], a["cs"], a["coefs"], a["y"], B, ho, wo, co)
+            elif ch.bits and co == 32:
+                _hip.check(lib.lad_bn_act_bits32(_hip.ptr(a["c2"]), _hip.ptr(a["coef2"]), _hip.ptr(cur), None, _hip.ptr(a["y"]),
+                                                 _hip.ptr(a["ybits"]), B, ho, wo, st), "lad_bn_act_bits32")
             elif ch.bits:
                 _hip.check(lib.lad_bn_act_bits(_hip.ptr(a["c2"]), _hip.ptr(a["coef2"]), _hip.ptr(cur), None, _hip.ptr(a["y"]),
                                                _hip.ptr(a["ybits"]), B, ho, wo, co, st), "lad_bn_act_bits")
@@ -1474,11 +1506,17 @@
                                                        _hip.ptr(stat[2]), B, hi, wi, st), "lad_conv_s2b3_dgrad " + c1s.name)
                 elif ch.entry == "s2_fused" and ch.dgrad1_bn:
                     n_part = int(lib.lad_conv_s2_dgrad_partials(B, hi, wi))
-                    assert n_part * 2 * 64 <= p["partials"].numel()
-                    _hip.check(lib.lad_conv_s2_dgrad_fused_bnstat(_hip.ptr(dc1), _hip.ptr(c1s.par.wt_d), _hip.ptr(aux), _hip.ptr(sc.par.wt_d), _hip.ptr(dx),
-                                                                  _hip.ptr(p["partials"]), _hip.ptr(stat[0]), _hip.ptr(stat[1]),
-                                                                  _hip.ptr(stat[2]), B, hi, wi, c1s.cin, c1s.cout, st),
-                               "lad_conv_s2_dgrad_fused_bnstat " + c1s.name)
+                    assert n_part * 2 * c1s.cin <= p["partials"].numel()
+                    if c1s.cin == 32:
+                        _hip.check(lib.lad_conv_s2_dgrad_fused_bnstat32(_hip.ptr(dc1), _hip.ptr(c1s.par.wt_d), _hip.ptr(aux), _hip.ptr(sc.par.wt_d),
+                                                                         _hip.ptr(dx), _hip.ptr(p["partials"]), _hip.ptr(stat[0]), _hip.ptr(stat[1]),
+                                                                         _hip.ptr(stat[2]), B, hi, wi, st),
+                                   "lad_conv_s2_dgrad_fused_bnstat32 " + c1s.name)
+                    else:
+                        _hip.check(lib.lad_conv_s2_dgrad_fused_bnstat(_hip.ptr(dc1), _hip.ptr(c1s.par.wt_d), _hip.ptr(aux), _hip.ptr(sc.par.wt_d),
+                                                                      _hip.ptr(dx), _hip.ptr(p["partials"]), _hip.ptr(stat[0]), _hip.ptr(stat[1]),
+                                                                      _hip.ptr(stat[2]), B, hi, wi, c1s.cin, c1s.cout, st),
+                                   "lad_conv_s2_dgrad_fused_bnstat " + c1s.name)
                 elif ch.entry == "s2_fused":
                     _hip.check(lib.lad_conv_s2_dgrad_fused(_hip.ptr(dc1), _hip.ptr(c1s.par.wt_d), _hip.ptr(aux), _hip.ptr(sc.par.wt_d), _hip.ptr(dx),
                                                            B, hi, wi, c1s.cin, c1s.cout, st), "lad_conv_s2_dgrad_fused " + c1s.name)
```

After: 50250 segments/s, median of 6. Within noise of the previous version (+0.8%).
